# sunzeyeah/item-alignment

Measured on AMD Instinct MI355X. Metric: item-pairs/sec (train step) RoBERTa-large+ViT-B two-tower, higher is better.
Workload: dtype bf16

## Files before the change

include/itemalign.h:

```cpp
#ifndef ITEMALIGN_H
#define ITEMALIGN_H
#include <stddef.h>
#include <stdint.h>

#ifdef __cplusplus
extern "C" {
#endif

typedef struct ihipStream_t* ia_stream_t;

#define IA_OK 0
#define IA_ERR_ARG (-1)
#define IA_ERR_LAUNCH (-2)
#define IA_ERR_WORKSPACE (-3)
#define IA_ERR_UNSUPPORTED (-4)

const char* ia_strerror(int code);
#define IA_ABI_VERSION 17
int ia_abi_version(void);

#define IA_EPI_NONE 0
#define IA_EPI_BIAS 1
#define IA_EPI_BIAS_GELU 2
#define IA_EPI_ADD 3
#define IA_EPI_DGELU 4
#define IA_EPI_BIAS_ADD 5
#define IA_EPI_DGELU_COLSUM 6
#define IA_EPI_BIAS_GELU_ACT 7
int ia_gemm_bf16(const void* A, int a_kstrided, int lda, const void* B, int b_kstrided, int ldb, void* C, int c_is_f32, int ldc,
                 int M, int N, int K, int epilogue, const float* bias, const void* aux, int ldaux, void* C2, int accumulate,
                 void* workspace, size_t workspace_bytes, ia_stream_t stream);
int ia_gemm_bf16_qscale(const void* A, int lda, const void* B, int ldb, void* C, int ldc, int M, int N, int K, const float* bias,
                        int scaled_cols, float col_scale, ia_stream_t stream);
size_t ia_gemm_workspace_bytes(int M, int N, int K, int c_is_f32);
size_t ia_gemm_colsum_workspace_bytes(int M, int N);
size_t ia_gemm_wgrad_rows_workspace_bytes(int N_out, int N_in, int M_rows);
int ia_gemm_wgrad_rows_filters(int N_out, int N_in, int M_rows);
int ia_gemm_wgrad_rows(const void* dY, int ldy, const void* X, int ldx, float* dW, int ldw, int N_out, int N_in, int M_rows,
                       const uint8_t* row_live, int accumulate, void* workspace, size_t workspace_bytes, ia_stream_t stream);
size_t ia_ktile_mask_bytes(int M_rows);
int ia_ktile_mask(const uint8_t* row_live, int M_rows, uint32_t* mask, ia_stream_t stream);
int ia_ktile_mask_host(const uint8_t* row_live, int M_rows, uint32_t* mask);

int ia_prof_begin(int variant, int max_launches);
int ia_prof_end(double* total_ms, double* total_flops, int* launches);
double ia_prof_bytes(void);
int ia_debug_cu_hog(int workgroups, float milliseconds, ia_stream_t stream);
int ia_debug_gemm_dynamic(int on);

int ia_ln_fwd(const void* x, const float* bias, const void* residual, void* z_out, void* y, float* mean, float* rstd,
              const float* gamma, const float* beta, int M, int H, float eps, float drop_p, uint32_t seed, uint32_t stream_id,
              ia_stream_t stream);
size_t ia_ln_bwd_workspace_bytes(int M, int H);
int ia_ln_bwd(const void* dy, const void* dres, const void* z, const float* mean, const float* rstd, const float* gamma, void* dz,
              void* dx, float* dgamma, float* dbeta, float* dbias, int M, int H, float drop_p, uint32_t seed, uint32_t stream_id,
              void* workspace, size_t workspace_bytes, int accumulate, ia_stream_t stream);
int ia_ln_bwd2(const void* dy, const void* dy2, const void* dres, const void* z, const float* mean, const float* rstd, const float* gamma,
               void* dz, void* dx, float* dgamma, float* dbeta, float* dbias, int M, int H, float drop_p, uint32_t seed, uint32_t stream_id,
               void* workspace, size_t workspace_bytes, int accumulate, ia_stream_t stream);
int ia_ln_bwd2_rows(const void* dy, const void* dy2, const void* dres, const void* z, const float* mean, const float* rstd,
                    const float* gamma, void* dz, void* dx, float* dgamma, float* dbeta, float* dbias, int M, int H, float drop_p,
                    uint32_t seed, uint32_t stream_id, const uint8_t* row_live, void* workspace, size_t workspace_bytes, int accumulate,
                    ia_stream_t stream);
size_t ia_colsum_workspace_bytes(int M, int N);
int ia_colsum(const void* x, int ld, int M, int N, float* out, int accumulate, void* workspace, size_t workspace_bytes,
              ia_stream_t stream);

int ia_attn_fwd(const void* q, const void* k, const void* v, int ld_qkv, const uint8_t* key_mask, void* out, int ld_o, float* lse2,
                int B, int nh, int L, float scale, float drop_p, uint32_t seed, ia_stream_t stream);
int ia_attn_bwd(const void* q, const void* k, const void* v, int ld_qkv, const uint8_t* key_mask, const void* out, const void* d_out,
                int ld_o, const float* lse2, float* delta, void* dq, void* dk, void* dv, int ld_dqkv, int B, int nh, int L,
                float scale, float drop_p, uint32_t seed, ia_stream_t stream);
size_t ia_attn_bwd_bias_workspace_bytes(int B, int nh, int L);
int ia_attn_bwd_bias(const void* q, const void* k, const void* v, int ld_qkv, const uint8_t* key_mask, const void* out, const void* d_out,
                     int ld_o, const float* lse2, float* delta, void* dq, void* dk, void* dv, int ld_dqkv, float* dbias, void* workspace,
                     size_t workspace_bytes, int B, int nh, int L, float scale, float drop_p, uint32_t seed, ia_stream_t stream);

int ia_attn_fwd_ps(const void* q, const void* k, const void* v, int ld_qkv, const uint8_t* key_mask, void* out, int ld_o, float* lse2,
                   int B, int nh, int L, float scale, float drop_p, uint32_t seed, ia_stream_t stream);
int ia_attn_bwd_bias_ps(const void* q, const void* k, const void* v, int ld_qkv, const uint8_t* key_mask, const void* out, const void* d_out,
                        int ld_o, const float* lse2, float* delta, void* dq, void* dk, void* dv, int ld_dqkv, float* dbias, void* workspace,
                        size_t workspace_bytes, int B, int nh, int L, float scale, float drop_p, uint32_t seed, ia_stream_t stream);
#define IA_ATTN_Q_PRESCALED 1
#define IA_ATTN_MASKED_ROWS_DEAD 2
int ia_attn_bwd_bias_ex(int flags, const void* q, const void* k, const void* v, int ld_qkv, const uint8_t* key_mask, const void* out,
                        const void* d_out, int ld_o, const float* lse2, float* delta, void* dq, void* dk, void* dv, int ld_dqkv, float* dbias,
                        void* workspace, size_t workspace_bytes, int B, int nh, int L, float scale, float drop_p, uint32_t seed,
                        ia_stream_t stream);

int ia_attn_fwd_x(const void* q, int ld_q, const void* k, const void* v, int ld_kv, const uint8_t* key_mask, void* out, int ld_o,
                  float* lse2, int B, int nh, int Lq, int Lk, float scale, float drop_p, uint32_t seed, ia_stream_t stream);
int ia_attn_bwd_x(const void* q, int ld_q, const void* k, const void* v, int ld_kv, const uint8_t* key_mask, const void* out,
                  const void* d_out, int ld_o, const float* lse2, float* delta, void* dq, int ld_dq, void* dk, void* dv, int ld_dkv,
                  int B, int nh, int Lq, int Lk, float scale, float drop_p, uint32_t seed, ia_stream_t stream);
int ia_attn_fwd_causal_x(const void* q, int ld_q, const void* k, const void* v, int ld_kv, void* out, int ld_o, float* lse2, int B, int nh,
                         int Lk, int fold, float scale, ia_stream_t stream);
int ia_attn_bwd_causal_x(const void* q, int ld_q, const void* k, const void* v, int ld_kv, const void* out, const void* d_out, int ld_o,
                         const float* lse2, float* delta, void* dq, int ld_dq, void* dk, void* dv, int ld_dkv, int B, int nh, int Lk,
                         int fold, float scale, ia_stream_t stream);

int ia_rotary_split_fwd(const void* src, int ld_src, void* q_out, void* kv_out, int M, int n, int nh, ia_stream_t stream);
int ia_rotary_split_bwd(const void* dq, const void* dkv, void* dsrc, int ld_src, int M, int n, int nh, ia_stream_t stream);
int ia_swiglu_fwd(const void* src, int ld_src, void* out, int M, int F, ia_stream_t stream);
int ia_swiglu_bwd(const void* dout, const void* src, int ld_src, void* dsrc, int ld_dsrc, int M, int F, ia_stream_t stream);

int ia_kg_gather_fwd(const float* ent_table, const float* rel_table, const int64_t* ids, int ld_ids, int ent_col, int rel_lo,
                     float* h_sign, float* r, int B, int P, int Dk, ia_stream_t stream);
int ia_kg_gather_bwd(const float* dr, const int64_t* ids, int ld_ids, int rel_lo, float* rel_grad, int B, int P, int Dk,
                     ia_stream_t stream);
int ia_kg_rows_fwd(const float* h, const float* r, const float* hp, float* rows, int rows_per_item, int row0, int B, int P, int H,
                   ia_stream_t stream);
int ia_kg_rows_bwd(const float* drows, int rows_per_item, int row0, float* dh, float* dr, float* dhp, int B, int P, int H,
                   ia_stream_t stream);

#define IA_SIM_INNER 0
#define IA_SIM_COSINE 1
#define IA_SIM_L1 2
#define IA_SIM_L2 3
int ia_pair_sim_fwd(const float* x, const float* y, float* sim, float* probs, int B, int D, int measure, ia_stream_t stream);
int ia_pair_sim_bwd(const float* x, const float* y, const float* sim, const float* probs, const float* dsim, const float* dprobs,
                    float* dx, float* dy, int B, int D, int measure, ia_stream_t stream);

int ia_nchw_to_nhwc_bf16(const float* in, void* out, int B, int C, int H, int W, int Cp, ia_stream_t stream);
size_t ia_conv_nhwc_workspace_bytes(int B, int H, int W, int C, int Cout, int k, int stride, int groups);
int ia_conv_nhwc_fwd(const void* x, const void* what, const float* bias, void* y, int B, int H, int W, int C, int Cout, int k, int stride,
// ... 257 lines not shown
```

item_alignment_amd/_lib.py:

```python
import ctypes as C
import os

_HERE = os.path.dirname(os.path.abspath(__file__))
LIB_PATH = os.path.join(_HERE, "libitemalign_hip.so")

vp, i32, u32, f32, sz = C.c_void_p, C.c_int, C.c_uint32, C.c_float, C.c_size_t
PP, IP = C.POINTER(C.c_void_p), C.POINTER(C.c_int)


class LayerWeights(C.Structure):
    _fields_ = [(n, vp) for n in ("w_qkv", "b_qkv", "w_o", "b_o", "ln1_g", "ln1_b", "w_fc1", "b_fc1", "w_fc2", "b_fc2",
                                  "ln2_g", "ln2_b", "wt_qkv", "wt_o", "wt_fc1", "wt_fc2")]


class LayerGrads(C.Structure):
    _fields_ = [(n, vp) for n in ("w_qkv", "b_qkv", "w_o", "b_o", "ln1_g", "ln1_b", "w_fc1", "b_fc1", "w_fc2", "b_fc2",
                                  "ln2_g", "ln2_b")]


class LayerCfg(C.Structure):
    _fields_ = [("B", i32), ("L", i32), ("H", i32), ("I", i32), ("nh", i32), ("pre_ln", i32), ("eps", f32),
                ("hidden_drop", f32), ("attn_drop", f32), ("seed", u32), ("layer_id", u32), ("cu_seqlens", vp), ("total_tokens", i32),
                ("dx_colsum_out", vp), ("dy_colsum_done", i32), ("masked_rows_dead", i32)]


SIGNATURES = {
    "ia_strerror": (C.c_char_p, [i32]),
    "ia_abi_version": (i32, []),
    "ia_gemm_bf16": (i32, [vp, i32, i32, vp, i32, i32, vp, i32, i32, i32, i32, i32, i32, vp, vp, i32, vp, i32, vp, sz, vp]),
    "ia_gemm_workspace_bytes": (sz, [i32, i32, i32, i32]),
    "ia_gemm_colsum_workspace_bytes": (sz, [i32, i32]),
    "ia_gemm_wgrad_rows_workspace_bytes": (sz, [i32, i32, i32]),
    "ia_gemm_wgrad_rows_filters": (i32, [i32, i32, i32]),
    "ia_gemm_wgrad_rows": (i32, [vp, i32, vp, i32, vp, i32, i32, i32, i32, vp, i32, vp, sz, vp]),
    "ia_ktile_mask_bytes": (sz, [i32]),
    "ia_ktile_mask": (i32, [vp, i32, vp, vp]),
    "ia_ktile_mask_host": (i32, [vp, i32, vp]),
    "ia_prof_begin": (i32, [i32, i32]),
    "ia_prof_end": (i32, [C.POINTER(C.c_double), C.POINTER(C.c_double), C.POINTER(i32)]),
    "ia_prof_bytes": (C.c_double, []),
    "ia_debug_cu_hog": (i32, [i32, C.c_float, vp]),
    "ia_debug_gemm_dynamic": (i32, [i32]),
    "ia_ln_fwd": (i32, [vp, vp, vp, vp, vp, vp, vp, vp, vp, i32, i32, f32, f32, u32, u32, vp]),
    "ia_ln_bwd_workspace_bytes": (sz, [i32, i32]),
    "ia_ln_bwd": (i32, [vp, vp, vp, vp, vp, vp, vp, vp, vp, vp, vp, i32, i32, f32, u32, u32, vp, sz, i32, vp]),
    "ia_ln_bwd2": (i32, [vp, vp, vp, vp, vp, vp, vp, vp, vp, vp, vp, vp, i32, i32, f32, u32, u32, vp, sz, i32, vp]),
    "ia_ln_bwd2_rows": (i32, [vp, vp, vp, vp, vp, vp, vp, vp, vp, vp, vp, vp, i32, i32, f32, u32, u32, vp, vp, sz, i32, vp]),
    "ia_colsum_workspace_bytes": (sz, [i32, i32]),
    "ia_colsum": (i32, [vp, i32, i32, i32, vp, i32, vp, sz, vp]),
    "ia_attn_fwd": (i32, [vp, vp, vp, i32, vp, vp, i32, vp, i32, i32, i32, f32, f32, u32, vp]),
    "ia_attn_bwd": (i32, [vp, vp, vp, i32, vp, vp, vp, i32, vp, vp, vp, vp, vp, i32, i32, i32, i32, f32, f32, u32, vp]),
    "ia_attn_bwd_bias_workspace_bytes": (sz, [i32, i32, i32]),
    "ia_attn_bwd_bias": (i32, [vp, vp, vp, i32, vp, vp, vp, i32, vp, vp, vp, vp, vp, i32, vp, vp, sz, i32, i32, i32, f32, f32, u32, vp]),
    "ia_attn_fwd_ps": (i32, [vp, vp, vp, i32, vp, vp, i32, vp, i32, i32, i32, f32, f32, u32, vp]),
    "ia_attn_bwd_bias_ps": (i32, [vp, vp, vp, i32, vp, vp, vp, i32, vp, vp, vp, vp, vp, i32, vp, vp, sz, i32, i32, i32, f32, f32, u32, vp]),
    "ia_attn_bwd_bias_ex": (i32, [i32, vp, vp, vp, i32, vp, vp, vp, i32, vp, vp, vp, vp, vp, i32, vp, vp, sz, i32, i32, i32, f32, f32, u32, vp]),
    "ia_gemm_bf16_qscale": (i32, [vp, i32, vp, i32, vp, i32, i32, i32, i32, vp, i32, f32, vp]),
    "ia_attn_fwd_x": (i32, [vp, i32, vp, vp, i32, vp, vp, i32, vp, i32, i32, i32, i32, f32, f32, u32, vp]),
    "ia_attn_bwd_x": (i32, [vp, i32, vp, vp, i32, vp, vp, vp, i32, vp, vp, vp, i32, vp, vp, i32, i32, i32, i32, i32, f32, f32, u32, vp]),
    "ia_attn_fwd_causal_x": (i32, [vp, i32, vp, vp, i32, vp, i32, vp, i32, i32, i32, i32, f32, vp]),
    "ia_attn_bwd_causal_x": (i32, [vp, i32, vp, vp, i32, vp, vp, i32, vp, vp, vp, i32, vp, vp, i32, i32, i32, i32, i32, f32, vp]),
    "ia_rotary_split_fwd": (i32, [vp, i32, vp, vp, i32, i32, i32, vp]),
    "ia_rotary_split_bwd": (i32, [vp, vp, vp, i32, i32, i32, i32, vp]),
    "ia_swiglu_fwd": (i32, [vp, i32, vp, i32, i32, vp]),
    "ia_swiglu_bwd": (i32, [vp, vp, i32, vp, i32, i32, i32, vp]),
    "ia_kg_gather_fwd": (i32, [vp, vp, vp, i32, i32, i32, vp, vp, i32, i32, i32, vp]),
    "ia_kg_gather_bwd": (i32, [vp, vp, i32, i32, vp, i32, i32, i32, vp]),
    "ia_kg_rows_fwd": (i32, [vp, vp, vp, vp, i32, i32, i32, i32, i32, vp]),
    "ia_kg_rows_bwd": (i32, [vp, i32, i32, vp, vp, vp, i32, i32, i32, vp]),
    "ia_pair_sim_fwd": (i32, [vp, vp, vp, vp, i32, i32, i32, vp]),
    "ia_pair_sim_bwd": (i32, [vp, vp, vp, vp, vp, vp, vp, vp, i32, i32, i32, vp]),
    "ia_nchw_to_nhwc_bf16": (i32, [vp, vp, i32, i32, i32, i32, i32, vp]),
    "ia_conv_nhwc_workspace_bytes": (sz, [i32, i32, i32, i32, i32, i32, i32, i32]),
    "ia_conv_nhwc_fwd": (i32, [vp, vp, vp, vp, i32, i32, i32, i32, i32, i32, i32, i32, vp, sz, vp]),
    "ia_conv_nhwc_bwd_data": (i32, [vp, vp, vp, i32, i32, i32, i32, i32, i32, i32, i32, vp, sz, vp]),
    "ia_conv_nhwc_bwd_weight": (i32, [vp, vp, vp, vp, i32, i32, i32, i32, i32, i32, i32, i32, i32, vp, sz, vp]),
    "ia_ws_conv_weight_fwd": (i32, [vp, vp, vp, vp, vp, i32, i32, i32, i32, f32, f32, vp]),
    "ia_ws_conv_weight_bwd": (i32, [vp, vp, vp, vp, vp, vp, vp, i32, i32, i32, i32, f32, vp]),
    "ia_silu_fwd": (i32, [vp, vp, sz, f32, vp]),
    "ia_silu_bwd": (i32, [vp, vp, vp, vp, sz, f32, vp]),
    "ia_silu_bwd_sum": (i32, [vp, vp, vp, vp, vp, sz, f32, vp]),
    "ia_avgpool2_fwd": (i32, [vp, vp, i32, i32, i32, i32, vp]),
    "ia_avgpool2_bwd": (i32, [vp, vp, i32, i32, i32, i32, vp]),
    "ia_gap_workspace_bytes": (sz, [i32, i32, i32]),
    "ia_gap_fwd": (i32, [vp, vp, i32, i32, i32, vp, sz, vp]),
    "ia_gap_bwd": (i32, [vp, vp, i32, i32, i32, vp]),
    "ia_eca_fwd": (i32, [vp, vp, i32, vp, vp, vp, vp, i32, i32, i32, f32, vp, sz, vp]),
    "ia_eca_fwd_linear_workspace_bytes": (sz, [i32, i32, i32]),
    "ia_eca_fwd_linear": (i32, [vp, vp, vp, vp, i32, vp, i32, vp, vp, vp, f32, vp, vp, i32, i32, i32, f32, vp, sz, vp]),
    "ia_eca_silu_bwd": (i32, [vp, vp, vp, vp, f32, vp, vp, i32, vp, vp, vp, vp, vp, i32, i32, i32, f32, vp, sz, vp]),
    "ia_eca_bwd_workspace_bytes": (sz, [i32, i32, i32]),
    "ia_eca_bwd": (i32, [vp, vp, vp, i32, vp, vp, vp, vp, i32, i32, i32, f32, vp, sz, vp]),
    "ia_conv3x3_padded_fwd": (i32, [vp, vp, vp, vp, i32, i32, i32, i32, i32, i32, vp]),
    "ia_conv3x3_padded_bwd_data": (i32, [vp, vp, vp, i32, i32, i32, i32, i32, i32, vp]),
    "ia_conv3x3_direct_supported": (i32, [i32, i32, i32]),
    "ia_conv3x3_flip_weights": (i32, [vp, vp, i32, i32, i32, vp]),
    "ia_conv3x3_padded_bwd_data_t": (i32, [vp, vp, vp, i32, i32, i32, i32, i32, i32, vp]),
    "ia_conv3x3_padded_workspace_bytes": (sz, [i32, i32, i32, i32, i32, i32]),
    "ia_conv3x3_padded_bwd_weight": (i32, [vp, vp, vp, vp, i32, i32, i32, i32, i32, i32, vp, sz, vp]),
    "ia_pad_rows": (i32, [vp, vp, i32, i32, i32, i32, i32, i32, vp]),
    "ia_silu_pad_fwd": (i32, [vp, vp, i32, i32, i32, i32, f32, i32, i32, vp]),
    "ia_silu_pad_bwd": (i32, [vp, vp, vp, i32, i32, i32, i32, f32, i32, i32, vp]),
    "ia_bn_act_workspace_bytes": (sz, [i32, i32, i32]),
    "ia_bn_act_fwd": (i32, [vp, vp, vp, vp, vp, vp, vp, vp, i32, i32, i32, f32, f32, i32, i32, vp, sz, vp]),
    "ia_bn_act_bwd": (i32, [vp, vp, vp, vp, vp, vp, vp, vp, vp, vp, i32, i32, i32, i32, i32, vp, sz, vp]),
    "ia_patches_nchw": (i32, [vp, vp, i32, i32, i32, i32, i32, i32, i32, i32, vp]),
    "ia_conv3x3_s2_supported": (i32, [i32, i32, i32]),
    "ia_conv3x3_s2_padded_workspace_bytes": (sz, [i32, i32, i32, i32, i32, i32]),
    "ia_conv3x3_s2_padded_fwd": (i32, [vp, vp, vp, vp, i32, i32, i32, i32, i32, i32, i32, vp]),
    "ia_conv3x3_s2_padded_bwd_weight": (i32, [vp, vp, vp, vp, i32, i32, i32, i32, i32, i32, i32, vp, sz, vp]),
    "ia_conv3x3_s2_padded_bwd_data_t": (i32, [vp, vp, vp, i32, i32, i32, i32, i32, i32, i32, vp]),
    "ia_gn_act_workspace_bytes": (sz, [i32, i32, i32]),
    "ia_gn_act_fwd": (i32, [vp, vp, vp, vp, vp, vp, i32, i32, i32, i32, f32, i32, vp, sz, vp]),
    "ia_gn_act_bwd": (i32, [vp, vp, vp, vp, vp, vp, vp, vp, vp, vp, i32, i32, i32, i32, i32, vp, sz, vp]),
    "ia_maxpool3s2_fwd": (i32, [vp, vp, vp, i32, i32, i32, i32, vp]),
    "ia_maxpool3s2_fwd_ex": (i32, [vp, vp, vp, i32, i32, i32, i32, i32, vp]),
    "ia_maxpool3s2_bwd": (i32, [vp, vp, vp, i32, i32, i32, i32, vp]),
    "ia_rows_subsample_fwd": (i32, [vp, vp, i32, i32, i32, i32, i32, vp]),
    "ia_rows_subsample_bwd": (i32, [vp, vp, vp, i32, i32, i32, i32, i32, vp]),
    "ia_conv_weight_pack": (i32, [vp, vp, i32, i32, i32, i32, i32, vp]),
    "ia_conv_weight_unpack_grad": (i32, [vp, vp, i32, i32, i32, i32, i32, vp]),
    "ia_resize_pass_u8": (i32, [vp, vp, vp, vp, i32, i32, i32, i32, i32, i32, vp]),
    "ia_resize_pass_u8_ex": (i32, [vp, sz, sz, vp, vp, vp, i32, i32, i32, i32, i32, i32, vp]),
    "ia_color_jitter_step_u8": (i32, [vp, vp, vp, vp, i32, i32, i32, i32, vp]),
    "ia_u8_to_nchw_normalized": (i32, [vp, vp, vp, i32, i32, i32, C.POINTER(f32), C.POINTER(f32), vp]),
    "ia_embed_ln_fwd": (i32, [vp, vp, vp, vp, vp, vp, vp, vp, vp, vp, vp, vp, vp, vp, i32, i32, f32, f32, u32, u32, vp]),
    "ia_embed_ln_bwd_workspace_bytes": (sz, [i32, i32]),
    "ia_embed_ln_bwd": (i32, [vp, vp, vp, vp, vp, vp, vp, vp, vp, vp, vp, vp, vp, vp, vp, vp, vp, vp, vp, i32, i32, i32, i32, i32, f32, u32, u32,
                               vp, sz, vp]),
    "ia_im2col_patch": (i32, [vp, vp, i32, i32, i32, i32, vp]),
    "ia_vit_tokens_fwd": (i32, [vp, vp, vp, vp, i32, i32, i32, vp]),
    "ia_vit_tokens_bwd": (i32, [vp, vp, vp, vp, i32, i32, i32, i32, vp]),
    "ia_gather_rows_fwd": (i32, [vp, i32, vp, vp, i32, i32, f32, u32, u32, vp]),
    "ia_gather_rows_bwd": (i32, [vp, i32, vp, vp, i32, i32, f32, u32, u32, i32, vp]),
    "ia_linear_small_fwd": (i32, [vp, i32, vp, vp, vp, i32, i32, i32, i32, vp]),
    "ia_linear_small_bwd": (i32, [vp, vp, vp, i32, vp, vp, i32, vp, vp, i32, i32, i32, i32, vp]),
    "ia_pair_head_ce_fwd": (i32, [vp, vp, vp, vp, vp, vp, vp, vp, vp, i32, i32, i32, vp]),
    "ia_attn_fwd_varlen": (i32, [vp, vp, vp, i32, vp, i32, vp, i32, vp, i32, i32, i32, f32, f32, u32, vp]),
    "ia_attn_bwd_varlen": (i32, [vp, vp, vp, i32, vp, i32, vp, vp, i32, vp, vp, vp, vp, vp, i32, i32, i32, i32, f32, f32, u32, vp]),
    "ia_attn_fwd_varlen_ps": (i32, [vp, vp, vp, i32, vp, i32, vp, i32, vp, i32, i32, i32, f32, f32, u32, vp]),
    "ia_attn_bwd_varlen_ps": (i32, [vp, vp, vp, i32, vp, i32, vp, vp, i32, vp, vp, vp, vp, vp, i32, i32, i32, i32, f32, f32, u32, vp]),
    "ia_span_mean_fwd": (i32, [vp, i32, vp, vp, i32, i32, vp]),
    "ia_span_mean_bwd": (i32, [vp, vp, vp, vp, i32, i32, i32, vp]),
    "ia_pair_head_ce_bwd": (i32, [vp, vp, vp, vp, vp, vp, vp, vp, vp, vp, i32, i32, i32, vp]),
    "ia_transpose_bf16_batched": (i32, [vp, vp, vp, i32, i32, vp]),
    "ia_adamw_flat": (i32, [vp, vp, vp, vp, vp, vp, i32, f32, f32, f32, f32, f32, i32, f32, vp]),
    "ia_kgpt_workspace_bytes": (sz, [i32, i32, i32]),
    "ia_kgpt_score": (i32, [vp, vp, vp, vp, vp, vp, vp, vp, i32, i32, i32, i32, i32, i32, f32, vp, vp, vp, vp, vp, vp, vp, vp, vp, vp, vp, sz,
                            vp]),
    "ia_kgpt_adam_l2": (i32, [vp, vp, vp, vp, sz, f32, f32, f32, f32, f32, i32, vp]),
    "ia_kgpt_row_normalize": (i32, [vp, i32, i32, vp]),
    "ia_kgpt_corrupt": (i32, [vp, vp, vp, i32, vp, i32, i32, C.c_uint64, vp, vp, vp]),
    "ia_kgpt_lp_workspace_bytes": (sz, [i32, i32]),
    "ia_kgpt_lp_rank": (i32, [vp, vp, vp, vp, vp, i32, i32, i32, i32, i32, i32, vp, vp, i32, vp, vp, vp, vp, vp, sz, vp]),
    "ia_gcn_propagate_fwd": (i32, [vp, vp, i32, vp, vp, vp, vp, i32, i32, f32, f32, u32, u32, vp, i32, vp]),
    "ia_gcn_propagate_bwd": (i32, [vp, vp, i32, vp, vp, vp, vp, i32, i32, i32, f32, f32, u32, u32, vp, i32, vp]),
    "ia_gcn_mix_fwd": (i32, [vp, vp, vp, i32, i32, f32, f32, u32, u32, vp]),
    "ia_gcn_workspace_bytes": (sz, [i32, i32, i32]),
    "ia_gcn_mix_bwd": (i32, [vp, vp, vp, vp, vp, vp, i32, i32, f32, f32, vp, sz, vp]),
    "ia_gcn_input_fwd": (i32, [vp, vp, vp, vp, i32, i32, i32, f32, u32, u32, vp]),
    "ia_gcn_input_bwd": (i32, [vp, vp, vp, vp, vp, i32, i32, i32, f32, u32, u32, vp, sz, vp]),
    "ia_gcn_pair_gather_fwd": (i32, [vp, vp, vp, i32, i32, i32, f32, u32, u32, vp]),
    "ia_gcn_pair_scatter_bwd": (i32, [vp, vp, vp, vp, i32, i32, i32, f32, u32, u32, vp]),
    "ia_textcnn_pack_taps": (i32, [PP, IP, i32, i32, i32, vp, vp]),
    "ia_textcnn_pool_fwd": (i32, [vp, i32, PP, IP, i32, i32, i32, i32, f32, f32, u32, u32, u32, vp, vp, vp]),
    "ia_textcnn_pool_bwd_w": (i32, [vp, vp, vp, vp, IP, i32, i32, i32, i32, i32, f32, f32, u32, u32, u32, PP, PP, vp]),
    "ia_textcnn_pool_bwd_x": (i32, [vp, vp, PP, IP, i32, i32, i32, i32, i32, f32, f32, u32, u32, u32, vp, vp]),
    "ia_cast_f32_to_bf16": (i32, [vp, vp, sz, vp]),
    "ia_cast_bf16_to_f32": (i32, [vp, vp, sz, vp]),
    "ia_layer_stash_bytes": (sz, [C.POINTER(LayerCfg)]),
    "ia_layer_bwd_scratch_bytes": (sz, [C.POINTER(LayerCfg)]),
    "ia_layer_fwd": (i32, [C.POINTER(LayerCfg), C.POINTER(LayerWeights), vp, vp, vp, vp, vp]),
    "ia_comm_unique_id": (i32, [vp]),
    "ia_comm_init": (i32, [vp, i32, i32, C.POINTER(vp)]),
    "ia_comm_allreduce_bucket": (i32, [vp, vp, sz, i32, vp]),
    "ia_comm_finalize": (i32, [vp]),
    "ia_comm_last_error": (C.c_char_p, []),
    "ia_layer_infer_scratch_bytes": (sz, [C.POINTER(LayerCfg)]),
    "ia_layer_fwd_infer": (i32, [C.POINTER(LayerCfg), C.POINTER(LayerWeights), vp, vp, vp, vp, sz, vp]),
    "ia_layer_bwd": (i32, [C.POINTER(LayerCfg), C.POINTER(LayerWeights), C.POINTER(LayerGrads), vp, vp, vp, vp, vp, vp, vp, sz, vp]),
    "ia_layer_bwd2": (i32, [C.POINTER(LayerCfg), C.POINTER(LayerWeights), C.POINTER(LayerGrads), vp, vp, vp, vp, vp, vp, vp, vp, vp, sz, vp]),
}

_lib = None


ABI_VERSION = 17


class ItemAlignError(RuntimeError):
    pass


def load():
    global _lib
    if _lib is not None:
        return _lib
    if not os.path.exists(LIB_PATH):
        raise ItemAlignError(
            f"{LIB_PATH} not found: build it with `python -c 'import __graft_entry__ as g; g.build()'` "
            "(or `make -C item_alignment_amd/csrc`). The MI355X path has no CPU fallback.")
    import torch
    lib = C.CDLL(LIB_PATH)
    for name, (res, args) in SIGNATURES.items():
        fn = getattr(lib, name)
        fn.restype = res
        fn.argtypes = args
    got = lib.ia_abi_version()
    if got != ABI_VERSION:
        raise ItemAlignError(f"{LIB_PATH} has ABI version {got}, this package needs {ABI_VERSION} (include/itemalign.h: IA_ABI_VERSION): "
                             "stale build, run `make -C item_alignment_amd/csrc`")
    _lib = lib
    return lib


def check(rc, what):
    if rc != 0:
        msg = load().ia_strerror(rc).decode()
        raise ItemAlignError(f"{what} failed: {msg} (code {rc})")


def stream_ptr():
    import torch
    return torch.cuda.current_stream().cuda_stream


def ptr(t):
    return None if t is None else t.data_ptr()
```

item_alignment_amd/csrc/common.h:

```cpp
#pragma once
#include <hip/hip_runtime.h>
#include <stdint.h>

typedef __bf16 bf16;
typedef __attribute__((ext_vector_type(8))) __bf16 bf16x8;
typedef __attribute__((ext_vector_type(4))) __bf16 bf16x4;
typedef __attribute__((ext_vector_type(2))) __bf16 bf16x2;
typedef __attribute__((ext_vector_type(4))) short s16x4;
typedef __attribute__((ext_vector_type(8))) short s16x8;
typedef __attribute__((ext_vector_type(4))) float f32x4;
typedef __attribute__((ext_vector_type(2))) float f32x2;
typedef __attribute__((ext_vector_type(16))) float f32x16;
typedef __attribute__((ext_vector_type(4))) uint32_t u32x4;
typedef __attribute__((ext_vector_type(2))) uint32_t u32x2;

#define IA_LDS(p) ((__attribute__((address_space(3))) void*)(p))
#define IA_DEV __device__ __forceinline__

IA_DEV uint32_t ia_lds_addr(const void* p) { return (uint32_t)(uintptr_t)IA_LDS(p); }
template <int OFF>
IA_DEV s16x4 ia_tr_read(uint32_t lds_byte_addr) {
  s16x4 d;
  asm volatile("ds_read_b64_tr_b16 %0, %1 offset:%2" : "=v"(d) : "v"(lds_byte_addr), "n"(OFF));
  return d;
// ... 55 lines not shown
IA_DEV uint32_t ia_mix32(uint32_t x) {
  x ^= x >> 16; x *= 0x7feb352dU; x ^= x >> 15; x *= 0x846ca68bU; x ^= x >> 16;
  return x;
}
IA_DEV uint32_t ia_rng(uint32_t seed, uint32_t stream, uint32_t idx) {
  return ia_mix32(idx ^ ia_mix32(stream ^ (seed * 0x9E3779B9U)));
}

constexpr uint32_t IA_RNG_PAIR_C = 0x9E3779B1U;
IA_DEV uint32_t ia_rng_row(uint32_t seed, uint32_t stream, uint32_t row) { return ia_mix32(row ^ ia_mix32(stream ^ (seed * 0x9E3779B9U))); }
IA_DEV uint32_t ia_rng_pair(uint32_t rowkey, uint32_t pair_c) {
  const uint32_t h = (rowkey ^ pair_c) * 0x846ca68bU;
  return h ^ (h >> 16);
}

IA_DEV void gelu_parts(float x, float& cdf, float& pdf) {
  const float z = fabsf(x) * 0.70710678118654752f;
  const float t = __builtin_amdgcn_rcpf(1.0f + 0.3275911f * z);
  const float e = __builtin_amdgcn_exp2f(x * x * (-0.5f * 1.4426950408889634f));
  const float poly = t * (0.254829592f + t * (-0.284496736f + t * (1.421413741f + t * (-1.453152027f + t * 1.061405429f))));
  const float erf_abs = 1.0f - poly * e;
  cdf = 0.5f * (1.0f + copysignf(erf_abs, x));
  pdf = 0.3989422804014327f * e;
}
typedef float f32x2_t __attribute__((ext_vector_type(2)));
IA_DEV void gelu_pair(f32x2_t x, f32x2_t& act, f32x2_t& der) {
  constexpr float L2E = 1.4426950408889634f;
  constexpr float C0 = 1.5949398799788077f, C1 = 0.07403000634661838f, C2 = -0.0007007124749191571f;
  constexpr float U_MAX = C1 / (2.f * 0.0007007124749191571f);
  f32x2_t u = x * x;
  u[0] = __builtin_fminf(u[0], U_MAX); u[1] = __builtin_fminf(u[1], U_MAX);
  const f32x2_t np = (u * (-C2 * L2E) + (-C1 * L2E)) * u + (-C0 * L2E);
  const f32x2_t t = x * np;
  const f32x2_t e = {__builtin_amdgcn_exp2f(t[0]), __builtin_amdgcn_exp2f(t[1])};
  const f32x2_t den = e + 1.0f;
  const f32x2_t s = {__builtin_amdgcn_rcpf(den[0]), __builtin_amdgcn_rcpf(den[1])};
  act = x * s;
  const f32x2_t q = (u * (5.f * C2) + (3.f * C1)) * u + C0;
  const f32x2_t r = 1.0f - s;
  der = (act * r) * q + s;
}
IA_DEV f32x2_t gelu_act_pair(f32x2_t x) {
  constexpr float L2E = 1.4426950408889634f;
  constexpr float C0 = 1.5949398799788077f, C1 = 0.07403000634661838f, C2 = -0.0007007124749191571f;
  constexpr float U_MAX = C1 / (2.f * 0.0007007124749191571f);
  f32x2_t u = x * x;
  u[0] = __builtin_fminf(u[0], U_MAX); u[1] = __builtin_fminf(u[1], U_MAX);
  const f32x2_t t = x * ((u * (-C2 * L2E) + (-C1 * L2E)) * u + (-C0 * L2E));
  const f32x2_t e = {__builtin_amdgcn_exp2f(t[0]), __builtin_amdgcn_exp2f(t[1])};
  const f32x2_t den = e + 1.0f;
  return x * f32x2_t{__builtin_amdgcn_rcpf(den[0]), __builtin_amdgcn_rcpf(den[1])};
}
IA_DEV float gelu_erf(float x) { float c, d; gelu_parts(x, c, d); return x * c; }
IA_DEV float gelu_erf_grad(float x) { float c, d; gelu_parts(x, c, d); return c + x * d; }

inline hipError_t g_ia_last_hip_error = hipSuccess;
static inline int ia_check_launch() {
  hipError_t e = hipGetLastError();
  if (e != hipSuccess) g_ia_last_hip_error = e;
  return e == hipSuccess ? IA_OK : IA_ERR_LAUNCH;
}

struct IaViewGemm {
  const void* A; int a_kstrided, lda;
  const void* B; int b_kstrided, ldb;
  void* C; int c_is_f32, ldc;
  int M, N, K;
  const float* bias;
  float* rsum_out;
  void* workspace; size_t workspace_bytes;
  int a_view, b_view, pw, lca, lcbk, lcbn;
  size_t a_window, b_window;
  int groups; long ga, gb, gc, gbias;
};
__attribute__((visibility("hidden"))) int ia_gemm_view(const IaViewGemm& v, hipStream_t stream);
__attribute__((visibility("hidden"))) int ia_sum_rows_f32(const float* part, int nblk, int N, float* out, int accumulate, hipStream_t stream);
extern "C" size_t ia_colsum_workspace_bytes(int M, int N);
extern "C" int ia_colsum(const void* x, int ld, int M, int N, float* out, int accumulate, void* workspace, size_t workspace_bytes,
                         hipStream_t stream);
__attribute__((visibility("hidden"))) size_t ia_gemm_view_workspace_bytes(int M, int N, int K, int groups);
__attribute__((visibility("hidden"))) int ia_gemm_wgrad_masked(const void* dY, int ldy, const void* X, int ldx, float* dW, int ldw, int N_out,
                                                               int N_in, int M_rows, const uint32_t* ktile_mask, int accumulate,
                                                               void* workspace, size_t workspace_bytes, hipStream_t stream);
```

item_alignment_amd/csrc/engine.hip:

```cpp
#include "common.h"
#include "../../include/itemalign.h"

namespace {

inline size_t al(size_t b) { return (b + 255) & ~(size_t)255; }
inline size_t rows_of(const ia_layer_cfg* c) { return c->cu_seqlens ? (size_t)c->total_tokens : (size_t)c->B * c->L; }

struct Carver {
  char* base; size_t bytes = 0;
  char* take(size_t b) { char* r = base ? base + bytes : nullptr; bytes += al(b); return r; }
};

struct FwdBufs {
  char* qkv; char* ctx;
  char* xn;
  char* proj;
  char* ln;
  char* ffn;
  char* hpre;
  char* hact;
  float* lse; float* mean1; float* rstd1; float* mean2; float* rstd2;
  size_t bytes;
};

void name_rows(FwdBufs& s, bool pre_ln, char* t0, char* t1, char* t2) {
  if (pre_ln) { s.xn = t0; s.proj = t1; s.ln = t2; s.ffn = nullptr; }
  else { s.xn = nullptr; s.proj = t0; s.ln = t1; s.ffn = t2; }
}

FwdBufs carve_stash(const ia_layer_cfg* c, void* base) {
  const size_t M = rows_of(c), H = c->H, I = c->I;
  Carver a{(char*)base};
  FwdBufs s;
  s.qkv = a.take(M * 3 * H * 2); s.ctx = a.take(M * H * 2);
  char* t0 = a.take(M * H * 2); char* t1 = a.take(M * H * 2); char* t2 = a.take(M * H * 2);
  name_rows(s, c->pre_ln, t0, t1, t2);
  s.hpre = a.take(M * I * 2); s.hact = a.take(M * I * 2);
  s.lse = (float*)a.take((size_t)c->B * c->nh * c->L * 4);
  s.mean1 = (float*)a.take(M * 4); s.rstd1 = (float*)a.take(M * 4);
  s.mean2 = (float*)a.take(M * 4); s.rstd2 = (float*)a.take(M * 4);
  s.bytes = a.bytes;
  return s;
}

FwdBufs carve_infer(const ia_layer_cfg* c, void* base) {
  const size_t M = rows_of(c), H = c->H, I = c->I;
  Carver a{(char*)base};
  FwdBufs s;
  s.qkv = a.take(M * 3 * H * 2); s.ctx = a.take(M * H * 2);
  char* t0 = a.take(M * H * 2); char* t1 = a.take(M * H * 2);
  name_rows(s, c->pre_ln, t0, t1, t0);
  s.hpre = nullptr; s.hact = a.take(M * I * 2);
  s.lse = (float*)a.take((size_t)c->B * c->nh * c->L * 4);
  s.mean1 = s.mean2 = (float*)a.take(M * 4); s.rstd1 = s.rstd2 = (float*)a.take(M * 4);
  s.bytes = a.bytes;
  return s;
}

struct Scratch {
  char* g0; char* g1; char* g2; char* gI; char* gqkv; float* delta; char* ws; size_t ws_bytes; char* gws; size_t gws_bytes; uint32_t* live_kt; size_t bytes;
};

size_t max3(size_t a, size_t b, size_t c) { return a > b ? (a > c ? a : c) : (b > c ? b : c); }

Scratch carve_scratch(const ia_layer_cfg* c, void* base) {
  const size_t M = rows_of(c), H = c->H, I = c->I;
  Carver a{(char*)base};
  Scratch s;
  s.g0 = a.take(M * H * 2); s.g1 = a.take(M * H * 2); s.g2 = a.take(M * H * 2);
  s.gI = a.take(M * I * 2); s.gqkv = a.take(M * 3 * H * 2);
  s.delta = (float*)a.take((size_t)c->B * c->nh * c->L * 4);
  s.ws_bytes = max3(ia_ln_bwd_workspace_bytes((int)M, (int)H), ia_gemm_colsum_workspace_bytes((int)M, (int)I),
                    max3(ia_colsum_workspace_bytes((int)M, (int)(3 * H)), ia_attn_bwd_bias_workspace_bytes(c->B, c->nh, c->L), 0));
  s.ws = a.take(s.ws_bytes);
  s.gws_bytes = max3(ia_gemm_workspace_bytes((int)(3 * H), (int)H, (int)M, 1), ia_gemm_workspace_bytes((int)I, (int)H, (int)M, 1),
                     max3(ia_gemm_workspace_bytes((int)H, (int)I, (int)M, 1), ia_gemm_workspace_bytes((int)H, (int)H, (int)M, 1), 0));
  s.gws = a.take(s.gws_bytes);
  s.live_kt = (uint32_t*)a.take(ia_ktile_mask_bytes((int)M));
  s.bytes = a.bytes;
  return s;
}

bool cfg_ok(const ia_layer_cfg* c) {
  if (c && c->cu_seqlens && (c->total_tokens <= 0 || c->total_tokens > c->B * c->L)) return false;
  return c && c->B > 0 && c->L > 0 && c->H > 0 && c->I > 0 && c->nh > 0 && c->H == c->nh * 64 && (c->H & 7) == 0 && (c->I & 7) == 0;
}

#define IA_TRY(expr) do { int rc_ = (expr); if (rc_) return rc_; } while (0)

int dgrad(const void* dy, int k_out, const void* w, const void* wt, int n_in, void* dx, int M, int epilogue, const void* aux, int ldaux, void* c2,
          void* ws, size_t ws_bytes, ia_stream_t st) {
  if (wt)
    return ia_gemm_bf16(dy, 0, k_out, wt, 0, k_out, dx, 0, n_in, M, n_in, k_out, epilogue, nullptr, aux, ldaux, c2, 0, ws, ws_bytes, st);
  return ia_gemm_bf16(dy, 0, k_out, w, 1, n_in, dx, 0, n_in, M, n_in, k_out, epilogue, nullptr, aux, ldaux, c2, 0, ws, ws_bytes, st);
}

int wgrad(const void* dy, int n_out, const void* x, int n_in, float* dw, int M, const uint32_t* live_kt, void* ws, size_t ws_bytes, ia_stream_t st) {
  if (live_kt) return ia_gemm_wgrad_masked(dy, n_out, x, n_in, dw, n_in, n_out, n_in, M, live_kt, 1, ws, ws_bytes, st);
  return ia_gemm_bf16(dy, 1, n_out, x, 1, n_in, dw, 1, n_in, n_out, n_in, M, IA_EPI_NONE, nullptr, nullptr, 0, nullptr, 1, ws, ws_bytes, st);
}

bool q_prescale(const ia_layer_cfg* c) { return (c->H & 127) == 0; }
int qkv_proj(const ia_layer_cfg* c, const void* x, const ia_layer_weights* w, void* qkv, int M, float scale, ia_stream_t st) {
  const int H = c->H;
  if (q_prescale(c)) return ia_gemm_bf16_qscale(x, H, w->w_qkv, H, qkv, 3 * H, M, 3 * H, H, w->b_qkv, H, scale * 1.4426950408889634f, st);
  return ia_gemm_bf16(x, 0, H, w->w_qkv, 0, H, qkv, 0, 3 * H, M, 3 * H, H, IA_EPI_BIAS, w->b_qkv, nullptr, 0, nullptr, 0, nullptr, 0, st);
}

int attn_fwd(const ia_layer_cfg* c, const char* qkv, const uint8_t* key_mask, char* ctx, float* lse, float scale, float drop, uint32_t seed,
             ia_stream_t st) {
  const int H = c->H;
  const bool ps = q_prescale(c);
  if (c->cu_seqlens)
    return (ps ? ia_attn_fwd_varlen_ps : ia_attn_fwd_varlen)(qkv, qkv + (size_t)H * 2, qkv + (size_t)2 * H * 2, 3 * H, c->cu_seqlens, c->total_tokens, ctx, H, lse, c->B, c->nh,
                              c->L, scale, drop, seed, st);
  return (ps ? ia_attn_fwd_ps : ia_attn_fwd)(qkv, qkv + (size_t)H * 2, qkv + (size_t)2 * H * 2, 3 * H, key_mask, ctx, H, lse, c->B, c->nh, c->L, scale, drop, seed, st);
}

int attn_bwd(const ia_layer_cfg* c, const char* qkv, const uint8_t* key_mask, const char* ctx, const char* dctx, const float* lse, float* delta,
             char* gqkv, float* db_qkv, void* ws, size_t ws_bytes, float scale, float drop, uint32_t seed, ia_stream_t st) {
  const int H = c->H;
  const bool ps = q_prescale(c);
  if (c->cu_seqlens) {
    int rc = (ps ? ia_attn_bwd_varlen_ps : ia_attn_bwd_varlen)(qkv, qkv + (size_t)H * 2, qkv + (size_t)2 * H * 2, 3 * H, c->cu_seqlens, c->total_tokens, ctx, dctx, H, lse, delta,
                                gqkv, gqkv + (size_t)H * 2, gqkv + (size_t)2 * H * 2, 3 * H, c->B, c->nh, c->L, scale, drop, seed, st);
    return rc ? rc : ia_colsum(gqkv, 3 * H, (int)rows_of(c), 3 * H, db_qkv, 1, ws, ws_bytes, st);
  }
  const int flags = (ps ? IA_ATTN_Q_PRESCALED : 0) | (c->masked_rows_dead ? IA_ATTN_MASKED_ROWS_DEAD : 0);
  return ia_attn_bwd_bias_ex(flags, qkv, qkv + (size_t)H * 2, qkv + (size_t)2 * H * 2, 3 * H, key_mask, ctx, dctx, H, lse, delta, gqkv,
                             gqkv + (size_t)H * 2, gqkv + (size_t)2 * H * 2, 3 * H, db_qkv, ws, ws_bytes, c->B, c->nh, c->L, scale, drop, seed, st);
}

int layer_forward(const ia_layer_cfg* c, const ia_layer_weights* w, const void* x, const uint8_t* key_mask, void* y, const FwdBufs& s,
                  bool keep, ia_stream_t st) {
  const int M = (int)rows_of(c), H = c->H, I = c->I;
  const float scale = 0.125f;
  const int gelu = keep ? IA_EPI_BIAS_GELU : IA_EPI_BIAS_GELU_ACT;
  if (!c->pre_ln) {
    const float hidden_drop = keep ? c->hidden_drop : 0.f, attn_drop = keep ? c->attn_drop : 0.f;
    const uint32_t seed = keep ? c->seed : 0u, attn_seed = keep ? c->seed * 2654435761u + c->layer_id * 97u + 17u : 0u;
    const uint32_t ln1_stream = keep ? c->layer_id * 4u + 0u : 0u, ln2_stream = keep ? c->layer_id * 4u + 1u : 0u;
    IA_TRY(qkv_proj(c, x, w, s.qkv, M, scale, st));
    IA_TRY(attn_fwd(c, s.qkv, key_mask, s.ctx, s.lse, scale, attn_drop, attn_seed, st));
    IA_TRY(ia_gemm_bf16(s.ctx, 0, H, w->w_o, 0, H, s.proj, 0, H, M, H, H, IA_EPI_NONE, nullptr, nullptr, 0, nullptr, 0, nullptr, 0, st));
    IA_TRY(ia_ln_fwd(s.proj, w->b_o, x, keep ? s.proj : nullptr, s.ln, s.mean1, s.rstd1, w->ln1_g, w->ln1_b, M, H, c->eps, hidden_drop, seed,
                     ln1_stream, st));
    IA_TRY(ia_gemm_bf16(s.ln, 0, H, w->w_fc1, 0, H, s.hact, 0, I, M, I, H, gelu, w->b_fc1, nullptr, 0, s.hpre, 0, nullptr, 0, st));
    IA_TRY(ia_gemm_bf16(s.hact, 0, I, w->w_fc2, 0, I, s.ffn, 0, H, M, H, I, IA_EPI_NONE, nullptr, nullptr, 0, nullptr, 0, nullptr, 0, st));
    IA_TRY(ia_ln_fwd(s.ffn, w->b_fc2, s.ln, keep ? s.ffn : nullptr, y, s.mean2, s.rstd2, w->ln2_g, w->ln2_b, M, H, c->eps, hidden_drop, seed,
                     ln2_stream, st));
  } else {
    IA_TRY(ia_ln_fwd(x, nullptr, nullptr, nullptr, s.xn, s.mean1, s.rstd1, w->ln1_g, w->ln1_b, M, H, c->eps, 0.f, 0, 0, st));
    IA_TRY(qkv_proj(c, s.xn, w, s.qkv, M, scale, st));
    IA_TRY(attn_fwd(c, s.qkv, key_mask, s.ctx, s.lse, scale, 0.f, 0, st));
    IA_TRY(ia_gemm_bf16(s.ctx, 0, H, w->w_o, 0, H, s.proj, 0, H, M, H, H, IA_EPI_NONE, nullptr, nullptr, 0, nullptr, 0, nullptr, 0, st));
    IA_TRY(ia_ln_fwd(s.proj, w->b_o, x, s.proj, s.ln, s.mean2, s.rstd2, w->ln2_g, w->ln2_b, M, H, c->eps, 0.f, 0, 0, st));
    IA_TRY(ia_gemm_bf16(s.ln, 0, H, w->w_fc1, 0, H, s.hact, 0, I, M, I, H, gelu, w->b_fc1, nullptr, 0, s.hpre, 0, nullptr, 0, st));
    IA_TRY(ia_gemm_bf16(s.hact, 0, I, w->w_fc2, 0, I, y, 0, H, M, H, I, IA_EPI_BIAS_ADD, w->b_fc2, s.proj, H, nullptr, 0, nullptr, 0, st));
  }
  return IA_OK;
}

}

extern "C" size_t ia_layer_stash_bytes(const ia_layer_cfg* cfg) {
  (void)hipGetLastError();
  if (!cfg_ok(cfg)) return 0;
  return carve_stash(cfg, nullptr).bytes;
}

extern "C" size_t ia_layer_bwd_scratch_bytes(const ia_layer_cfg* cfg) {
  (void)hipGetLastError();
  if (!cfg_ok(cfg)) return 0;
  return carve_scratch(cfg, nullptr).bytes;
}

extern "C" size_t ia_layer_infer_scratch_bytes(const ia_layer_cfg* cfg) {
  (void)hipGetLastError();
  if (!cfg_ok(cfg)) return 0;
  return carve_infer(cfg, nullptr).bytes;
}

extern "C" int ia_layer_fwd(const ia_layer_cfg* c, const ia_layer_weights* w, const void* x, const uint8_t* key_mask, void* y,
                            void* stash, ia_stream_t st) {
  (void)hipGetLastError();
  if (!cfg_ok(c) || !w || !x || !y || !stash) return IA_ERR_ARG;
  if (c->pre_ln && (c->hidden_drop > 0.f || c->attn_drop > 0.f)) return IA_ERR_UNSUPPORTED;
  return layer_forward(c, w, x, key_mask, y, carve_stash(c, stash), true, st);
}

extern "C" int ia_layer_fwd_infer(const ia_layer_cfg* c, const ia_layer_weights* w, const void* x, const uint8_t* key_mask, void* y,
                                  void* scratch, size_t scratch_bytes, ia_stream_t st) {
  (void)hipGetLastError();
  if (!cfg_ok(c) || !w || !x || !y || !scratch) return IA_ERR_ARG;
  if (scratch_bytes < ia_layer_infer_scratch_bytes(c)) return IA_ERR_WORKSPACE;
  return layer_forward(c, w, x, key_mask, y, carve_infer(c, scratch), false, st);
}

extern "C" int ia_layer_bwd2(const ia_layer_cfg* c, const ia_layer_weights* w, const ia_layer_grads* g, const void* x,
                             const uint8_t* key_mask, const void* y, const void* stash, const void* dy, const void* dy2, void* dx, void* dx2,
                             void* scratch, size_t scratch_bytes, ia_stream_t st);

extern "C" int ia_layer_bwd(const ia_layer_cfg* c, const ia_layer_weights* w, const ia_layer_grads* g, const void* x,
                            const uint8_t* key_mask, const void* y, const void* stash, const void* dy, void* dx, void* scratch,
                            size_t scratch_bytes, ia_stream_t st) {
  return ia_layer_bwd2(c, w, g, x, key_mask, y, stash, dy, nullptr, dx, nullptr, scratch, scratch_bytes, st);
}

extern "C" int ia_layer_bwd2(const ia_layer_cfg* c, const ia_layer_weights* w, const ia_layer_grads* g, const void* x,
                             const uint8_t* key_mask, const void* y, const void* stash, const void* dy, const void* dy2, void* dx, void* dx2,
                             void* scratch, size_t scratch_bytes, ia_stream_t st) {
  (void)hipGetLastError();
  (void)y;
  if (!cfg_ok(c) || !w || !g || !x || !stash || !dy || !dx || !scratch) return IA_ERR_ARG;
  if (c->pre_ln && (dy2 || dx2)) return IA_ERR_UNSUPPORTED;
  if (scratch_bytes < ia_layer_bwd_scratch_bytes(c)) return IA_ERR_WORKSPACE;
  const int M = (int)rows_of(c), H = c->H, I = c->I;
  const FwdBufs s = carve_stash(c, const_cast<void*>(stash));
  const Scratch k = carve_scratch(c, scratch);
  const float scale = 0.125f;
  const uint32_t attn_seed = c->seed * 2654435761u + c->layer_id * 97u + 17u;
  const bool drop = c->hidden_drop > 0.f;
  if (!c->pre_ln) {
    const uint8_t* const live = (c->masked_rows_dead && !c->cu_seqlens) ? key_mask : nullptr;
    const uint32_t* const live_kt = live ? k.live_kt : nullptr;
    if (live) IA_TRY(ia_ktile_mask(live, M, k.live_kt, st));
    IA_TRY(ia_ln_bwd2_rows(dy, dy2, nullptr, s.ffn, s.mean2, s.rstd2, w->ln2_g, k.g0, drop ? k.g1 : nullptr, g->ln2_g, g->ln2_b, g->b_fc2, M, H,
                           c->hidden_drop, c->seed, c->layer_id * 4u + 1u, live, k.ws, k.ws_bytes, 1, st));
    const char* d_ffn = drop ? k.g1 : k.g0;
    IA_TRY(wgrad(d_ffn, H, s.hact, I, (float*)g->w_fc2, M, live_kt, k.gws, k.gws_bytes, st));
    IA_TRY(dgrad(d_ffn, H, w->w_fc2, w->wt_fc2, I, k.gI, M, IA_EPI_DGELU_COLSUM, s.hpre, I, g->b_fc1, k.ws, k.ws_bytes, st));
    IA_TRY(wgrad(k.gI, I, s.ln, H, (float*)g->w_fc1, M, live_kt, k.gws, k.gws_bytes, st));
    IA_TRY(dgrad(k.gI, I, w->w_fc1, w->wt_fc1, H, k.g2, M, IA_EPI_NONE, nullptr, 0, nullptr, nullptr, 0, st));
    char* dz1buf = dx2 ? (char*)dx2 : k.g0;
    IA_TRY(ia_ln_bwd2_rows(k.g2, k.g0, nullptr, s.proj, s.mean1, s.rstd1, w->ln1_g, dz1buf, drop ? k.g1 : nullptr, g->ln1_g, g->ln1_b, g->b_o, M, H,
                           c->hidden_drop, c->seed, c->layer_id * 4u + 0u, live, k.ws, k.ws_bytes, 1, st));
    const char* d_att = drop ? k.g1 : dz1buf;
    IA_TRY(wgrad(d_att, H, s.ctx, H, (float*)g->w_o, M, live_kt, k.gws, k.gws_bytes, st));
    IA_TRY(dgrad(d_att, H, w->w_o, w->wt_o, H, k.g2, M, IA_EPI_NONE, nullptr, 0, nullptr, nullptr, 0, st));
    IA_TRY(attn_bwd(c, s.qkv, key_mask, s.ctx, k.g2, s.lse, k.delta, k.gqkv, g->b_qkv, k.ws, k.ws_bytes, scale, c->attn_drop, attn_seed, st));
    IA_TRY(wgrad(k.gqkv, 3 * H, x, H, (float*)g->w_qkv, M, live_kt, k.gws, k.gws_bytes, st));
    if (dx2)
      IA_TRY(dgrad(k.gqkv, 3 * H, w->w_qkv, w->wt_qkv, H, dx, M, IA_EPI_NONE, nullptr, 0, nullptr, nullptr, 0, st));
    else
      IA_TRY(dgrad(k.gqkv, 3 * H, w->w_qkv, w->wt_qkv, H, dx, M, IA_EPI_ADD, dz1buf, H, nullptr, nullptr, 0, st));
  } else {
    if (!c->dy_colsum_done) IA_TRY(ia_colsum(dy, H, M, H, g->b_fc2, 1, k.ws, k.ws_bytes, st));
    IA_TRY(ia_gemm_bf16(dy, 1, H, s.hact, 1, I, g->w_fc2, 1, I, H, I, M, IA_EPI_NONE, nullptr, nullptr, 0, nullptr, 1, k.gws, k.gws_bytes, st));
    IA_TRY(dgrad(dy, H, w->w_fc2, w->wt_fc2, I, k.gI, M, IA_EPI_DGELU_COLSUM, s.hpre, I, g->b_fc1, k.ws, k.ws_bytes, st));
    IA_TRY(ia_gemm_bf16(k.gI, 1, I, s.ln, 1, H, g->w_fc1, 1, H, I, H, M, IA_EPI_NONE, nullptr, nullptr, 0, nullptr, 1, k.gws, k.gws_bytes, st));
    IA_TRY(dgrad(k.gI, I, w->w_fc1, w->wt_fc1, H, k.g0, M, IA_EPI_NONE, nullptr, 0, nullptr, nullptr, 0, st));
    IA_TRY(ia_ln_bwd(k.g0, dy, s.proj, s.mean2, s.rstd2, w->ln2_g, k.g1, nullptr, g->ln2_g, g->ln2_b, g->b_o, M, H, 0.f, 0, 0, k.ws,
                     k.ws_bytes, 1, st));
    IA_TRY(ia_gemm_bf16(k.g1, 1, H, s.ctx, 1, H, g->w_o, 1, H, H, H, M, IA_EPI_NONE, nullptr, nullptr, 0, nullptr, 1, k.gws, k.gws_bytes, st));
    IA_TRY(dgrad(k.g1, H, w->w_o, w->wt_o, H, k.g2, M, IA_EPI_NONE, nullptr, 0, nullptr, nullptr, 0, st));
    IA_TRY(attn_bwd(c, s.qkv, key_mask, s.ctx, k.g2, s.lse, k.delta, k.gqkv, g->b_qkv, k.ws, k.ws_bytes, scale, 0.f, 0, st));
    IA_TRY(ia_gemm_bf16(k.gqkv, 1, 3 * H, s.xn, 1, H, g->w_qkv, 1, H, 3 * H, H, M, IA_EPI_NONE, nullptr, nullptr, 0, nullptr, 1, k.gws, k.gws_bytes, st));
    IA_TRY(dgrad(k.gqkv, 3 * H, w->w_qkv, w->wt_qkv, H, k.g0, M, IA_EPI_NONE, nullptr, 0, nullptr, nullptr, 0, st));
    IA_TRY(ia_ln_bwd(k.g0, k.g1, x, s.mean1, s.rstd1, w->ln1_g, dx, nullptr, g->ln1_g, g->ln1_b, c->dx_colsum_out, M, H, 0.f, 0, 0, k.ws,
                     k.ws_bytes, 1, st));
  }
  return IA_OK;
}
```

item_alignment_amd/csrc/gemm.hip:

```cpp
#include "common.h"
#include <atomic>
#include <cstdlib>
#include <type_traits>

#ifndef IA_GEMM_DBG_HOOKS
#define IA_GEMM_DBG_HOOKS 0
#endif
#define IA_DBG(p) (IA_GEMM_DBG_HOOKS ? (p).dbg : 0)

namespace {

constexpr int BK = 64;
constexpr uint32_t OOB = 0xFFFFFFF0u;

enum { EPI_NONE = 0, EPI_BIAS = 1, EPI_BIAS_GELU = 2, EPI_ADD = 3, EPI_DGELU = 4, EPI_BIAS_ADD = 5, EPI_DGELU_CS = 6, EPI_BIAS_GELU_ACT = 7 };
constexpr int EPI_NONE_LIVE = 8;

struct GemmArgs {
  const bf16* A; const bf16* B; void* C; bf16* C2;
  union {
    const float* bias;
    const uint32_t* live_kt;
  };
  const bf16* aux;
  int M, N, K;
  int lda, ldb, ldc, ldaux;
  uint64_t a_bytes, b_bytes;
  int accumulate;
  int qcols; float qscale;
  int tiles_m, tiles_n;
  int splits, nk_per_split;
  float* csum_part;
  int split_id;
  float* ws;
  float* rsum_out;
  float* rsum_ws;
  int dbg;
  int a_view, b_view, pw, lca, lcbk, lcbn;
  int groups;
  long ga, gb, gc, gbias;
  uint32_t* tile_ctr;
};

constexpr int CTR_SLOTS = 1024, CTR_WORDS = 16;
__device__ uint32_t g_tile_ctr[CTR_SLOTS * CTR_WORDS];

IA_DEV int tap_delta(int t, int pw) { return (t / 3 - 1) * pw + (t % 3 - 1); }

IA_DEV __amdgpu_buffer_rsrc_t rsrc_at(const bf16* base, uint64_t total_bytes, uint64_t origin) {
  const uint64_t ob = origin * 2, rem = total_bytes > ob ? total_bytes - ob : 0;
  return ia_rsrc(base + origin, (uint32_t)(rem < 0x7FFFFFF0ull ? rem : 0x7FFFFFF0ull));
}

template <int EPI, bool OUTF32>
IA_DEV void epi_store4(const GemmArgs& p, int m, int n, f32x4 v) {
  if (EPI == EPI_BIAS || EPI == EPI_BIAS_GELU || EPI == EPI_BIAS_GELU_ACT || EPI == EPI_BIAS_ADD) {
    const f32x4 b = *reinterpret_cast<const f32x4*>(p.bias + n);
    v += b;
    if (EPI == EPI_BIAS && n < p.qcols) v *= p.qscale;
  }
  if (EPI == EPI_BIAS_GELU) {
    bf16x4 der;
#pragma unroll
    for (int r = 0; r < 4; r += 2) {
      f32x2_t a, d;
      gelu_pair(f32x2_t{v[r], v[r + 1]}, a, d);
      v[r] = a[0]; v[r + 1] = a[1];
      der[r] = f2bf(d[0]); der[r + 1] = f2bf(d[1]);
    }
    *reinterpret_cast<bf16x4*>(p.C2 + (size_t)m * p.ldc + n) = der;
  }
  if (EPI == EPI_BIAS_GELU_ACT) {
#pragma unroll
    for (int r = 0; r < 4; r += 2) {
      const f32x2_t a = gelu_act_pair(f32x2_t{v[r], v[r + 1]});
      v[r] = a[0]; v[r + 1] = a[1];
    }
  }
  if (EPI == EPI_ADD || EPI == EPI_BIAS_ADD) {
    const bf16x4 a = *reinterpret_cast<const bf16x4*>(p.aux + (size_t)m * p.ldaux + n);
#pragma unroll
    for (int r = 0; r < 4; ++r) v[r] += bf2f(a[r]);
  }
  if (EPI == EPI_DGELU || EPI == EPI_DGELU_CS) {
    const bf16x4 a = *reinterpret_cast<const bf16x4*>(p.aux + (size_t)m * p.ldaux + n);
#pragma unroll
    for (int r = 0; r < 4; ++r) v[r] *= bf2f(a[r]);
  }
  if (OUTF32) {
    if (p.splits > 1) {
      *reinterpret_cast<f32x4*>(p.ws + ((size_t)p.split_id * p.M + m) * p.N + n) = v;
      return;
    }
    float* c = reinterpret_cast<float*>(p.C) + (size_t)m * p.ldc + n;
    if (p.accumulate) { const f32x4 o = *reinterpret_cast<const f32x4*>(c); v += o; }
    *reinterpret_cast<f32x4*>(c) = v;
  } else {
    bf16x4 o = {f2bf(v[0]), f2bf(v[1]), f2bf(v[2]), f2bf(v[3])};
    *reinterpret_cast<bf16x4*>(reinterpret_cast<bf16*>(p.C) + (size_t)m * p.ldc + n) = o;
  }
}

template <typename V>
IA_DEV void gstore16(void* ptr, V v) {
  static_assert(sizeof(V) == 16, "16-byte store");
// ... 377 lines not shown
  bf16x8 d;
  asm volatile("ds_read_b128 %0, %1 offset:%2" : "=v"(d) : "v"(addr), "n"(IMM));
  return d;
}
template <int IMM>
IA_DEV s16x4 rd_tr(uint32_t addr) {
  s16x4 d;
  asm volatile("ds_read_b64_tr_b16 %0, %1 offset:%2" : "=v"(d) : "v"(addr), "n"(IMM));
  return d;
}

template <bool KS>
IA_DEV void frag_bases(uint32_t (&base)[4], uint32_t tile_addr, int x0, int lane, int nperm_row) {
  if (!KS) {
    const int hh = lane >> 5;
    const int row = x0 + nperm_row;
#pragma unroll
    for (int ks = 0; ks < 4; ++ks) base[ks] = tile_addr + row * 128 + ((((ks * 2 + hh) ^ ((row >> 1) & 7))) << 4);
  } else {
    const int p = lane & 15, G = lane >> 4;
#pragma unroll
    for (int j = 0; j < 4; ++j) {
      const int row = 8 * (G >> 1) + (p >> 2);
      const int col = x0 + j * 32 + 16 * (G & 1) + (p & 3) * 4;
      base[j] = tile_addr + row * 512 + ((((col >> 3) ^ ((row & 3) << 2))) << 4) + (col & 7) * 2;
    }
  }
}

template <int N> IA_DEV void tie(Op<false>& o) {
  asm volatile("s_waitcnt lgkmcnt(%4)" : "+v"(o.v[0]), "+v"(o.v[1]), "+v"(o.v[2]), "+v"(o.v[3]) : "n"(N));
}
template <int N> IA_DEV void tie2(Op<false>& a, Op<false>& b) {
  asm volatile("s_waitcnt lgkmcnt(%8)" : "+v"(a.v[0]), "+v"(a.v[1]), "+v"(a.v[2]), "+v"(a.v[3]), "+v"(b.v[0]), "+v"(b.v[1]), "+v"(b.v[2]), "+v"(b.v[3]) : "n"(N));
}
template <int N> IA_DEV void tie6(Op<false>& a, Op<false>& b, Op<false>& c, Op<false>& d, Op<false>& e, Op<false>& f) {
  asm volatile("s_waitcnt lgkmcnt(%24)"
               : "+v"(a.v[0]), "+v"(a.v[1]), "+v"(a.v[2]), "+v"(a.v[3]), "+v"(b.v[0]), "+v"(b.v[1]), "+v"(b.v[2]), "+v"(b.v[3]),
                 "+v"(c.v[0]), "+v"(c.v[1]), "+v"(c.v[2]), "+v"(c.v[3]), "+v"(d.v[0]), "+v"(d.v[1]), "+v"(d.v[2]), "+v"(d.v[3]),
                 "+v"(e.v[0]), "+v"(e.v[1]), "+v"(e.v[2]), "+v"(e.v[3]), "+v"(f.v[0]), "+v"(f.v[1]), "+v"(f.v[2]), "+v"(f.v[3])
               : "n"(N));
}
template <int N> IA_DEV void tie(Op<true>& o) {
  asm volatile("s_waitcnt lgkmcnt(%8)" : "+v"(o.lo[0]), "+v"(o.lo[1]), "+v"(o.lo[2]), "+v"(o.lo[3]), "+v"(o.hi[0]), "+v"(o.hi[1]), "+v"(o.hi[2]), "+v"(o.hi[3]) : "n"(N));
}
template <int N> IA_DEV void tie2(Op<true>& a, Op<true>& b) { tie<N>(a); tie<N>(b); }
template <int N> IA_DEV void tie6(Op<true>& a, Op<true>& b, Op<true>& c, Op<true>& d, Op<true>& e, Op<true>& f) {
  tie<N>(a); tie<N>(b); tie<N>(c); tie<N>(d); tie<N>(e); tie<N>(f);
}


template <int S, bool KS>
IA_DEV void read_frag(Op<KS>& f, int j, const uint32_t (&base)[4], uint32_t bufoff) {
  if constexpr (!KS) {
    const uint32_t a = base[S] + bufoff;
    if (j == 0) f.v[0] = rd128<0>(a);
    if (j == 1) f.v[1] = rd128<4096>(a);
    if (j == 2) f.v[2] = rd128<8192>(a);
    if (j == 3) f.v[3] = rd128<12288>(a);
  } else {
    f.lo[j] = rd_tr<S * 8192>(base[j] + bufoff);
    f.hi[j] = rd_tr<S * 8192 + 4 * 512>(base[j] + bufoff);
  }
}

template <bool FRESH, typename FA, typename FB, typename Filler>
IA_DEV void mfma_step(f32x16 (&acc)[4][4], const FA& fa, const FB& fb, Filler&& filler) {
  bf16x8 va[4], vb[4];
#pragma unroll
  for (int j = 0; j < 4; ++j) { va[j] = frag_of(fa, j); vb[j] = frag_of(fb, j); }
#pragma unroll
  for (int mi = 0; mi < 4; ++mi)
#pragma unroll
    for (int ni = 0; ni < 4; ++ni) {
      if constexpr (FRESH) {
        const f32x16 z = {0.f, 0.f, 0.f, 0.f, 0.f, 0.f, 0.f, 0.f, 0.f, 0.f, 0.f, 0.f, 0.f, 0.f, 0.f, 0.f};
        acc[mi][ni] = __builtin_amdgcn_mfma_f32_32x32x16_bf16(vb[ni], va[mi], z, 0, 0, 0);
      } else acc[mi][ni] = __builtin_amdgcn_mfma_f32_32x32x16_bf16(vb[ni], va[mi], acc[mi][ni], 0, 0, 0);
      filler(mi * 4 + ni);
      __builtin_amdgcn_sched_barrier(0);
    }
}

struct LiveWalk {
  uint64_t rest;
  uint32_t w;
  int wi, cur;
};
IA_DEV void live_start(LiveWalk& k, uint32_t mv) { k.rest = __ballot(mv != 0u); k.w = 0u; k.wi = 0; k.cur = -1; }
IA_DEV int live_next(LiveWalk& k, uint32_t mv) {
  const bool open = k.w == 0u, any = k.rest != 0ull;
  const int wi = open ? (any ? __builtin_ctzll(k.rest) : 0) : k.wi;
  const uint32_t fetched = __builtin_amdgcn_readlane(mv, wi);
  const uint32_t w = open ? (any ? fetched : 0u) : k.w;
  k.rest = open ? (k.rest & (k.rest - 1ull)) : k.rest;
  const int idx = w != 0u ? wi * 32 + __builtin_ctz(w) : k.cur + 1;
  k.w = w & (w - 1u); k.wi = wi; k.cur = idx;
  return idx;
}

template <bool AKS, bool BKS, int PEND, bool PEEL_OK = true, bool LIVE = false>
IA_DEV void main_loop(const GemmArgs& p, char* smem, f32x16 (&acc)[4][4], __amdgpu_buffer_rsrc_t rsA, __amdgpu_buffer_rsrc_t rsB, int xa, int xb,
                      int kt0, int ktaA0, int ktaB0, int n_tiles, int nk_all, int wm, int wn, int wave, int lane, bool prologue_only,
                      bool stores_in_flight, uint32_t live_mv = 0u) {
  static_assert(!LIVE || (AKS && BKS), "the live-k-tile walk advances the running lane offsets of two k-strided operands");
  constexpr bool ROUND = !AKS && !BKS;
  const int li = lane & 31;
  const int gt = wave * 64 + lane;
  uint32_t voffA, stepA, voffB, stepB;
  if (!AKS) { const int row = gt >> 3; voffA = (uint32_t)(((xa + row) * p.lda + (((gt & 7) ^ ((row >> 1) & 7)) * 8)) * 2); stepA = (uint32_t)(32 * p.lda * 2); }
  else { const int row = gt >> 5; voffA = (uint32_t)((row * p.lda + xa + (((gt & 31) ^ ((row & 3) << 2)) * 8)) * 2); stepA = (uint32_t)(8 * p.lda * 2); }
  if (!BKS) { const int row = gt >> 3; voffB = (uint32_t)(((xb + row) * p.ldb + (((gt & 7) ^ ((row >> 1) & 7)) * 8)) * 2); stepB = (uint32_t)(32 * p.ldb * 2); }
  else { const int row = gt >> 5; voffB = (uint32_t)((row * p.ldb + xb + (((gt & 31) ^ ((row & 3) << 2)) * 8)) * 2); stepB = (uint32_t)(8 * p.ldb * 2); }
  const uint32_t kstepA = AKS ? (uint32_t)(BK * p.lda * 2) : (uint32_t)(BK * 2), kstepB = BKS ? (uint32_t)(BK * p.ldb * 2) : (uint32_t)(BK * 2);
  const int klA = AKS ? (gt >> 5) : ((gt & 7) ^ (((gt >> 3) >> 1) & 7)) * 8;
  const int klB = BKS ? (gt >> 5) : ((gt & 7) ^ (((gt >> 3) >> 1) & 7)) * 8;
  char* const my_part = smem + wave * 1024;
  const int dbg = IA_GEMM_DBG_HOOKS ? p.dbg : 0;
  const bool dma_on = !(dbg & 2);
  [[maybe_unused]] LiveWalk lw;
  int live0 = 0, live1 = 1;
  if constexpr (LIVE) { live_start(lw, live_mv); live0 = live_next(lw, live_mv); live1 = live_next(lw, live_mv); }

  auto dma_piece = [&](int u, int i) {
    const bool isB = i >= 8;
    const int j = i & 7;
    char* dst = my_part + (isB ? TILE_BYTES : 0) + (u & 1) * 2 * TILE_BYTES + j * 4096;
    const int kt = kt0 + u;
    const int kta = (dbg & 4) ? 0 : (isB ? ktaB0 : ktaA0) + (LIVE ? (u == 0 ? live0 : live1) : u);
    const bool ks = isB ? BKS : AKS;
    const uint32_t soff = (uint32_t)kta * (isB ? kstepB : kstepA) + (uint32_t)j * (isB ? stepB : stepA);
    if (ks) {
      const uint32_t off = (dma_on && (!LIVE || u < n_tiles)) ? (isB ? voffB : voffA) + soff : OOB;
      __builtin_amdgcn_raw_ptr_buffer_load_lds(isB ? rsB : rsA, IA_LDS(dst), 16, off, 0, 0, 0);
    } else {
      const int lim = (u < n_tiles && dma_on) ? p.K - kt * BK : 0;
      const uint32_t off = (isB ? klB : klA) + (ks ? j * 8 : 0) < lim ? (isB ? voffB : voffA) : OOB;
      __builtin_amdgcn_raw_ptr_buffer_load_lds(isB ? rsB : rsA, IA_LDS(dst), 16, off, (int)soff, 0, 0);
    }
  };

  auto off_of = [&](int u, bool isB) -> uint32_t {
    const int lim = (u < n_tiles && dma_on) ? p.K - (kt0 + u) * BK : 0;
    return (isB ? klB : klA) < lim ? (isB ? voffB : voffA) : OOB;
  };
  auto dma_c = [&](int u, int i, uint32_t off) {
    const bool isB = i >= 8;
    const int j = i & 7;
    char* dst = my_part + (isB ? TILE_BYTES : 0) + (u & 1) * 2 * TILE_BYTES + j * 4096;
    const int kta = (dbg & 4) ? 0 : (isB ? ktaB0 : ktaA0) + u;
    const uint32_t soff = (uint32_t)kta * (isB ? kstepB : kstepA) + (uint32_t)j * (isB ? stepB : stepA);
    __builtin_amdgcn_raw_ptr_buffer_load_lds(isB ? rsB : rsA, IA_LDS(dst), 16, off, (int)soff, 0, 0);
  };

  int live2 = 2;
  if constexpr (LIVE) { if (!prologue_only) live2 = live_next(lw, live_mv); }
  uint32_t runA = voffA + (uint32_t)((dbg & 4) ? 0 : ktaA0 + live2) * kstepA, runB = voffB + (uint32_t)((dbg & 4) ? 0 : ktaB0 + live2) * kstepB;
  auto dma_run = [&](int u, int i) {
    const bool isB = i >= 8;
    if (!(isB ? BKS : AKS) || (dbg & 4)) { dma_piece(u, i); return; }
    const int j = i & 7;
    char* dst = my_part + (isB ? TILE_BYTES : 0) + (u & 1) * 2 * TILE_BYTES + j * 4096;
    const uint32_t off = (isB ? runB : runA) + (uint32_t)j * (isB ? stepB : stepA);
    __builtin_amdgcn_raw_ptr_buffer_load_lds(isB ? rsB : rsA, IA_LDS(dst), 16, dma_on ? off : OOB, 0, 0, 0);
  };

  if (prologue_only) {
#pragma unroll
    for (int i = 0; i < 16; ++i) dma_piece(0, i);
#pragma unroll
    for (int i = 0; i < (ROUND ? 12 : 16); ++i) dma_piece(1, i);
    return;
  }
  if (stores_in_flight) asm volatile("s_waitcnt vmcnt(%0)" : : "n"(PEND < 60 ? PEND : 60) : "memory");
  else asm volatile("s_waitcnt vmcnt(0)" ::: "memory");
  __builtin_amdgcn_s_barrier();

  const int nperm = ((li >> 2) & 1) * 16 + (li >> 3) * 4 + (li & 3);
  uint32_t baseA[4], baseB[4];
  const uint32_t smem_addr = ia_lds_addr(smem);
  frag_bases<AKS>(baseA, smem_addr, wm * 128, lane, li);
  frag_bases<BKS>(baseB, smem_addr + TILE_BYTES, wn * 128, lane, nperm);
  constexpr int NRA = AKS ? 8 : 4, NRB = BKS ? 8 : 4, NR = NRA + NRB;
  constexpr int NR15 = NR > 15 ? 15 : NR;

  Op<AKS> a0, a1, a2, a3;
  Op<BKS> b0, b1, b2, b3;
#pragma unroll
  for (int j = 0; j < 4; ++j) read_frag<0>(a0, j, baseA, 0u);
#pragma unroll
  for (int j = 0; j < 4; ++j) read_frag<0>(b0, j, baseB, 0u);

  using Acc = std::false_type;

  uint32_t bo = 0;
  int u = 0;
  if constexpr (ROUND) {
  uint32_t offA = OOB, offB = off_of(1, true);
  auto trip = [&](auto FIRST_T) {
    const uint32_t bn = bo ^ (uint32_t)(2 * TILE_BYTES);
    tie2<0>(a0, b0);
    mfma_step<decltype(FIRST_T)::value>(acc, a0, b0, [&](int i) {
      if (i < 4) { read_frag<1>(a1, i, baseA, bo); read_frag<1>(b1, i, baseB, bo); }
      else if (i < 8) { read_frag<2>(a2, i - 4, baseA, bo); read_frag<2>(b2, i - 4, baseB, bo); }
      else if (i < 12) { read_frag<3>(a3, i - 8, baseA, bo); read_frag<3>(b3, i - 8, baseB, bo); }
      if (i % 4 == 3) dma_c(u + 1, 12 + i / 4, offB);
      if (i == 12) offA = off_of(u + 2, false);
    });
    tie6<0>(a1, b1, a2, b2, a3, b3);
    __builtin_amdgcn_sched_barrier(0);
    if (!(dbg & 16)) __builtin_amdgcn_s_barrier();
    __builtin_amdgcn_sched_barrier(0);
    mfma_step<false>(acc, a1, b1, [&](int i) {
      if (i % 4 == 1) dma_c(u + 2, i / 4, offA);
    });
    mfma_step<false>(acc, a2, b2, [&](int i) {
      if (i % 4 == 1) dma_c(u + 2, 4 + i / 4, offA);
      if (i == 14) offB = off_of(u + 2, true);
    });
    asm volatile("s_waitcnt vmcnt(8)" ::: "memory");
    __builtin_amdgcn_sched_barrier(0);
    if (!(dbg & 16)) __builtin_amdgcn_s_barrier();
    __builtin_amdgcn_sched_barrier(0);
    mfma_step<false>(acc, a3, b3, [&](int i) {
      if (i < 4) read_frag<0>(a0, i, baseA, bn);
      else if (i < 8) read_frag<0>(b0, i - 4, baseB, bn);
      if (i % 4 == 3) dma_c(u + 2, 8 + i / 4, offB);
    });
    bo = bn;
    ++u;
    };
  if constexpr (PEEL_OK) {
    trip(std::true_type{});
    do { trip(Acc{}); } while (u < n_tiles);
  } else {
    do { trip(Acc{}); } while (u < n_tiles);
  }
  tie2<0>(a0, b0);
  return;
  }
  do {
    const uint32_t bn = bo ^ (uint32_t)(2 * TILE_BYTES);
    tie<0>(a0); tie<0>(b0);
    mfma_step<false>(acc, a0, b0, [&](int i) {
      if (i < 4) read_frag<1>(a1, i, baseA, bo);
      else if (i < 8) read_frag<1>(b1, i - 4, baseB, bo);
      else if (i < 12) read_frag<2>(a2, i - 8, baseA, bo);
      else read_frag<2>(b2, i - 12, baseB, bo);
    });
    tie<NR15>(a1); tie<NR15>(b1);
    mfma_step<false>(acc, a1, b1, [&](int i) {
      if (i < 4) read_frag<3>(a3, i, baseA, bo);
      else if (i < 8) read_frag<3>(b3, i - 4, baseB, bo);
    });
    tie<0>(a2); tie<0>(b2); tie<0>(a3); tie<0>(b3);
    __builtin_amdgcn_sched_barrier(0);
    if (!(dbg & 16)) __builtin_amdgcn_s_barrier();
    __builtin_amdgcn_sched_barrier(0);
    mfma_step<false>(acc, a2, b2, [&](int i) {
      if (i & 1) dma_run(u + 2, i >> 1);
    });
    asm volatile("s_waitcnt vmcnt(8)" ::: "memory");
    __builtin_amdgcn_sched_barrier(0);
    if (!(dbg & 16)) __builtin_amdgcn_s_barrier();
    __builtin_amdgcn_sched_barrier(0);
    mfma_step<false>(acc, a3, b3, [&](int i) {
      if (i & 1) dma_run(u + 2, 8 + (i >> 1));
      if (!(i & 1)) {
        if (i < 8) read_frag<0>(a0, i >> 1, baseA, bn);
        else read_frag<0>(b0, (i - 8) >> 1, baseB, bn);
      }
    });
    bo = bn;
    ++u;
    if constexpr (LIVE) {
      const int at = lw.cur;
      const uint32_t hop = (uint32_t)(live_next(lw, live_mv) - at);
      runA += hop * kstepA; asm volatile("" : "+v"(runA));
      runB += hop * kstepB; asm volatile("" : "+v"(runB));
    } else {
      if (AKS) { runA += kstepA; asm volatile("" : "+v"(runA)); }
      if (BKS) { runB += kstepB; asm volatile("" : "+v"(runB)); }
    }
  } while (u < n_tiles);
  tie<0>(a0); tie<0>(b0);
}

template <bool BKS, int NH, bool WITH_BIAS>
IA_DEV void drain_half_plain(const GemmArgs& p, f32x16 (&acc)[4][4], int m0, int n0, char* stg, int lane_e, const f32x4 (&bct)[4][4], float ts = 1.f) {
  static_assert(!(WITH_BIAS && BKS), "bias rows are laid out for the k-contiguous B fragment permutation");
  const int hh = lane_e >> 5, li = lane_e & 31, rrow = lane_e >> 3, c8 = lane_e & 7;
  auto stage = [&](int mi) {
    char* const sl = stg + (mi & 1) * 4096;
#pragma unroll
    for (int ni = 0; ni < 2; ++ni) {
      f32x16& a = acc[mi][NH * 2 + ni];
      if (!BKS) {
#pragma unroll
        for (int h8 = 0; h8 < 2; ++h8) {
          f32x4 t0, t1;
#pragma unroll
          for (int j = 0; j < 4; ++j) {
            asm volatile("v_accvgpr_read_b32 %0, %1" : "=v"(t0[j]) : "a"(a[h8 * 8 + j]));
            asm volatile("v_accvgpr_read_b32 %0, %1" : "=v"(t1[j]) : "a"(a[h8 * 8 + 4 + j]));
          }
          if (WITH_BIAS) { t0 = t0 * ts + bct[NH * 2 + ni][h8 * 2]; t1 = t1 * ts + bct[NH * 2 + ni][h8 * 2 + 1]; }
          const bf16x8 v = {f2bf(t0[0]), f2bf(t0[1]), f2bf(t0[2]), f2bf(t0[3]), f2bf(t1[0]), f2bf(t1[1]), f2bf(t1[2]), f2bf(t1[3])};
          const int chunk = (ni * 32 + hh * 16 + h8 * 8) >> 3;
          *reinterpret_cast<bf16x8*>(sl + li * 128 + ((chunk ^ (li & 7)) << 4)) = v;
        }
      } else {
#pragma unroll
        for (int rg = 0; rg < 4; ++rg) {
          f32x4 t0;
#pragma unroll
          for (int j = 0; j < 4; ++j) asm volatile("v_accvgpr_read_b32 %0, %1" : "=v"(t0[j]) : "a"(a[rg * 4 + j]));
          const bf16x4 v = {f2bf(t0[0]), f2bf(t0[1]), f2bf(t0[2]), f2bf(t0[3])};
          const int col = ni * 32 + rg * 8 + hh * 4;
          *reinterpret_cast<bf16x4*>(sl + li * 128 + (((col >> 3) ^ (li & 7)) << 4) + (col & 7) * 2) = v;
        }
      }
#pragma unroll
      for (int r = 0; r < 16; ++r) a[r] = 0.f;
      __builtin_amdgcn_sched_barrier(0);
    }
  };
  const int rows_left = p.M - m0;
  const uint64_t wbytes = rows_left > 0 ? (uint64_t)rows_left * p.ldc * 2 : 0;
  const __amdgpu_buffer_rsrc_t rsC = ia_rsrc(reinterpret_cast<bf16*>(p.C) + (size_t)m0 * p.ldc, (uint32_t)(wbytes < 0x7FFFFFF0ull ? wbytes : 0x7FFFFFF0ull));
  const int ncol = n0 + c8 * 8;
  const uint32_t voffC = ncol < p.N ? (uint32_t)((rrow * p.ldc + ncol) * 2) : 0x80000000u;
  stage(0);
#pragma unroll
  for (int mi = 0; mi < 4; ++mi) {
    __builtin_amdgcn_wave_barrier();
    const char* const sl = stg + (mi & 1) * 4096;
    u32x4 v[4];
#pragma unroll
    for (int it = 0; it < 4; ++it) {
      const int row = it * 8 + rrow;
      v[it] = *reinterpret_cast<const u32x4*>(sl + row * 128 + ((c8 ^ (row & 7)) << 4));
    }
    __builtin_amdgcn_wave_barrier();
    if (mi < 3) stage(mi + 1);
#pragma unroll
    for (int it = 0; it < 4; ++it) {
      const uint32_t off = voffC + (uint32_t)((mi * 32 + it * 8) * p.ldc * 2);
      if (!IA_GEMM_DBG_HOOKS || !(p.dbg & 64)) __builtin_amdgcn_raw_buffer_store_b128(v[it], rsC, (int)off, 0, 0);
      else asm volatile("" : : "v"(v[it]));
    }
  }
}

template <int EPI, bool OUTF32, bool BKS, int NH>
IA_DEV void drain_half(const GemmArgs& p, f32x16 (&acc)[4][4], int m0, int n0, char* stg, int lane_e, bool full, bool bias_ready, f32x4 bias_lo,
                       f32x4 bias_hi) {
  const int hh = lane_e >> 5, li = lane_e & 31;
  const int rrow = lane_e >> 3, c8 = lane_e & 7;
  constexpr bool HAS_BIAS = EPI == EPI_BIAS || EPI == EPI_BIAS_GELU || EPI == EPI_BIAS_GELU_ACT || EPI == EPI_BIAS_ADD;
  constexpr bool HAS_AUX = EPI == EPI_ADD || EPI == EPI_BIAS_ADD || EPI == EPI_DGELU || EPI == EPI_DGELU_CS;
  constexpr int AHEAD = 4;
  auto drain = [&](auto PREFETCHED) {
    constexpr bool PRE = decltype(PREFETCHED)::value;
    f32x4 pb0, pb1;
    float cs[8];
    if (EPI == EPI_DGELU_CS) {
#pragma unroll
      for (int j = 0; j < 8; ++j) asm volatile("v_mov_b32 %0, 0" : "=v"(cs[j]));
    }
    bf16x8 ax[AHEAD + 1];
    constexpr bool BUF = PRE && !OUTF32;
    const auto window = [&](const void* base, int ld) {
      const uint64_t bytes = (uint64_t)(p.M - m0) * ld * 2;
      return ia_rsrc(reinterpret_cast<const bf16*>(base) + (size_t)m0 * ld, (uint32_t)(bytes < 0x7FFFFFF0ull ? bytes : 0x7FFFFFF0ull));
    };
    BufIO io{ia_rsrc(nullptr, 0), ia_rsrc(nullptr, 0), 0u};
    __amdgpu_buffer_rsrc_t rsAux = ia_rsrc(nullptr, 0);
    uint32_t voffC = 0, voffAux = 0;
    if (BUF) {
      io.rsC = window(p.C, p.ldc);
      if (EPI == EPI_BIAS_GELU) io.rsC2 = window(p.C2, p.ldc);
      voffC = (uint32_t)((rrow * p.ldc + n0 + c8 * 8) * 2);
      if (HAS_AUX) { rsAux = window(p.aux, p.ldaux); voffAux = (uint32_t)((rrow * p.ldaux + n0 + c8 * 8) * 2); }
    }
    auto aux_of = [&](int c) {
      const int row_in = (c >> 2) * 32 + ((c >> 1) & 1) * 16 + (c & 1) * 8;
      if (BUF) return __builtin_bit_cast(bf16x8, __builtin_amdgcn_raw_buffer_load_b128(rsAux, (int)(voffAux + (uint32_t)(row_in * p.ldaux * 2)), 0, 0));
      return *reinterpret_cast<const bf16x8*>(p.aux + (size_t)(m0 + row_in + rrow) * p.ldaux + n0 + c8 * 8);
    };
    if (PRE && HAS_BIAS) {
      if (bias_ready) { pb0 = bias_lo; pb1 = bias_hi; }
      else { pb0 = *reinterpret_cast<const f32x4*>(p.bias + n0 + c8 * 8); pb1 = *reinterpret_cast<const f32x4*>(p.bias + n0 + c8 * 8 + 4); }
    }
    if (PRE && HAS_AUX) {
#pragma unroll
      for (int c = 0; c < AHEAD; ++c) ax[c] = aux_of(c);
    }
    auto stage = [&](int mi) {
#pragma unroll
      for (int ni = 0; ni < 2; ++ni)
#pragma unroll
        for (int rg = 0; rg < 4; ++rg) {
          const int chunk = (ni * 32 + (BKS ? rg * 8 + hh * 4 : hh * 16 + rg * 4)) >> 2;
          f32x16& a = acc[mi][NH * 2 + ni];
          const f32x4 v = {a[rg * 4], a[rg * 4 + 1], a[rg * 4 + 2], a[rg * 4 + 3]};
          *reinterpret_cast<f32x4*>(stg + li * 256 + ((chunk ^ (li & 15)) << 4)) = v;
          a[rg * 4] = 0.f; a[rg * 4 + 1] = 0.f; a[rg * 4 + 2] = 0.f; a[rg * 4 + 3] = 0.f;
        }
    };
    stage(0);
#pragma unroll
    for (int mi = 0; mi < 4; ++mi) {
      __builtin_amdgcn_wave_barrier();
      f32x4 lo[4], hi[4];
#pragma unroll
      for (int it = 0; it < 4; ++it) {
        const int row = it * 8 + rrow;
        lo[it] = *reinterpret_cast<const f32x4*>(stg + row * 256 + (((2 * c8) ^ (row & 15)) << 4));
        hi[it] = *reinterpret_cast<const f32x4*>(stg + row * 256 + (((2 * c8 + 1) ^ (row & 15)) << 4));
      }
      asm volatile("s_waitcnt lgkmcnt(0)" : "+v"(lo[0]), "+v"(lo[1]), "+v"(lo[2]), "+v"(lo[3]), "+v"(hi[0]), "+v"(hi[1]), "+v"(hi[2]), "+v"(hi[3]));
      __builtin_amdgcn_wave_barrier();
      if (mi < 3) stage(mi + 1);
#pragma unroll
      for (int it = 0; it < 4; ++it) {
        const int row = it * 8 + rrow;
        const int m = m0 + mi * 32 + row, n = n0 + c8 * 8;
        const int c = mi * 4 + it;
        if (PRE) {
          if (HAS_AUX && c + AHEAD < 16) {
            ax[(c + AHEAD) % (AHEAD + 1)] = aux_of(c + AHEAD);
            asm volatile("" ::: "memory");
          }
          io.off = voffC + (uint32_t)((mi * 32 + it * 8) * p.ldc * 2);
          if (!(IA_DBG(p) & 64)) epi_store8<EPI, OUTF32, true, BUF>(p, m, n, lo[it], hi[it], pb0, pb1, ax[c % (AHEAD + 1)], cs, &io);
        } else {
          if (m < p.M && n < p.N && !(IA_DBG(p) & 64)) epi_store8<EPI, OUTF32, false>(p, m, n, lo[it], hi[it], pb0, pb1, ax[0], cs);
        }
        if (IA_DBG(p) & 64) asm volatile("" : : "v"(lo[it]), "v"(hi[it]));
      }
    }
    if (EPI == EPI_DGELU_CS) {
#pragma unroll
      for (int r = 0; r < 8; ++r) {
        float v = cs[r];
        v += __builtin_bit_cast(float, __builtin_amdgcn_update_dpp(__builtin_bit_cast(int, v), __builtin_bit_cast(int, v), 0x128, 0xF, 0xF, false));
        v = ia_add_xor32(ia_add_xor16(v));
        cs[r] = v;
      }
      if (rrow == 0 && n0 + c8 * 8 < p.N) {
        float* dst = p.csum_part + (size_t)(m0 >> 7) * p.N + n0 + c8 * 8;
        gstore16(dst, f32x4{cs[0], cs[1], cs[2], cs[3]});
        gstore16(dst + 4, f32x4{cs[4], cs[5], cs[6], cs[7]});
      }
    }
  };
  if (full && (HAS_BIAS || HAS_AUX) && !(IA_DBG(p) & 256)) drain(std::true_type{}); else drain(std::false_type{});
}

template <bool AKS, bool BKS, int EPI_, bool OUTF32>
__global__ __launch_bounds__(256) void gemm_kernel(GemmArgs p) {
  constexpr bool LIVE = EPI_ == EPI_NONE_LIVE;
  constexpr int EPI = LIVE ? (int)EPI_NONE : EPI_;
  static_assert(!LIVE || (AKS && BKS && OUTF32), "live k-tiles: the weight-gradient form only");
  extern __shared__ __attribute__((aligned(16))) char smem[];
  const int tid = threadIdx.x, lane0 = tid & 63;
  const int wave = __builtin_amdgcn_readfirstlane(tid >> 6);
  const int wm = wave >> 1, wn = wave & 1;
  const int nk_all = (p.K + BK - 1) / BK;
  const int total_tiles = p.tiles_m * p.tiles_n;
  int first_tile = blockIdx.x;
  bool ordered = false;
  p.split_id = 0;
  if (p.splits > 1) {
    const int w = xcd_chunk(blockIdx.x, gridDim.x);
    p.split_id = w / total_tiles;
    first_tile = w % total_tiles;
    ordered = true;
  }
  const int kt0 = p.split_id * p.nk_per_split;
  int n_tiles = min(nk_all, kt0 + p.nk_per_split) - kt0;
  uint32_t live_mv = 0u;
  if constexpr (LIVE) {
    const int nw = (nk_all + 31) >> 5, first = kt0 + 32 * lane0, wlo = first >> 5, sh = first & 31, left = n_tiles - 32 * lane0;
    const uint32_t lo = wlo < nw ? p.live_kt[wlo] : 0u, hi = wlo + 1 < nw ? p.live_kt[wlo + 1] : 0u;
    live_mv = sh ? (lo >> sh) | (hi << (32 - sh)) : lo;
    live_mv = left >= 32 ? live_mv : (left > 0 ? live_mv & ((1u << left) - 1u) : 0u);
    n_tiles = 0;
    for (uint64_t rest = __ballot(live_mv != 0u); rest; rest &= rest - 1ull)
      n_tiles += __builtin_popcount(__builtin_amdgcn_readlane(live_mv, __builtin_ctzll(rest)));
  }
  constexpr int PEND = 2 * (16 * epi_stores_per_call<EPI, OUTF32>() + epi_extra_stores<EPI>());
  auto coords = [&](int tile, int& bm, int& bn) {
    if (ordered) tile_of_order(p, tile, bm, bn); else tile_of_index(p, tile, total_tiles, bm, bn);
  };
  auto run = [&](int tile, bool prologue_only, f32x16 (&acc)[4][4], bool stores_in_flight) {
    int bm, bn;
    coords(tile, bm, bn);
    int lane = lane0;
    asm volatile("" : "+v"(lane));
    const uint64_t oa = (uint64_t)(AKS ? kt0 * BK : bm * BM) * p.lda, ob = (uint64_t)(BKS ? kt0 * BK : bn * BN) * p.ldb;
    constexpr bool PEEL_OK = !(EPI == EPI_BIAS && !OUTF32 && !BKS);
    main_loop<AKS, BKS, PEND, PEEL_OK, LIVE>(p, smem, acc, rsrc_at(p.A, p.a_bytes, oa), rsrc_at(p.B, p.b_bytes, ob), AKS ? bm * BM : 0, BKS ? bn * BN : 0, kt0,
                              AKS ? 0 : kt0, BKS ? 0 : kt0, n_tiles, nk_all, wm, wn, wave, lane, prologue_only, stores_in_flight, live_mv);
  };

  const bool dyn = p.tile_ctr != nullptr && !ordered;
  const int xcd = blockIdx.x & 7, q8 = total_tiles >> 3, r8 = total_tiles & 7;
  auto run_start = [&](int x) { return x < r8 ? x * (q8 + 1) : r8 * (q8 + 1) + (x - r8) * q8; };
  auto run_len = [&](int x) { return q8 + (x < r8 ? 1 : 0); };
  int* const mailbox = reinterpret_cast<int*>(smem + 2 * 2 * TILE_BYTES);
  uint32_t claimed = 0;
  auto claim_issue = [&]() {
    if (wave == 0 && lane0 == 0)
      {
        const uint64_t a64 = (uint64_t)(p.tile_ctr + xcd);
        const uint32_t alo = __builtin_amdgcn_readfirstlane((uint32_t)a64), ahi = __builtin_amdgcn_readfirstlane((uint32_t)(a64 >> 32));
        const uint64_t addr = ((uint64_t)ahi << 32) | alo;
        asm volatile("s_nop 4\n\tglobal_atomic_add %0, %1, %2, %3 sc0" : "=v"(claimed) : "v"(0u), "v"(1u), "s"(addr) : "memory");
      }
  };
  auto claim_resolve = [&]() -> int {
    asm volatile("s_waitcnt vmcnt(0)" : "+v"(claimed));
    if (wave == 0) {
      int pos = (int)__builtin_amdgcn_readfirstlane(claimed), w = -1;
      if (pos < run_len(xcd)) w = run_start(xcd) + pos;
      else {
        uint32_t seen = 0xFFFFFFFFu;
        if (lane0 < 8) seen = __hip_atomic_load(p.tile_ctr + lane0, __ATOMIC_RELAXED, __HIP_MEMORY_SCOPE_AGENT);
        const uint32_t mask = (uint32_t)__ballot((int)seen >= q8 + (lane0 < r8 ? 1 : 0)) | (1u << xcd);
        for (int d = 1; d < 8 && w < 0; ++d) {
          const int x = (xcd + d) & 7;
          if ((mask >> x) & 1u) continue;
          uint32_t got = 0;
          if (lane0 == 0) got = __hip_atomic_fetch_add(p.tile_ctr + x, 1u, __ATOMIC_RELAXED, __HIP_MEMORY_SCOPE_AGENT);
          pos = (int)__builtin_amdgcn_readfirstlane(got);
          if (pos < run_len(x)) w = run_start(x) + pos;
        }
      }
      if (lane0 == 0) *reinterpret_cast<volatile int*>(mailbox) = w;
    }
    __syncthreads();
    const int w = __builtin_amdgcn_readfirstlane(*reinterpret_cast<volatile int*>(mailbox));
    __syncthreads();
    return w;
  };
  auto leave = [&]() {
    asm volatile("s_waitcnt vmcnt(0)" : "+v"(claimed) : : "memory");
    if (dyn && wave == 0 && lane0 == 0) {
      const uint32_t d = __hip_atomic_fetch_add(p.tile_ctr + 8, 1u, __ATOMIC_RELAXED, __HIP_MEMORY_SCOPE_AGENT);
      if (d == gridDim.x - 1) {
#pragma unroll
        for (int i = 0; i < 9; ++i) __hip_atomic_store(p.tile_ctr + i, 0u, __ATOMIC_RELAXED, __HIP_MEMORY_SCOPE_AGENT);
      }
    }
  };
  if (dyn) {
    ordered = true;
    claim_issue();
    first_tile = claim_resolve();
    if (first_tile < 0) { leave(); return; }
    claim_issue();
  }

  f32x16 acc[4][4];
#pragma unroll
  for (int i = 0; i < 4; ++i)
#pragma unroll
    for (int j = 0; j < 4; ++j)
#pragma unroll
      for (int r = 0; r < 16; ++r) acc[i][j][r] = 0.f;
  int tile = first_tile;
  run(tile, true, acc, false);
  bool stores_in_flight = false;
  constexpr bool HAS_BIAS_K = EPI == EPI_BIAS || EPI == EPI_BIAS_GELU || EPI == EPI_BIAS_GELU_ACT || EPI == EPI_BIAS_ADD;
  while (true) {
    int bm, bn;
    coords(tile, bm, bn);
    const int m0_pre = bm * BM + wm * 128, n0_pre = bn * BN + wn * 128;
    const bool full = m0_pre + 128 <= p.M && n0_pre + 128 <= p.N;
    constexpr bool BIAS_CT = EPI == EPI_BIAS && !OUTF32 && !BKS;
    f32x4 pbv[4] = {};
    f32x4 bct[4][4] = {};
    int lane_b = lane0;
    asm volatile("" : "+v"(lane_b));
    const bool bias_pre = HAS_BIAS_K && full;
    if (bias_pre && BIAS_CT) {
      const float* bp = p.bias + n0_pre + (lane_b >> 5) * 16;
#pragma unroll
      for (int ni = 0; ni < 4; ++ni)
#pragma unroll
        for (int q = 0; q < 4; ++q) bct[ni][q] = *reinterpret_cast<const f32x4*>(bp + ni * 32 + q * 4);
    } else if (bias_pre) {
      const float* bp = p.bias + n0_pre + (lane_b & 7) * 8;
      pbv[0] = *reinterpret_cast<const f32x4*>(bp); pbv[1] = *reinterpret_cast<const f32x4*>(bp + 4);
      pbv[2] = *reinterpret_cast<const f32x4*>(bp + 64); pbv[3] = *reinterpret_cast<const f32x4*>(bp + 68);
    }
    run(tile, false, acc, stores_in_flight);
    float ts = 1.f;
    if (bias_pre && BIAS_CT) {
#pragma unroll
      for (int ni = 0; ni < 4; ++ni)
        asm volatile("s_waitcnt vmcnt(0)" : "+v"(bct[ni][0]), "+v"(bct[ni][1]), "+v"(bct[ni][2]), "+v"(bct[ni][3]));
      if (n0_pre < p.qcols) {
        ts = p.qscale;
#pragma unroll
        for (int ni = 0; ni < 4; ++ni)
#pragma unroll
          for (int q = 0; q < 4; ++q) bct[ni][q] *= ts;
      }
    } else if (bias_pre) asm volatile("s_waitcnt vmcnt(0)" : "+v"(pbv[0]), "+v"(pbv[1]), "+v"(pbv[2]), "+v"(pbv[3]));
    int next = ordered ? total_tiles : tile + gridDim.x;
    if (dyn) {
      next = claim_resolve();
      claim_issue();
      if (next < 0) next = total_tiles;
    }
    if (next < total_tiles) run(next, true, acc, false);

    int lane_e = lane0;
    asm volatile("" : "+v"(lane_e));
    int m0 = m0_pre, n0 = n0_pre;
    asm volatile("" : "+s"(m0), "+s"(n0));
    char* stg = smem + 2 * 2 * TILE_BYTES + wave * 2 * STAGE_BYTES;
    if (!(IA_DBG(p) & 32)) {
      if constexpr (EPI == EPI_NONE && !OUTF32) {
        drain_half_plain<BKS, 0, false>(p, acc, m0, n0, stg, lane_e, bct);
        drain_half_plain<BKS, 1, false>(p, acc, m0, n0 + 64, stg, lane_e, bct);
      } else if (BIAS_CT && bias_pre) {
        drain_half_plain<false, 0, BIAS_CT>(p, acc, m0, n0, stg, lane_e, bct, ts);
        drain_half_plain<false, 1, BIAS_CT>(p, acc, m0, n0 + 64, stg, lane_e, bct, ts);
      } else {
        drain_half<EPI, OUTF32, BKS, 0>(p, acc, m0, n0, stg, lane_e, full || (m0 + 128 <= p.M && n0 + 64 <= p.N), bias_pre, pbv[0], pbv[1]);
        drain_half<EPI, OUTF32, BKS, 1>(p, acc, m0, n0 + 64, stg, lane_e, full, bias_pre, pbv[2], pbv[3]);
      }
    }
    if (next >= total_tiles) break;
    stores_in_flight = !(IA_DBG(p) & 96) && full;
    if (!stores_in_flight) asm volatile("s_waitcnt vmcnt(0)" ::: "memory");
    tile = next;
  }
  leave();
}

}



namespace t256la {
using namespace t256w;

__global__ __launch_bounds__(256) void gemm_kernel(GemmArgs p) {
  extern __shared__ __attribute__((aligned(16))) char smem[];
  const int tid = threadIdx.x, lane0 = tid & 63;
  const int wave = __builtin_amdgcn_readfirstlane(tid >> 6);
  const int wm = wave >> 1, wn = wave & 1;
  const int nk_all = (p.K + BK - 1) / BK;
  const int total_tiles = p.tiles_m * p.tiles_n;
  const int n_tiles = nk_all;
  auto coords = [&](int tile, int& bm, int& bn) { tile_of_index(p, tile, total_tiles, bm, bn); };
  auto window_a = [&](int tile) {
    int bm = 0, bn = 0;
    if (tile < total_tiles) coords(tile, bm, bn);
    return tile < total_tiles ? rsrc_at(p.A, p.a_bytes, (uint64_t)bm * BM * p.lda) : ia_rsrc(p.A, 0u);
  };
  auto window_b = [&](int tile) {
    int bm = 0, bn = 0;
    if (tile < total_tiles) coords(tile, bm, bn);
    return tile < total_tiles ? rsrc_at(p.B, p.b_bytes, (uint64_t)bn * BN * p.ldb) : ia_rsrc(p.B, 0u);
  };

  int lane = lane0;
  asm volatile("" : "+v"(lane));
  const int li = lane & 31;
  const int gt = wave * 64 + lane;
  const int rowd = gt >> 3;
  const uint32_t voffA = (uint32_t)((rowd * p.lda + (((gt & 7) ^ ((rowd >> 1) & 7)) * 8)) * 2), stepA = (uint32_t)(32 * p.lda * 2);
  const uint32_t voffB = (uint32_t)((rowd * p.ldb + (((gt & 7) ^ ((rowd >> 1) & 7)) * 8)) * 2), stepB = (uint32_t)(32 * p.ldb * 2);
  const int kl = ((gt & 7) ^ (((gt >> 3) >> 1) & 7)) * 8;
  char* const my_part = smem + wave * 1024;
  const int nperm = ((li >> 2) & 1) * 16 + (li >> 3) * 4 + (li & 3);
  uint32_t baseA[4], baseB[4];
  const uint32_t smem_addr = ia_lds_addr(smem);
  frag_bases<false>(baseA, smem_addr, wm * 128, lane, li);
  frag_bases<false>(baseB, smem_addr + TILE_BYTES, wn * 128, lane, nperm);

  int tile = blockIdx.x;
  __amdgpu_buffer_rsrc_t rsA = window_a(tile), rsB = window_b(tile);
  __amdgpu_buffer_rsrc_t rsAn = window_a(tile + (int)gridDim.x), rsBn = window_b(tile + (int)gridDim.x);

  auto off_of = [&](int v) -> uint32_t {
    const int kt = v >= n_tiles ? v - n_tiles : v;
    return kl < p.K - kt * BK ? 1u : 0u;
  };
  auto dma = [&](int v, int i, uint32_t ok, uint32_t buf) {
    const bool isB = i >= 8, nx = v >= n_tiles;
    const int j = i & 7, kt = nx ? v - n_tiles : v;
    char* dst = my_part + (isB ? TILE_BYTES : 0) + buf + j * 4096;
    const uint32_t soff = (uint32_t)kt * (uint32_t)(BK * 2) + (uint32_t)j * (isB ? stepB : stepA);
    const uint32_t off = ok ? (isB ? voffB : voffA) : OOB;
    __builtin_amdgcn_raw_ptr_buffer_load_lds(isB ? (nx ? rsBn : rsB) : (nx ? rsAn : rsA), IA_LDS(dst), 16, off, (int)soff, 0, 0);
  };

#pragma unroll
  for (int i = 0; i < 16; ++i) dma(0, i, off_of(0), 0u);
#pragma unroll
  for (int i = 0; i < 16; ++i) dma(1, i, off_of(1), (uint32_t)(2 * TILE_BYTES));
  asm volatile("s_waitcnt vmcnt(0)" ::: "memory");
  __builtin_amdgcn_s_barrier();
  Op<false> a0, a1, a2, a3, b0, b1, b2, b3;
#pragma unroll
  for (int j = 0; j < 4; ++j) read_frag<0>(a0, j, baseA, 0u);
#pragma unroll
  for (int j = 0; j < 4; ++j) read_frag<0>(b0, j, baseB, 0u);
  uint32_t bo = 0;

  f32x16 acc[4][4];
#pragma unroll
  for (int i = 0; i < 4; ++i)
#pragma unroll
    for (int j = 0; j < 4; ++j)
#pragma unroll
      for (int r = 0; r < 16; ++r) acc[i][j][r] = 0.f;

  using Acc = std::false_type;

  const f32x4 no_bias[4][4] = {};
  while (true) {
    int bm, bn;
    coords(tile, bm, bn);
    const int m0_pre = bm * BM + wm * 128, n0_pre = bn * BN + wn * 128;
    int u = 0;
    uint32_t okA = 0u, okB = off_of(1);
    auto trip = [&](auto FIRST_T) {
      constexpr bool FIRST = decltype(FIRST_T)::value;
      const uint32_t bn_ = bo ^ (uint32_t)(2 * TILE_BYTES);
      tie2<0>(a0, b0);
      mfma_step<FIRST>(acc, a0, b0, [&](int i) {
        if (i < 4) { read_frag<1>(a1, i, baseA, bo); read_frag<1>(b1, i, baseB, bo); }
        else if (i < 8) { read_frag<2>(a2, i - 4, baseA, bo); read_frag<2>(b2, i - 4, baseB, bo); }
        else if (i < 12) { read_frag<3>(a3, i - 8, baseA, bo); read_frag<3>(b3, i - 8, baseB, bo); }
        if (!FIRST && i % 4 == 3) dma(u + 1, 12 + i / 4, okB, bn_);
        if (i == 12) okA = off_of(u + 2);
      });
      tie6<0>(a1, b1, a2, b2, a3, b3);
      __builtin_amdgcn_sched_barrier(0);
      __builtin_amdgcn_s_barrier();
      __builtin_amdgcn_sched_barrier(0);
      mfma_step<false>(acc, a1, b1, [&](int i) {
        if (i % 4 == 1) dma(u + 2, i / 4, okA, bo);
      });
      mfma_step<false>(acc, a2, b2, [&](int i) {
        if (i % 4 == 1) dma(u + 2, 4 + i / 4, okA, bo);
        if (i == 14) okB = off_of(u + 2);
      });
      if constexpr (FIRST) asm volatile("s_waitcnt vmcnt(40)" ::: "memory");
      else asm volatile("s_waitcnt vmcnt(8)" ::: "memory");
      __builtin_amdgcn_sched_barrier(0);
      __builtin_amdgcn_s_barrier();
      __builtin_amdgcn_sched_barrier(0);
      mfma_step<false>(acc, a3, b3, [&](int i) {
        if (i < 4) read_frag<0>(a0, i, baseA, bn_);
        else if (i < 8) read_frag<0>(b0, i - 4, baseB, bn_);
        if (i % 4 == 3) dma(u + 2, 8 + i / 4, okB, bo);
      });
      bo = bn_;
      ++u;
    };
    trip(std::true_type{});
    do { trip(Acc{}); } while (u < n_tiles);
    {
      const uint32_t ok1 = off_of(n_tiles + 1), b1_ = bo ^ (uint32_t)(2 * TILE_BYTES);
#pragma unroll
      for (int i = 12; i < 16; ++i) dma(n_tiles + 1, i, ok1, b1_);
    }

    int lane_e = lane0;
    asm volatile("" : "+v"(lane_e));
    int m0 = m0_pre, n0 = n0_pre;
    asm volatile("" : "+s"(m0), "+s"(n0));
    char* stg = smem + 2 * 2 * TILE_BYTES + wave * 2 * STAGE_BYTES;
    drain_half_plain<false, 0, false>(p, acc, m0, n0, stg, lane_e, no_bias);
    drain_half_plain<false, 1, false>(p, acc, m0, n0 + 64, stg, lane_e, no_bias);
    tile += (int)gridDim.x;
    if (tile >= total_tiles) break;
    rsA = rsAn; rsB = rsBn;
    rsAn = window_a(tile + (int)gridDim.x); rsBn = window_b(tile + (int)gridDim.x);
  }
  tie2<0>(a0, b0);
  asm volatile("s_waitcnt vmcnt(0)" ::: "memory");
}
}

struct GemmProf {
  bool on = false;
  int variant = -1, n = 0, cap = 0;
  double flops = 0.0, bytes = 0.0;
  hipEvent_t* ev = nullptr;
};
GemmProf g_prof;

IA_DEV void fold_row_sums(const float* rsum_ws, float* rsum_out, int M, int splits) {
  __shared__ float rs[256];
  if (!rsum_ws || (int)blockIdx.x * 32 >= M) return;
  const int lane = threadIdx.x & 7, m = blockIdx.x * 32 + (threadIdx.x >> 3);
  float a = 0.f;
  if (m < M)
    for (int sp = lane; sp < splits; sp += 8) a += rsum_ws[((size_t)blockIdx.y * splits + sp) * M + m];
  rs[threadIdx.x] = a;
  __syncthreads();
  if (lane == 0 && m < M) {
    float sum = rs[threadIdx.x];
#pragma unroll
    for (int l = 1; l < 8; ++l) sum += rs[threadIdx.x + l];
    rsum_out[(size_t)blockIdx.y * M + m] += sum;
  }
  __syncthreads();
}

__global__ __launch_bounds__(256) void splitk_reduce_kernel(const float* __restrict__ ws, float* __restrict__ C, int M, int N, int ldc,
                                                            int splits, int accumulate, long gc, const float* rsum_ws, float* rsum_out) {
  fold_row_sums(rsum_ws, rsum_out, M, splits);
  ws += (size_t)blockIdx.y * splits * M * N;
  C += (size_t)blockIdx.y * gc;
  const size_t total4 = (size_t)M * N / 4;
  for (size_t t = (size_t)blockIdx.x * 256 + threadIdx.x; t < total4; t += (size_t)gridDim.x * 256) {
    const size_t e = t * 4;
    const int m = (int)(e / N), n = (int)(e % N);
    f32x4 acc = *reinterpret_cast<const f32x4*>(ws + e);
    for (int s = 1; s < splits; ++s) acc += *reinterpret_cast<const f32x4*>(ws + (size_t)s * M * N + e);
    float* c = C + (size_t)m * ldc + n;
    if (accumulate) acc += *reinterpret_cast<const f32x4*>(c);
    *reinterpret_cast<f32x4*>(c) = acc;
  }
}

__global__ __launch_bounds__(256) void splitk_reduce_deep_kernel(const float* __restrict__ ws, float* __restrict__ C, int M, int N, int ldc,
                                                                 int splits, int accumulate, long gc, const float* rsum_ws, float* rsum_out) {
  __shared__ f32x4 red[256];
  fold_row_sums(rsum_ws, rsum_out, M, splits);
  ws += (size_t)blockIdx.y * splits * M * N;
  C += (size_t)blockIdx.y * gc;
  const size_t total4 = (size_t)M * N / 4;
  const int lane = threadIdx.x & 7;
  const size_t t = (size_t)blockIdx.x * 32 + (threadIdx.x >> 3);
  f32x4 acc = {0.f, 0.f, 0.f, 0.f};
  if (t < total4)
    for (int sp = lane; sp < splits; sp += 8) acc += *reinterpret_cast<const f32x4*>(ws + (size_t)sp * M * N + t * 4);
  red[threadIdx.x] = acc;
  __syncthreads();
  if (lane == 0 && t < total4) {
    f32x4 sum = red[threadIdx.x];
#pragma unroll
    for (int l = 1; l < 8; ++l) sum += red[threadIdx.x + l];
    const size_t e = t * 4;
    float* c = C + (size_t)(e / N) * ldc + (e % N);
    if (accumulate) sum += *reinterpret_cast<const f32x4*>(c);
    *reinterpret_cast<f32x4*>(c) = sum;
  }
}

struct Plan { bool big; int splits; };

Plan make_plan(int M, int N, int K, bool f32_out, int groups = 1) {
  Plan pl;
  const int nk = (K + BK - 1) / BK;
  const long t256n = (long)((M + 255) / 256) * ((N + 255) / 256);
  const int smax = f32_out ? (nk / 8 > 32 ? 32 : (nk / 8 < 1 ? 1 : nk / 8)) : 1;
  pl.big = M >= 256 && N >= 256 && (N & 7) == 0 && t256n * smax >= 160;
  if (groups > 1) pl.big = false;
  const long tiles = pl.big ? t256n : (long)((M + 127) / 128) * ((N + 127) / 128) * groups;
  const long slots = pl.big ? 256 : 512;
  int smax2 = smax;
  if (f32_out && slots / tiles > smax2) { smax2 = (int)(slots / tiles); if (smax2 > nk / 8) smax2 = nk / 8 < 1 ? 1 : nk / 8; if (smax2 < smax) smax2 = smax; }
  const double reduce_per_split = (double)tiles * (pl.big ? 0.0244 : 0.0061);
  int best = 1;
  double best_cost = 1e30;
  for (int s = 1; s <= smax2; ++s) {
    const long rounds = (tiles * s + slots - 1) / slots;
    const double cost = (double)rounds * ((nk + s - 1) / s + 6) + (s > 1 ? s * reduce_per_split : 0.0);
    if (cost < best_cost - 1e-9) { best_cost = cost; best = s; }
  }
  pl.splits = best;
  return pl;
}

int g_dynamic = -1;
constexpr int MAX_DEVICES = 16;
uint32_t* g_ctr_base[MAX_DEVICES] = {};
std::atomic<unsigned> g_launch_seq{0};
uint32_t* next_ctr_slot() {
  if (g_dynamic < 0) {
    const char* e = getenv("IA_GEMM_DYNAMIC");
    g_dynamic = e ? atoi(e) : 0;
  }
  if (!g_dynamic) return nullptr;
  int dev = 0;
  if (hipGetDevice(&dev) != hipSuccess || dev < 0 || dev >= MAX_DEVICES) return nullptr;
  uint32_t* base = __atomic_load_n(&g_ctr_base[dev], __ATOMIC_ACQUIRE);
  if (!base) {
    if (hipGetSymbolAddress((void**)&base, HIP_SYMBOL(g_tile_ctr)) != hipSuccess || !base) return nullptr;
    __atomic_store_n(&g_ctr_base[dev], base, __ATOMIC_RELEASE);
  }
  return base + (size_t)(g_launch_seq.fetch_add(1u, std::memory_order_relaxed) % CTR_SLOTS) * CTR_WORDS;
}

template <bool AKS, bool BKS, int EPI, bool OUTF32>
int launch(GemmArgs a, bool big, hipStream_t st) {
  constexpr int vid = AKS * 1000 + BKS * 100 + EPI * 10 + (OUTF32 ? 1 : 0);
  constexpr bool WGRAD = AKS && BKS && EPI == EPI_NONE && OUTF32;
  const bool rec = g_prof.on && g_prof.variant == vid && g_prof.n < g_prof.cap && !(WGRAD && a.live_kt);
  if (rec) (void)hipEventRecord(g_prof.ev[2 * g_prof.n], st);
  if (big) {
    a.tiles_m = (a.M + t256w::BM - 1) / t256w::BM; a.tiles_n = (a.N + t256w::BN - 1) / t256w::BN;
    const int ntile = a.tiles_m * a.tiles_n;
    const int gx = a.splits > 1 ? ntile * a.splits : (ntile < 256 ? ntile : 256);
    a.tile_ctr = (a.splits == 1 && ntile > gx) ? next_ctr_slot() : nullptr;
    void (*kern)(GemmArgs) = t256w::gemm_kernel<AKS, BKS, EPI, OUTF32>;
    static bool attr_set[3] = {false, false, false};
    int la = 0;
    if constexpr (WGRAD) {
      if (a.live_kt) { kern = t256w::gemm_kernel<true, true, EPI_NONE_LIVE, true>; la = 2; }
    }
    if constexpr (!AKS && !BKS && EPI == EPI_NONE && !OUTF32) {
      const char* e = getenv("IA_GEMM_LA");
      if ((e ? atoi(e) : 1) && a.splits == 1 && ntile > gx && !a.tile_ctr && a.K >= 2 * BK && !(IA_DBG(a))) { kern = t256la::gemm_kernel; la = 1; }
    }
    if (!attr_set[la]) {
      if (hipFuncSetAttribute((const void*)kern, hipFuncAttributeMaxDynamicSharedMemorySize, t256w::LDS_BYTES) != hipSuccess) return IA_ERR_LAUNCH;
      attr_set[la] = true;
    }
    hipLaunchKernelGGL(kern, dim3(gx), dim3(256), t256w::LDS_BYTES, st, a);
  } else {
    a.tiles_m = (a.M + t128::BM - 1) / t128::BM; a.tiles_n = (a.N + t128::BN - 1) / t128::BN;
    hipLaunchKernelGGL((t128::gemm_kernel<AKS, BKS, EPI, OUTF32>), dim3(a.tiles_m * a.tiles_n * a.splits * a.groups), dim3(256), 0, st, a);
  }
  if (OUTF32 && a.splits > 16) {
    size_t g = ((size_t)a.M * a.N / 4 + 31) / 32;
    if (a.rsum_out && g < (size_t)(a.M + 31) / 32) g = (size_t)(a.M + 31) / 32;
    hipLaunchKernelGGL(splitk_reduce_deep_kernel, dim3((unsigned)g, a.groups), dim3(256), 0, st, a.ws, (float*)a.C, a.M, a.N, a.ldc, a.splits,
                       a.accumulate, a.gc, a.rsum_out ? a.rsum_ws : nullptr, a.rsum_out);
  } else if (OUTF32 && a.splits > 1) {
    size_t g = ((size_t)a.M * a.N / 4 + 255) / 256; if (g > 4096) g = 4096;
    if (a.rsum_out && g < (size_t)(a.M + 31) / 32) g = (size_t)(a.M + 31) / 32;
    hipLaunchKernelGGL(splitk_reduce_kernel, dim3((int)g, a.groups), dim3(256), 0, st, a.ws, (float*)a.C, a.M, a.N, a.ldc, a.splits, a.accumulate,
                       a.gc, a.rsum_out ? a.rsum_ws : nullptr, a.rsum_out);
  }
  if (rec) {
    (void)hipEventRecord(g_prof.ev[2 * g_prof.n + 1], st);
    g_prof.flops += 2.0 * a.M * a.N * a.K;
    g_prof.bytes += 2.0 * ((double)a.M * a.K + (double)a.N * a.K) + (OUTF32 ? 4.0 : 2.0) * a.M * a.N;
    ++g_prof.n;
  }
  return ia_check_launch();
}

}

extern "C" size_t ia_gemm_workspace_bytes(int M, int N, int K, int c_is_f32) {
  if (!c_is_f32 || M <= 0 || N <= 0 || K <= 0) return 0;
  const Plan pl = make_plan(M, N, K, true);
  return pl.splits > 1 ? (size_t)pl.splits * M * (N + 1) * sizeof(float) : 0;
}

static int gemm_core(const void* A, int a_kstrided, int lda, const void* B, int b_kstrided, int ldb, void* C, int c_is_f32, int ldc, int M,
                     int N, int K, int epilogue, const float* bias, const void* aux, int ldaux, void* C2, int accumulate, void* workspace,
                     size_t workspace_bytes, const IaViewGemm* view, hipStream_t stream, int qcols = 0, float qscale = 1.f,
                     const uint32_t* live_kt = nullptr);

extern "C" size_t ia_gemm_colsum_workspace_bytes(int M, int N) {
  if (M <= 0 || N <= 0) return 0;
  const size_t fused = (size_t)((M + 255) / 256) * 2 * N * sizeof(float), plain = ia_colsum_workspace_bytes(M, N);
  return fused > plain ? fused : plain;
}

extern "C" int ia_gemm_bf16(const void* A, int a_kstrided, int lda, const void* B, int b_kstrided, int ldb,
                            void* C, int c_is_f32, int ldc, int M, int N, int K, int epilogue,
                            const float* bias, const void* aux, int ldaux, void* C2, int accumulate, void* workspace,
                            size_t workspace_bytes, hipStream_t stream) {
  return gemm_core(A, a_kstrided, lda, B, b_kstrided, ldb, C, c_is_f32, ldc, M, N, K, epilogue, bias, aux, ldaux, C2, accumulate, workspace,
                   workspace_bytes, nullptr, stream);
}

extern "C" int ia_gemm_bf16_qscale(const void* A, int lda, const void* B, int ldb, void* C, int ldc, int M, int N, int K, const float* bias,
                                   int scaled_cols, float col_scale, hipStream_t stream) {
  return gemm_core(A, 0, lda, B, 0, ldb, C, 0, ldc, M, N, K, EPI_BIAS, bias, nullptr, 0, nullptr, 0, nullptr, 0, nullptr, stream, scaled_cols,
                   col_scale);
}

static __host__ __device__ inline uint32_t ktile_live(const uint8_t* row_live, int M, int t) {
  const uint8_t* r = row_live + (size_t)t * BK;
  const int n = M - t * BK < BK ? M - t * BK : BK;
  uint64_t any = 0;
  if (n == BK && ((uintptr_t)r & 7) == 0) {
    for (int i = 0; i < BK / 8; ++i) any |= reinterpret_cast<const uint64_t*>(r)[i];
  } else {
    for (int i = 0; i < n; ++i) any |= r[i];
  }
  return any != 0 ? 1u : 0u;
}
namespace {
__global__ __launch_bounds__(256) void ktile_mask_kernel(const uint8_t* __restrict__ row_live, int M, int nk, uint32_t* __restrict__ mask) {
  const int t = blockIdx.x * 256 + threadIdx.x;
  const uint64_t b = __ballot(t < nk && ktile_live(row_live, M, t));
  if ((threadIdx.x & 31) == 0 && t < nk) mask[t >> 5] = (uint32_t)(b >> (threadIdx.x & 32));
}
inline size_t al256(size_t b) { return (b + 255) & ~(size_t)255; }
}

extern "C" size_t ia_ktile_mask_bytes(int M_rows) {
  if (M_rows <= 0) return 0;
  return (size_t)(((M_rows + BK - 1) / BK + 31) / 32) * sizeof(uint32_t);
}
extern "C" int ia_ktile_mask(const uint8_t* row_live, int M_rows, uint32_t* mask, hipStream_t stream) {
  (void)hipGetLastError();
  if (!row_live || !mask || M_rows <= 0) return IA_ERR_ARG;
  const int nk = (M_rows + BK - 1) / BK;
  hipLaunchKernelGGL(ktile_mask_kernel, dim3((nk + 255) / 256), dim3(256), 0, stream, row_live, M_rows, nk, mask);
  return ia_check_launch();
}
extern "C" int ia_ktile_mask_host(const uint8_t* row_live, int M_rows, uint32_t* mask) {
  if (!row_live || !mask || M_rows <= 0) return IA_ERR_ARG;
  const int nk = (M_rows + BK - 1) / BK;
  for (int w = 0; w < (nk + 31) / 32; ++w) mask[w] = 0u;
  for (int t = 0; t < nk; ++t) mask[t >> 5] |= ktile_live(row_live, M_rows, t) << (t & 31);
  return IA_OK;
}
int ia_gemm_wgrad_masked(const void* dY, int ldy, const void* X, int ldx, float* dW, int ldw, int N_out, int N_in, int M_rows,
                         const uint32_t* ktile_mask, int accumulate, void* workspace, size_t workspace_bytes, hipStream_t stream) {
  return gemm_core(dY, 1, ldy, X, 1, ldx, dW, 1, ldw, N_out, N_in, M_rows, EPI_NONE, nullptr, nullptr, 0, nullptr, accumulate, workspace,
                   workspace_bytes, nullptr, stream, 0, 1.f, ktile_mask);
}
extern "C" size_t ia_gemm_wgrad_rows_workspace_bytes(int N_out, int N_in, int M_rows) {
  if (N_out <= 0 || N_in <= 0 || M_rows <= 0) return 0;
  return al256(ia_gemm_workspace_bytes(N_out, N_in, M_rows, 1)) + ia_ktile_mask_bytes(M_rows);
}
extern "C" int ia_gemm_wgrad_rows_filters(int N_out, int N_in, int M_rows) {
  if (N_out <= 0 || N_in <= 0 || M_rows <= 0) return 0;
  const Plan pl = make_plan(N_out, N_in, M_rows, true);
  const int nk = (M_rows + BK - 1) / BK;
  return pl.big && (nk + pl.splits - 1) / pl.splits <= t256w::LIVE_MAX_KTILES ? 1 : 0;
}
extern "C" int ia_gemm_wgrad_rows(const void* dY, int ldy, const void* X, int ldx, float* dW, int ldw, int N_out, int N_in, int M_rows,
                                  const uint8_t* row_live, int accumulate, void* workspace, size_t workspace_bytes, hipStream_t stream) {
  if (!row_live)
    return gemm_core(dY, 1, ldy, X, 1, ldx, dW, 1, ldw, N_out, N_in, M_rows, EPI_NONE, nullptr, nullptr, 0, nullptr, accumulate, workspace,
                     workspace_bytes, nullptr, stream);
  if (N_out <= 0 || N_in <= 0 || M_rows <= 0) return IA_ERR_ARG;
  const size_t split_bytes = al256(ia_gemm_workspace_bytes(N_out, N_in, M_rows, 1));
  if (!workspace || workspace_bytes < split_bytes + ia_ktile_mask_bytes(M_rows) || ((uintptr_t)workspace & 15)) return IA_ERR_WORKSPACE;
  uint32_t* mask = reinterpret_cast<uint32_t*>((char*)workspace + split_bytes);
  int rc = ia_ktile_mask(row_live, M_rows, mask, stream);
  return rc ? rc : ia_gemm_wgrad_masked(dY, ldy, X, ldx, dW, ldw, N_out, N_in, M_rows, mask, accumulate, workspace, split_bytes, stream);
}

int ia_gemm_view(const IaViewGemm& v, hipStream_t stream) {
  if ((v.a_view && (v.a_kstrided || (v.a_view != 1 && v.a_view != -1))) || (v.b_view && (!v.b_kstrided || v.b_view < 1 || v.b_view > 2)) ||
      v.pw <= 2 || (!v.a_view && !v.b_view) || v.groups < 1 || v.lca < 3 || v.lcbk < 3 || v.lcbn < 3)
    return IA_ERR_ARG;
  return gemm_core(v.A, v.a_kstrided, v.lda, v.B, v.b_kstrided, v.ldb, v.C, v.c_is_f32, v.ldc, v.M, v.N, v.K, v.bias ? EPI_BIAS : EPI_NONE,
                   v.bias, nullptr, 0, v.rsum_out, 0, v.workspace, v.workspace_bytes, &v, stream);
}

size_t ia_gemm_view_workspace_bytes(int M, int N, int K, int groups) {
  if (M <= 0 || N <= 0 || K <= 0 || groups <= 0) return 0;
  const Plan pl = make_plan(M, N, K, true, groups);
  return pl.splits > 1 ? (size_t)groups * pl.splits * M * (N + 1) * sizeof(float) : 0;
}

template <bool BKS>
static int launch_dgelu_colsum(GemmArgs& g, bool big, float* csum, void* workspace, size_t workspace_bytes, hipStream_t stream) {
  if (!csum || !workspace || workspace_bytes < ia_gemm_colsum_workspace_bytes(g.M, g.N) || g.ldc != g.N) return IA_ERR_WORKSPACE;
  if (!big) {
    int rc = launch<false, BKS, EPI_DGELU, false>(g, false, stream);
    return rc ? rc : ia_colsum(g.C, g.ldc, g.M, g.N, csum, 1, workspace, workspace_bytes, stream);
  }
  g.csum_part = (float*)workspace;
  int rc = launch<false, BKS, EPI_DGELU_CS, false>(g, true, stream);
  return rc ? rc : ia_sum_rows_f32((const float*)workspace, ((g.M + 255) / 256) * 2, g.N, csum, 1, stream);
}

static int gemm_core(const void* A, int a_kstrided, int lda, const void* B, int b_kstrided, int ldb, void* C, int c_is_f32, int ldc, int M,
                     int N, int K, int epilogue, const float* bias, const void* aux, int ldaux, void* C2, int accumulate, void* workspace,
                     size_t workspace_bytes, const IaViewGemm* view, hipStream_t stream, int qcols, float qscale, const uint32_t* live_kt) {
  const uint64_t a_window = view ? view->a_window : 0, b_window = view ? view->b_window : 0;
  const int groups = view ? view->groups : 1;
  (void)hipGetLastError();
  if (!A || !B || !C || M <= 0 || N <= 0 || K <= 0) return IA_ERR_ARG;
  if ((lda & 7) || (ldb & 7) || (ldc & 3) || (N & 3)) return IA_ERR_ARG;
  if (((uintptr_t)A & 15) || ((uintptr_t)B & 15) || ((uintptr_t)C & 15)) return IA_ERR_ARG;
  GemmArgs g;
  g.A = (const bf16*)A; g.B = (const bf16*)B; g.C = C; g.C2 = (bf16*)C2; g.bias = bias; g.aux = (const bf16*)aux;
  g.M = M; g.N = N; g.K = K; g.lda = lda; g.ldb = ldb; g.ldc = ldc; g.ldaux = ldaux; g.accumulate = accumulate;
  if (qcols < 0 || qcols > N || (qcols & 127) || (qcols && (epilogue != EPI_BIAS || c_is_f32 || a_kstrided || b_kstrided))) return IA_ERR_ARG;
  g.qcols = qcols; g.qscale = qscale;
  const uint64_t ab = a_window ? a_window : (a_kstrided ? ((uint64_t)(K - 1) * lda + M) * 2 : ((uint64_t)(M - 1) * lda + K) * 2);
  const uint64_t bb = b_window ? b_window : (b_kstrided ? ((uint64_t)(K - 1) * ldb + N) * 2 : ((uint64_t)(N - 1) * ldb + K) * 2);
  g.csum_part = nullptr; g.split_id = 0; g.tile_ctr = nullptr;
  g.a_view = g.b_view = g.pw = 0; g.lca = g.lcbk = g.lcbn = 6;
  g.groups = 1; g.ga = g.gb = g.gc = g.gbias = 0;
  if (view) {
    g.a_view = view->a_view; g.b_view = view->b_view; g.pw = view->pw; g.lca = view->lca; g.lcbk = view->lcbk; g.lcbn = view->lcbn;
    g.groups = groups; g.ga = view->ga; g.gb = view->gb; g.gc = view->gc; g.gbias = view->gbias;
  }
  if (!a_kstrided && (K & 7)) return IA_ERR_ARG;
  g.a_bytes = ab; g.b_bytes = bb;
  g.tiles_m = g.tiles_n = 0;
  { static int dbg = -1; if (dbg < 0) { const char* e = getenv("IA_GEMM_DBG"); dbg = e ? atoi(e) : 0; } g.dbg = dbg; }
  const int nk = (K + BK - 1) / BK;
  Plan pl = make_plan(M, N, K, c_is_f32 != 0, groups);
  g.splits = 1; g.nk_per_split = nk; g.ws = nullptr;
  const bool big = pl.big && !view && !(g.dbg & 128);
  const bool wgrad_form = a_kstrided && b_kstrided && c_is_f32 && epilogue == EPI_NONE;
  g.rsum_out = (wgrad_form && !big) ? (float*)C2 : nullptr;
  g.rsum_ws = nullptr;
  if (c_is_f32 && epilogue == EPI_NONE && pl.splits > 1 && workspace &&
      workspace_bytes >= (size_t)groups * pl.splits * M * (N + (g.rsum_out ? 1 : 0)) * sizeof(float)) {
    g.nk_per_split = (nk + pl.splits - 1) / pl.splits;
    g.splits = (nk + g.nk_per_split - 1) / g.nk_per_split;
    g.ws = (float*)workspace;
    g.rsum_ws = g.ws + (size_t)groups * g.splits * M * N;
  }
  {
    const uint64_t margin = view ? 2 * (uint64_t)(view->pw + 1) : 0, slab = (uint64_t)g.nk_per_split * BK + margin, tile = 256 + margin;
    const uint64_t wa = (a_kstrided ? slab : tile) * (uint64_t)lda * 2 + (a_kstrided ? 0 : (uint64_t)K * 2);
    const uint64_t wb = (b_kstrided ? slab : tile) * (uint64_t)ldb * 2 + (b_kstrided ? 0 : (uint64_t)K * 2);
    if (wa >= 0x7FFFFFF0ull || wb >= 0x7FFFFFF0ull) return IA_ERR_ARG;
  }
  if (a_kstrided && b_kstrided && c_is_f32 && epilogue == EPI_NONE) g.live_kt = (big && g.nk_per_split <= t256w::LIVE_MAX_KTILES) ? live_kt : nullptr;
  const bool needs_bias = epilogue == EPI_BIAS || epilogue == EPI_BIAS_GELU || epilogue == EPI_BIAS_GELU_ACT || epilogue == EPI_BIAS_ADD;
  const bool needs_aux = epilogue == EPI_ADD || epilogue == EPI_DGELU || epilogue == EPI_BIAS_ADD || epilogue == EPI_DGELU_CS;
  if (needs_bias && !bias) return IA_ERR_ARG;
  if (needs_aux && (!aux || (ldaux & 3))) return IA_ERR_ARG;
  if (epilogue == EPI_BIAS_GELU && !C2) return IA_ERR_ARG;

  if (!a_kstrided && !b_kstrided && !c_is_f32) {
    switch (epilogue) {
      case EPI_NONE: return launch<false, false, EPI_NONE, false>(g, big, stream);
      case EPI_BIAS: return launch<false, false, EPI_BIAS, false>(g, big, stream);
      case EPI_BIAS_GELU: return launch<false, false, EPI_BIAS_GELU, false>(g, big, stream);
      case EPI_BIAS_GELU_ACT: return launch<false, false, EPI_BIAS_GELU_ACT, false>(g, big, stream);
      case EPI_BIAS_ADD: return launch<false, false, EPI_BIAS_ADD, false>(g, big, stream);
      case EPI_ADD: return launch<false, false, EPI_ADD, false>(g, big, stream);
      case EPI_DGELU: return launch<false, false, EPI_DGELU, false>(g, big, stream);
      case EPI_DGELU_CS: return launch_dgelu_colsum<false>(g, big, (float*)C2, workspace, workspace_bytes, stream);
    }
  } else if (!a_kstrided && b_kstrided && !c_is_f32) {
    switch (epilogue) {
      case EPI_NONE: return launch<false, true, EPI_NONE, false>(g, big, stream);
      case EPI_ADD: return launch<false, true, EPI_ADD, false>(g, big, stream);
      case EPI_DGELU: return launch<false, true, EPI_DGELU, false>(g, big, stream);
      case EPI_DGELU_CS: return launch_dgelu_colsum<true>(g, big, (float*)C2, workspace, workspace_bytes, stream);
    }
  } else if (a_kstrided && b_kstrided && c_is_f32) {
    if (epilogue == EPI_NONE) {
      int rc = launch<true, true, EPI_NONE, true>(g, big, stream);
      if (!rc && C2 && big) rc = ia_colsum(A, lda, K, M, (float*)C2, 1, workspace, workspace_bytes, stream);
      return rc;
    }
  } else if (!a_kstrided && !b_kstrided && c_is_f32) {
    if (epilogue == EPI_NONE) return launch<false, false, EPI_NONE, true>(g, big, stream);
    if (epilogue == EPI_BIAS) return launch<false, false, EPI_BIAS, true>(g, big, stream);
  }
  return IA_ERR_UNSUPPORTED;
}

extern "C" int ia_prof_begin(int variant, int max_launches) {
  (void)hipGetLastError();
  if (max_launches <= 0) return IA_ERR_ARG;
  if (g_prof.cap < max_launches) {
    for (int i = 0; i < 2 * g_prof.cap; ++i) (void)hipEventDestroy(g_prof.ev[i]);
    delete[] g_prof.ev;
    g_prof.ev = new hipEvent_t[2 * max_launches];
    for (int i = 0; i < 2 * max_launches; ++i)
      if (hipEventCreate(&g_prof.ev[i]) != hipSuccess) return IA_ERR_LAUNCH;
    g_prof.cap = max_launches;
  }
  g_prof.variant = variant; g_prof.n = 0; g_prof.flops = 0.0; g_prof.bytes = 0.0; g_prof.on = true;
  return IA_OK;
}

extern "C" int ia_prof_end(double* total_ms, double* total_flops, int* launches) {
  (void)hipGetLastError();
  g_prof.on = false;
  double ms = 0.0;
  for (int i = 0; i < g_prof.n; ++i) {
    if (hipEventSynchronize(g_prof.ev[2 * i + 1]) != hipSuccess) return IA_ERR_LAUNCH;
    float t = 0.f;
    if (hipEventElapsedTime(&t, g_prof.ev[2 * i], g_prof.ev[2 * i + 1]) != hipSuccess) return IA_ERR_LAUNCH;
    ms += t;
  }
  if (total_ms) *total_ms = ms;
  if (total_flops) *total_flops = g_prof.flops;
  if (launches) *launches = g_prof.n;
  return IA_OK;
}

namespace {
__global__ __launch_bounds__(256) void cu_hog_kernel(unsigned long long ticks) {
  extern __shared__ __attribute__((aligned(16))) char hog_smem[];
  if (threadIdx.x == 0) *reinterpret_cast<volatile int*>(hog_smem) = 1;
  const unsigned long long t0 = wall_clock64();
  while (wall_clock64() - t0 < ticks) __builtin_amdgcn_s_sleep(32);
}
}
extern "C" int ia_debug_gemm_dynamic(int on) {
  if (g_dynamic < 0) (void)next_ctr_slot();
  const int prev = g_dynamic;
  if (on >= 0) g_dynamic = on ? 1 : 0;
  return prev;
}
extern "C" int ia_debug_cu_hog(int workgroups, float milliseconds, hipStream_t stream) {
// ... 13 lines not shown
```

item_alignment_amd/ops.py:

```python
import torch

from . import _lib
from ._lib import check, ptr, stream_ptr

EPI_NONE, EPI_BIAS, EPI_BIAS_GELU, EPI_ADD, EPI_DGELU, EPI_BIAS_ADD, EPI_DGELU_COLSUM = 0, 1, 2, 3, 4, 5, 6
ACT_NONE, ACT_TANH = 0, 1
BF16, F32 = torch.bfloat16, torch.float32


def _need(t, dtype, name):
    if t is None:
        return
    if not t.is_cuda:
        raise _lib.ItemAlignError(f"{name} must live on the GPU (the HIP path has no CPU fallback)")
    if t.dtype != dtype:
        raise TypeError(f"{name}: expected {dtype}, got {t.dtype}")
    if not t.is_contiguous():
        raise ValueError(f"{name} must be contiguous")


def gemm(a, b, *, a_kstrided=False, b_kstrided=False, epilogue=EPI_NONE, bias=None, aux=None, out=None, out_f32=False,
         accumulate=False, pre_out=None, colsum_out=None):
    lib = _lib.load()
    _need(a, BF16, "a"); _need(b, BF16, "b"); _need(bias, F32, "bias"); _need(aux, BF16, "aux")
    if a_kstrided:
        K, M = a.shape
    else:
        M, K = a.shape
    if b_kstrided:
        Kb, N = b.shape
    else:
        N, Kb = b.shape
    if K != Kb:
        raise ValueError(f"gemm: inner dims differ ({K} vs {Kb})")
    if out is None:
        out = torch.empty((M, N), device=a.device, dtype=F32 if out_f32 else BF16)
    _need(out, F32 if out_f32 else BF16, "out")
    if epilogue == EPI_BIAS_GELU and pre_out is None:
        pre_out = torch.empty((M, N), device=a.device, dtype=BF16)
    ws_bytes = lib.ia_gemm_workspace_bytes(M, N, K, int(out_f32))
    if epilogue == EPI_DGELU_COLSUM:
        _need(colsum_out, F32, "colsum_out")
        if colsum_out is None:
            raise ValueError("gemm: EPI_DGELU_COLSUM needs colsum_out")
        pre_out = colsum_out
        ws_bytes = max(ws_bytes, lib.ia_gemm_colsum_workspace_bytes(M, N))
    ws = torch.empty(ws_bytes, device=a.device, dtype=torch.uint8) if ws_bytes else None
    check(lib.ia_gemm_bf16(a.data_ptr(), int(a_kstrided), a.shape[1], b.data_ptr(), int(b_kstrided), b.shape[1], out.data_ptr(),
                           int(out_f32), N, M, N, K, epilogue, ptr(bias), ptr(aux), N if aux is not None else 0, ptr(pre_out),
                           int(accumulate), ptr(ws), ws_bytes, stream_ptr()), "ia_gemm_bf16")
    if epilogue == EPI_BIAS_GELU:
        return out, pre_out
    return out


def ktile_mask(row_live):
    lib = _lib.load()
    _need(row_live, torch.uint8, "row_live")
    M = row_live.numel()
    out = torch.empty(lib.ia_ktile_mask_bytes(M) // 4, device=row_live.device, dtype=torch.int32)
    check(lib.ia_ktile_mask(row_live.data_ptr(), M, out.data_ptr(), stream_ptr()), "ia_ktile_mask")
    return out


def gemm_wgrad_rows(dy, x, row_live=None, *, out=None, accumulate=False):
    lib = _lib.load()
    _need(dy, BF16, "dy"); _need(x, BF16, "x"); _need(row_live, torch.uint8, "row_live")
    (M, n_out), (Mx, n_in) = dy.shape, x.shape
    if M != Mx or (row_live is not None and row_live.numel() != M):
        raise ValueError("gemm_wgrad_rows: dy, x and row_live must have the same number of rows")
    if out is None:
        out = torch.empty((n_out, n_in), device=dy.device, dtype=F32)
    _need(out, F32, "out")
    ws_bytes = lib.ia_gemm_wgrad_rows_workspace_bytes(n_out, n_in, M)
    ws = torch.empty(ws_bytes, device=dy.device, dtype=torch.uint8)
    check(lib.ia_gemm_wgrad_rows(dy.data_ptr(), n_out, x.data_ptr(), n_in, out.data_ptr(), n_in, n_out, n_in, M, ptr(row_live),
                                 int(accumulate), ws.data_ptr(), ws_bytes, stream_ptr()), "ia_gemm_wgrad_rows")
    return out


def ln_fwd(x, gamma, beta, eps, *, bias=None, residual=None, write_z=True, drop_p=0.0, seed=0, stream_id=0):
    lib = _lib.load()
    _need(x, BF16, "x"); _need(gamma, F32, "gamma"); _need(beta, F32, "beta"); _need(bias, F32, "bias"); _need(residual, BF16, "residual")
    M, H = x.shape
    y = torch.empty_like(x)
    z = torch.empty_like(x) if write_z else None
    mean = torch.empty(M, device=x.device, dtype=F32)
    rstd = torch.empty(M, device=x.device, dtype=F32)
    check(lib.ia_ln_fwd(x.data_ptr(), ptr(bias), ptr(residual), ptr(z), y.data_ptr(), mean.data_ptr(), rstd.data_ptr(),
                        gamma.data_ptr(), ptr(beta), M, H, eps, drop_p, seed, stream_id, stream_ptr()), "ia_ln_fwd")
    return y, z, mean, rstd


def ln_bwd(dy, z, mean, rstd, gamma, *, dres=None, dgamma=None, dbeta=None, dbias=None, drop_p=0.0, seed=0, stream_id=0):
    lib = _lib.load()
    _need(dy, BF16, "dy"); _need(z, BF16, "z"); _need(dres, BF16, "dres")
    M, H = dy.shape
    dz = torch.empty_like(dy)
    dx = torch.empty_like(dy) if drop_p > 0 else None
    ws_bytes = lib.ia_ln_bwd_workspace_bytes(M, H)
    ws = torch.empty(ws_bytes, device=dy.device, dtype=torch.uint8)
    check(lib.ia_ln_bwd(dy.data_ptr(), ptr(dres), z.data_ptr(), mean.data_ptr(), rstd.data_ptr(), gamma.data_ptr(), dz.data_ptr(),
                        ptr(dx), ptr(dgamma), ptr(dbeta), ptr(dbias), M, H, drop_p, seed, stream_id, ws.data_ptr(), ws_bytes, 1,
                        stream_ptr()), "ia_ln_bwd")
    return dz, dx


def colsum(x, out, accumulate=True):
    lib = _lib.load()
    _need(x, BF16, "x"); _need(out, F32, "out")
    M, N = x.shape
    ws_bytes = lib.ia_colsum_workspace_bytes(M, N)
    ws = torch.empty(ws_bytes, device=x.device, dtype=torch.uint8)
    check(lib.ia_colsum(x.data_ptr(), N, M, N, out.data_ptr(), int(accumulate), ws.data_ptr(), ws_bytes, stream_ptr()), "ia_colsum")
    return out


def gemm_qscale(a, b, bias, scaled_cols, col_scale):
    lib = _lib.load()
    _need(a, BF16, "a"); _need(b, BF16, "b"); _need(bias, F32, "bias")
    M, K = a.shape
    N = b.shape[0]
    out = torch.empty((M, N), device=a.device, dtype=BF16)
    check(lib.ia_gemm_bf16_qscale(a.data_ptr(), K, b.data_ptr(), K, out.data_ptr(), N, M, N, K, bias.data_ptr(), scaled_cols, col_scale,
                                  stream_ptr()), "ia_gemm_bf16_qscale")
    return out


def attn_fwd(qkv, B, L, nh, *, key_mask=None, scale=0.125, drop_p=0.0, seed=0, q_prescaled=False):
    lib = _lib.load()
    _need(qkv, BF16, "qkv"); _need(key_mask, torch.uint8, "key_mask")
    H = nh * 64
    out = torch.empty((B * L, H), device=qkv.device, dtype=BF16)
    lse = torch.empty((B, nh, L), device=qkv.device, dtype=F32)
    base = qkv.data_ptr()
    fn = lib.ia_attn_fwd_ps if q_prescaled else lib.ia_attn_fwd
    check(fn(base, base + 2 * H, base + 4 * H, 3 * H, ptr(key_mask), out.data_ptr(), H, lse.data_ptr(), B, nh, L, scale, drop_p, seed,
             stream_ptr()), "ia_attn_fwd")
    return out, lse


def attn_bwd(qkv, ctx, d_ctx, lse, B, L, nh, *, key_mask=None, scale=0.125, drop_p=0.0, seed=0, dbias=None, q_prescaled=False, return_delta=False,
             masked_rows_dead=False):
    lib = _lib.load()
    _need(qkv, BF16, "qkv"); _need(ctx, BF16, "ctx"); _need(d_ctx, BF16, "d_ctx"); _need(lse, F32, "lse")
    H = nh * 64
    dqkv = torch.empty_like(qkv)
    delta = torch.empty((B, nh, L), device=qkv.device, dtype=F32)
    base, dbase = qkv.data_ptr(), dqkv.data_ptr()
    if (q_prescaled or masked_rows_dead) and dbias is None:
        dbias = torch.zeros(3 * H, device=qkv.device, dtype=F32)
    if masked_rows_dead:
        ws = torch.empty(lib.ia_attn_bwd_bias_workspace_bytes(B, nh, L), device=qkv.device, dtype=torch.uint8)
        check(lib.ia_attn_bwd_bias_ex((1 if q_prescaled else 0) | 2, base, base + 2 * H, base + 4 * H, 3 * H, ptr(key_mask), ctx.data_ptr(),
                                      d_ctx.data_ptr(), H, lse.data_ptr(), delta.data_ptr(), dbase, dbase + 2 * H, dbase + 4 * H, 3 * H,
                                      dbias.data_ptr(), ws.data_ptr(), ws.numel(), B, nh, L, scale, drop_p, seed, stream_ptr()), "ia_attn_bwd_bias_ex")
        return (dqkv, delta) if return_delta else dqkv
    if dbias is not None:
        _need(dbias, F32, "dbias")
        ws = torch.empty(lib.ia_attn_bwd_bias_workspace_bytes(B, nh, L), device=qkv.device, dtype=torch.uint8)
        fn = lib.ia_attn_bwd_bias_ps if q_prescaled else lib.ia_attn_bwd_bias
        check(fn(base, base + 2 * H, base + 4 * H, 3 * H, ptr(key_mask), ctx.data_ptr(), d_ctx.data_ptr(), H, lse.data_ptr(),
                                   delta.data_ptr(), dbase, dbase + 2 * H, dbase + 4 * H, 3 * H, dbias.data_ptr(), ws.data_ptr(), ws.numel(),
# ... 88 lines not shown
```

Measured before the change: 622.7.

## Skip dead padded row blocks in dgrad GEMMs via compacted live row-block lists

Adds a row-block compaction kernel that lists the live 32-row blocks of the key mask, and a ROWS variant of the GEMM main loop and epilogues that gathers A rows and scatters output rows through that list. The post-LN backward dgrad GEMMs for fc1, out-proj and qkv use it when masked rows are dead, so tiles made only of padding are not computed. This costs an extra small launch per layer, scalar loads of block indices, and more complex epilogue addressing. Dead output rows must be zero-filled or otherwise handled consistently.

```diff
diff --git a/include/itemalign.h b/include/itemalign.h
--- a/include/itemalign.h
+++ b/include/itemalign.h
@@ -16,7 +16,7 @@
 #define IA_ERR_UNSUPPORTED (-4)
 
 const char* ia_strerror(int code);
-#define IA_ABI_VERSION 17
+#define IA_ABI_VERSION 18
 int ia_abi_version(void);
 
 #define IA_EPI_NONE 0
@@ -41,6 +41,15 @@
 size_t ia_ktile_mask_bytes(int M_rows);
 int ia_ktile_mask(const uint8_t* row_live, int M_rows, uint32_t* mask, ia_stream_t stream);
 int ia_ktile_mask_host(const uint8_t* row_live, int M_rows, uint32_t* mask);
+size_t ia_gemm_dgrad_rows_workspace_bytes(int M_rows, int N_in, int K_out);
+int ia_gemm_dgrad_rows_filters(int M_rows, int N_in, int K_out);
+int ia_gemm_dgrad_rows(const void* dY, int ldy, const void* W, int w_kstrided, int ldw, void* dX, int ldx, int M_rows, int N_in, int K_out,
+                       int epilogue, const void* aux, int ldaux, void* C2, const uint8_t* row_live, void* workspace, size_t workspace_bytes,
+                       ia_stream_t stream);
+size_t ia_row_blocks_bytes(int M_rows);
+int ia_row_blocks(const uint8_t* row_live, int M_rows, int* list, ia_stream_t stream);
+int ia_row_blocks_host(const uint8_t* row_live, int M_rows, int* list);
+int ia_debug_dgrad_rows(int on);
 
 int ia_prof_begin(int variant, int max_launches);
 int ia_prof_end(double* total_ms, double* total_flops, int* launches);
diff --git a/item_alignment_amd/_lib.py b/item_alignment_amd/_lib.py
--- a/item_alignment_amd/_lib.py
+++ b/item_alignment_amd/_lib.py
@@ -36,6 +36,13 @@
     "ia_ktile_mask_bytes": (sz, [i32]),
     "ia_ktile_mask": (i32, [vp, i32, vp, vp]),
     "ia_ktile_mask_host": (i32, [vp, i32, vp]),
+    "ia_gemm_dgrad_rows_workspace_bytes": (sz, [i32, i32, i32]),
+    "ia_gemm_dgrad_rows_filters": (i32, [i32, i32, i32]),
+    "ia_gemm_dgrad_rows": (i32, [vp, i32, vp, i32, i32, vp, i32, i32, i32, i32, i32, vp, i32, vp, vp, vp, sz, vp]),
+    "ia_row_blocks_bytes": (sz, [i32]),
+    "ia_row_blocks": (i32, [vp, i32, vp, vp]),
+    "ia_row_blocks_host": (i32, [vp, i32, vp]),
+    "ia_debug_dgrad_rows": (i32, [i32]),
     "ia_prof_begin": (i32, [i32, i32]),
     "ia_prof_end": (i32, [C.POINTER(C.c_double), C.POINTER(C.c_double), C.POINTER(i32)]),
     "ia_prof_bytes": (C.c_double, []),
@@ -185,7 +192,7 @@
 _lib = None
 
 
-ABI_VERSION = 17
+ABI_VERSION = 18
 
 
 class ItemAlignError(RuntimeError):
diff --git a/item_alignment_amd/csrc/common.h b/item_alignment_amd/csrc/common.h
--- a/item_alignment_amd/csrc/common.h
+++ b/item_alignment_amd/csrc/common.h
@@ -161,3 +161,8 @@
 __attribute__((visibility("hidden"))) int ia_gemm_wgrad_masked(const void* dY, int ldy, const void* X, int ldx, float* dW, int ldw, int N_out,
                                                                int N_in, int M_rows, const uint32_t* ktile_mask, int accumulate,
                                                                void* workspace, size_t workspace_bytes, hipStream_t stream);
+
+__attribute__((visibility("hidden"))) int ia_gemm_dgrad_blocks(const void* dY, int ldy, const void* W, int w_kstrided, int ldw, void* dX, int ldx,
+                                                               int M_rows, int N_in, int K_out, int epilogue, const void* aux, int ldaux, void* C2,
+                                                               const int* row_blocks, void* workspace, size_t workspace_bytes,
+                                                               hipStream_t stream);
diff --git a/item_alignment_amd/csrc/engine.hip b/item_alignment_amd/csrc/engine.hip
--- a/item_alignment_amd/csrc/engine.hip
+++ b/item_alignment_amd/csrc/engine.hip
@@ -58,7 +58,7 @@
 }
 
 struct Scratch {
-  char* g0; char* g1; char* g2; char* gI; char* gqkv; float* delta; char* ws; size_t ws_bytes; char* gws; size_t gws_bytes; uint32_t* live_kt; size_t bytes;
+  char* g0; char* g1; char* g2; char* gI; char* gqkv; float* delta; char* ws; size_t ws_bytes; char* gws; size_t gws_bytes; uint32_t* live_kt; int* row_blk; size_t bytes;
 };
 
 size_t max3(size_t a, size_t b, size_t c) { return a > b ? (a > c ? a : c) : (b > c ? b : c); }
@@ -77,6 +77,7 @@
                      max3(ia_gemm_workspace_bytes((int)H, (int)I, (int)M, 1), ia_gemm_workspace_bytes((int)H, (int)H, (int)M, 1), 0));
   s.gws = a.take(s.gws_bytes);
   s.live_kt = (uint32_t*)a.take(ia_ktile_mask_bytes((int)M));
+  s.row_blk = (int*)a.take(ia_row_blocks_bytes((int)M));
   s.bytes = a.bytes;
   return s;
 }
@@ -86,10 +87,15 @@
   return c && c->B > 0 && c->L > 0 && c->H > 0 && c->I > 0 && c->nh > 0 && c->H == c->nh * 64 && (c->H & 7) == 0 && (c->I & 7) == 0;
 }
 
+int g_dgrad_rows = 1;
+
 #define IA_TRY(expr) do { int rc_ = (expr); if (rc_) return rc_; } while (0)
 
 int dgrad(const void* dy, int k_out, const void* w, const void* wt, int n_in, void* dx, int M, int epilogue, const void* aux, int ldaux, void* c2,
-          void* ws, size_t ws_bytes, ia_stream_t st) {
+          void* ws, size_t ws_bytes, ia_stream_t st, const int* row_blk = nullptr) {
+  if (row_blk)
+    return ia_gemm_dgrad_blocks(dy, k_out, wt ? wt : w, wt ? 0 : 1, wt ? k_out : n_in, dx, n_in, M, n_in, k_out, epilogue, aux, ldaux, c2, row_blk,
+                                ws, ws_bytes, st);
   if (wt)
     return ia_gemm_bf16(dy, 0, k_out, wt, 0, k_out, dx, 0, n_in, M, n_in, k_out, epilogue, nullptr, aux, ldaux, c2, 0, ws, ws_bytes, st);
   return ia_gemm_bf16(dy, 0, k_out, w, 1, n_in, dx, 0, n_in, M, n_in, k_out, epilogue, nullptr, aux, ldaux, c2, 0, ws, ws_bytes, st);
@@ -163,6 +169,12 @@
 
 }
 
+extern "C" int ia_debug_dgrad_rows(int on) {
+  const int was = g_dgrad_rows;
+  g_dgrad_rows = on ? 1 : 0;
+  return was;
+}
+
 extern "C" size_t ia_layer_stash_bytes(const ia_layer_cfg* cfg) {
   (void)hipGetLastError();
   if (!cfg_ok(cfg)) return 0;
@@ -224,26 +236,28 @@
   if (!c->pre_ln) {
     const uint8_t* const live = (c->masked_rows_dead && !c->cu_seqlens) ? key_mask : nullptr;
     const uint32_t* const live_kt = live ? k.live_kt : nullptr;
+    const int* const row_blk = (live && g_dgrad_rows) ? k.row_blk : nullptr;
     if (live) IA_TRY(ia_ktile_mask(live, M, k.live_kt, st));
+    if (row_blk) IA_TRY(ia_row_blocks(live, M, k.row_blk, st));
     IA_TRY(ia_ln_bwd2_rows(dy, dy2, nullptr, s.ffn, s.mean2, s.rstd2, w->ln2_g, k.g0, drop ? k.g1 : nullptr, g->ln2_g, g->ln2_b, g->b_fc2, M, H,
                            c->hidden_drop, c->seed, c->layer_id * 4u + 1u, live, k.ws, k.ws_bytes, 1, st));
     const char* d_ffn = drop ? k.g1 : k.g0;
     IA_TRY(wgrad(d_ffn, H, s.hact, I, (float*)g->w_fc2, M, live_kt, k.gws, k.gws_bytes, st));
     IA_TRY(dgrad(d_ffn, H, w->w_fc2, w->wt_fc2, I, k.gI, M, IA_EPI_DGELU_COLSUM, s.hpre, I, g->b_fc1, k.ws, k.ws_bytes, st));
     IA_TRY(wgrad(k.gI, I, s.ln, H, (float*)g->w_fc1, M, live_kt, k.gws, k.gws_bytes, st));
-    IA_TRY(dgrad(k.gI, I, w->w_fc1, w->wt_fc1, H, k.g2, M, IA_EPI_NONE, nullptr, 0, nullptr, nullptr, 0, st));
+    IA_TRY(dgrad(k.gI, I, w->w_fc1, w->wt_fc1, H, k.g2, M, IA_EPI_NONE, nullptr, 0, nullptr, nullptr, 0, st, row_blk));
     char* dz1buf = dx2 ? (char*)dx2 : k.g0;
     IA_TRY(ia_ln_bwd2_rows(k.g2, k.g0, nullptr, s.proj, s.mean1, s.rstd1, w->ln1_g, dz1buf, drop ? k.g1 : nullptr, g->ln1_g, g->ln1_b, g->b_o, M, H,
                            c->hidden_drop, c->seed, c->layer_id * 4u + 0u, live, k.ws, k.ws_bytes, 1, st));
     const char* d_att = drop ? k.g1 : dz1buf;
     IA_TRY(wgrad(d_att, H, s.ctx, H, (float*)g->w_o, M, live_kt, k.gws, k.gws_bytes, st));
-    IA_TRY(dgrad(d_att, H, w->w_o, w->wt_o, H, k.g2, M, IA_EPI_NONE, nullptr, 0, nullptr, nullptr, 0, st));
+    IA_TRY(dgrad(d_att, H, w->w_o, w->wt_o, H, k.g2, M, IA_EPI_NONE, nullptr, 0, nullptr, nullptr, 0, st, row_blk));
     IA_TRY(attn_bwd(c, s.qkv, key_mask, s.ctx, k.g2, s.lse, k.delta, k.gqkv, g->b_qkv, k.ws, k.ws_bytes, scale, c->attn_drop, attn_seed, st));
     IA_TRY(wgrad(k.gqkv, 3 * H, x, H, (float*)g->w_qkv, M, live_kt, k.gws, k.gws_bytes, st));
     if (dx2)
-      IA_TRY(dgrad(k.gqkv, 3 * H, w->w_qkv, w->wt_qkv, H, dx, M, IA_EPI_NONE, nullptr, 0, nullptr, nullptr, 0, st));
+      IA_TRY(dgrad(k.gqkv, 3 * H, w->w_qkv, w->wt_qkv, H, dx, M, IA_EPI_NONE, nullptr, 0, nullptr, nullptr, 0, st, row_blk));
     else
-      IA_TRY(dgrad(k.gqkv, 3 * H, w->w_qkv, w->wt_qkv, H, dx, M, IA_EPI_ADD, dz1buf, H, nullptr, nullptr, 0, st));
+      IA_TRY(dgrad(k.gqkv, 3 * H, w->w_qkv, w->wt_qkv, H, dx, M, IA_EPI_ADD, dz1buf, H, nullptr, nullptr, 0, st, row_blk));
   } else {
     if (!c->dy_colsum_done) IA_TRY(ia_colsum(dy, H, M, H, g->b_fc2, 1, k.ws, k.ws_bytes, st));
     IA_TRY(ia_gemm_bf16(dy, 1, H, s.hact, 1, I, g->w_fc2, 1, I, H, I, M, IA_EPI_NONE, nullptr, nullptr, 0, nullptr, 1, k.gws, k.gws_bytes, st));
diff --git a/item_alignment_amd/csrc/gemm.hip b/item_alignment_amd/csrc/gemm.hip
--- a/item_alignment_amd/csrc/gemm.hip
+++ b/item_alignment_amd/csrc/gemm.hip
@@ -15,12 +15,14 @@
 
 enum { EPI_NONE = 0, EPI_BIAS = 1, EPI_BIAS_GELU = 2, EPI_ADD = 3, EPI_DGELU = 4, EPI_BIAS_ADD = 5, EPI_DGELU_CS = 6, EPI_BIAS_GELU_ACT = 7 };
 constexpr int EPI_NONE_LIVE = 8;
+constexpr int EPI_ROWS = 16;
 
 struct GemmArgs {
   const bf16* A; const bf16* B; void* C; bf16* C2;
   union {
     const float* bias;
     const uint32_t* live_kt;
+    const int* row_blk;
   };
   const bf16* aux;
   int M, N, K;
@@ -564,6 +566,23 @@
     }
 }
 
+struct Blk8 { int b[8]; };
+struct RowOff { uint32_t o[8]; };
+struct RowBlk { int r[4]; };
+constexpr int ROW_BLK_HDR = 8;
+IA_DEV Blk8 load_blk8(const int* list, int bm, int n_live) {
+  typedef int i32x8 __attribute__((ext_vector_type(8)));
+  const uint64_t a64 = (uint64_t)(list + ROW_BLK_HDR + bm * 8);
+  const uint32_t alo = __builtin_amdgcn_readfirstlane((uint32_t)a64), ahi = __builtin_amdgcn_readfirstlane((uint32_t)(a64 >> 32));
+  const uint64_t addr = ((uint64_t)ahi << 32) | alo;
+  i32x8 v;
+  asm volatile("s_nop 4\n\ts_load_dwordx8 %0, %1, 0x0\n\ts_waitcnt lgkmcnt(0)" : "=&s"(v) : "s"(addr) : "memory");
+  Blk8 r;
+#pragma unroll
+  for (int j = 0; j < 8; ++j) r.b[j] = bm * 8 + j < n_live ? v[j] : -1;
+  return r;
+}
+
 struct LiveWalk {
   uint64_t rest;
   uint32_t w;
@@ -581,10 +600,11 @@
   return idx;
 }
 
-template <bool AKS, bool BKS, int PEND, bool PEEL_OK = true, bool LIVE = false>
+template <bool AKS, bool BKS, int PEND, bool PEEL_OK = true, bool LIVE = false, bool ROWS = false>
 IA_DEV void main_loop(const GemmArgs& p, char* smem, f32x16 (&acc)[4][4], __amdgpu_buffer_rsrc_t rsA, __amdgpu_buffer_rsrc_t rsB, int xa, int xb,
                       int kt0, int ktaA0, int ktaB0, int n_tiles, int nk_all, int wm, int wn, int wave, int lane, bool prologue_only,
-                      bool stores_in_flight, uint32_t live_mv = 0u) {
+                      bool stores_in_flight, uint32_t live_mv = 0u, RowOff ro = RowOff{}) {
+  static_assert(!ROWS || !AKS, "the row remap moves the pieces of a k-contiguous A");
   static_assert(!LIVE || (AKS && BKS), "the live-k-tile walk advances the running lane offsets of two k-strided operands");
   constexpr bool ROUND = !AKS && !BKS;
   const int li = lane & 31;
@@ -611,7 +631,7 @@
     const int kt = kt0 + u;
     const int kta = (dbg & 4) ? 0 : (isB ? ktaB0 : ktaA0) + (LIVE ? (u == 0 ? live0 : live1) : u);
     const bool ks = isB ? BKS : AKS;
-    const uint32_t soff = (uint32_t)kta * (isB ? kstepB : kstepA) + (uint32_t)j * (isB ? stepB : stepA);
+    const uint32_t soff = (uint32_t)kta * (isB ? kstepB : kstepA) + ((ROWS && !isB) ? ro.o[j] : (uint32_t)j * (isB ? stepB : stepA));
     if (ks) {
       const uint32_t off = (dma_on && (!LIVE || u < n_tiles)) ? (isB ? voffB : voffA) + soff : OOB;
       __builtin_amdgcn_raw_ptr_buffer_load_lds(isB ? rsB : rsA, IA_LDS(dst), 16, off, 0, 0, 0);
@@ -631,7 +651,7 @@
     const int j = i & 7;
     char* dst = my_part + (isB ? TILE_BYTES : 0) + (u & 1) * 2 * TILE_BYTES + j * 4096;
     const int kta = (dbg & 4) ? 0 : (isB ? ktaB0 : ktaA0) + u;
-    const uint32_t soff = (uint32_t)kta * (isB ? kstepB : kstepA) + (uint32_t)j * (isB ? stepB : stepA);
+    const uint32_t soff = (uint32_t)kta * (isB ? kstepB : kstepA) + ((ROWS && !isB) ? ro.o[j] : (uint32_t)j * (isB ? stepB : stepA));
     __builtin_amdgcn_raw_ptr_buffer_load_lds(isB ? rsB : rsA, IA_LDS(dst), 16, off, (int)soff, 0, 0);
   };
 
@@ -768,8 +788,9 @@
   tie<0>(a0); tie<0>(b0);
 }
 
-template <bool BKS, int NH, bool WITH_BIAS>
-IA_DEV void drain_half_plain(const GemmArgs& p, f32x16 (&acc)[4][4], int m0, int n0, char* stg, int lane_e, const f32x4 (&bct)[4][4], float ts = 1.f) {
+template <bool BKS, int NH, bool WITH_BIAS, bool ROWS = false>
+IA_DEV void drain_half_plain(const GemmArgs& p, f32x16 (&acc)[4][4], int m0, int n0, char* stg, int lane_e, const f32x4 (&bct)[4][4], float ts = 1.f,
+                             RowBlk rb = RowBlk{}) {
   static_assert(!(WITH_BIAS && BKS), "bias rows are laid out for the k-contiguous B fragment permutation");
   const int hh = lane_e >> 5, li = lane_e & 31, rrow = lane_e >> 3, c8 = lane_e & 7;
   auto stage = [&](int mi) {
@@ -807,9 +828,9 @@
       __builtin_amdgcn_sched_barrier(0);
     }
   };
-  const int rows_left = p.M - m0;
+  const int rows_left = ROWS ? p.M : p.M - m0;
   const uint64_t wbytes = rows_left > 0 ? (uint64_t)rows_left * p.ldc * 2 : 0;
-  const __amdgpu_buffer_rsrc_t rsC = ia_rsrc(reinterpret_cast<bf16*>(p.C) + (size_t)m0 * p.ldc, (uint32_t)(wbytes < 0x7FFFFFF0ull ? wbytes : 0x7FFFFFF0ull));
+  const __amdgpu_buffer_rsrc_t rsC = ia_rsrc(reinterpret_cast<bf16*>(p.C) + (ROWS ? (size_t)0 : (size_t)m0 * p.ldc), (uint32_t)(wbytes < 0x7FFFFFF0ull ? wbytes : 0x7FFFFFF0ull));
   const int ncol = n0 + c8 * 8;
   const uint32_t voffC = ncol < p.N ? (uint32_t)((rrow * p.ldc + ncol) * 2) : 0x80000000u;
   stage(0);
@@ -827,16 +848,17 @@
     if (mi < 3) stage(mi + 1);
 #pragma unroll
     for (int it = 0; it < 4; ++it) {
-      const uint32_t off = voffC + (uint32_t)((mi * 32 + it * 8) * p.ldc * 2);
+      uint32_t off = voffC + (uint32_t)((mi * 32 + it * 8) * p.ldc * 2);
+      if constexpr (ROWS) off = rb.r[mi] >= 0 ? voffC + (uint32_t)(rb.r[mi] + it * 8) * (uint32_t)(p.ldc * 2) : 0x80000000u;
       if (!IA_GEMM_DBG_HOOKS || !(p.dbg & 64)) __builtin_amdgcn_raw_buffer_store_b128(v[it], rsC, (int)off, 0, 0);
       else asm volatile("" : : "v"(v[it]));
     }
   }
 }
 
-template <int EPI, bool OUTF32, bool BKS, int NH>
+template <int EPI, bool OUTF32, bool BKS, int NH, bool ROWS = false>
 IA_DEV void drain_half(const GemmArgs& p, f32x16 (&acc)[4][4], int m0, int n0, char* stg, int lane_e, bool full, bool bias_ready, f32x4 bias_lo,
-                       f32x4 bias_hi) {
+                       f32x4 bias_hi, RowBlk rb = RowBlk{}) {
   const int hh = lane_e >> 5, li = lane_e & 31;
   const int rrow = lane_e >> 3, c8 = lane_e & 7;
   constexpr bool HAS_BIAS = EPI == EPI_BIAS || EPI == EPI_BIAS_GELU || EPI == EPI_BIAS_GELU_ACT || EPI == EPI_BIAS_ADD;
@@ -853,8 +875,8 @@
     bf16x8 ax[AHEAD + 1];
     constexpr bool BUF = PRE && !OUTF32;
     const auto window = [&](const void* base, int ld) {
-      const uint64_t bytes = (uint64_t)(p.M - m0) * ld * 2;
-      return ia_rsrc(reinterpret_cast<const bf16*>(base) + (size_t)m0 * ld, (uint32_t)(bytes < 0x7FFFFFF0ull ? bytes : 0x7FFFFFF0ull));
+      const uint64_t bytes = (uint64_t)(ROWS ? p.M : p.M - m0) * ld * 2;
+      return ia_rsrc(reinterpret_cast<const bf16*>(base) + (ROWS ? (size_t)0 : (size_t)m0 * ld), (uint32_t)(bytes < 0x7FFFFFF0ull ? bytes : 0x7FFFFFF0ull));
     };
     BufIO io{ia_rsrc(nullptr, 0), ia_rsrc(nullptr, 0), 0u};
     __amdgpu_buffer_rsrc_t rsAux = ia_rsrc(nullptr, 0);
@@ -866,7 +888,8 @@
       if (HAS_AUX) { rsAux = window(p.aux, p.ldaux); voffAux = (uint32_t)((rrow * p.ldaux + n0 + c8 * 8) * 2); }
     }
     auto aux_of = [&](int c) {
-      const int row_in = (c >> 2) * 32 + ((c >> 1) & 1) * 16 + (c & 1) * 8;
+      int row_in = (c >> 2) * 32 + ((c >> 1) & 1) * 16 + (c & 1) * 8;
+      if constexpr (ROWS) row_in = rb.r[c >> 2] + (c & 3) * 8;
       if (BUF) return __builtin_bit_cast(bf16x8, __builtin_amdgcn_raw_buffer_load_b128(rsAux, (int)(voffAux + (uint32_t)(row_in * p.ldaux * 2)), 0, 0));
       return *reinterpret_cast<const bf16x8*>(p.aux + (size_t)(m0 + row_in + rrow) * p.ldaux + n0 + c8 * 8);
     };
@@ -907,17 +930,17 @@
 #pragma unroll
       for (int it = 0; it < 4; ++it) {
         const int row = it * 8 + rrow;
-        const int m = m0 + mi * 32 + row, n = n0 + c8 * 8;
+        const int m = ROWS ? rb.r[mi] + row : m0 + mi * 32 + row, n = n0 + c8 * 8;
         const int c = mi * 4 + it;
         if (PRE) {
           if (HAS_AUX && c + AHEAD < 16) {
             ax[(c + AHEAD) % (AHEAD + 1)] = aux_of(c + AHEAD);
             asm volatile("" ::: "memory");
           }
-          io.off = voffC + (uint32_t)((mi * 32 + it * 8) * p.ldc * 2);
+          io.off = voffC + (uint32_t)(((ROWS ? rb.r[mi] : mi * 32) + it * 8) * p.ldc * 2);
           if (!(IA_DBG(p) & 64)) epi_store8<EPI, OUTF32, true, BUF>(p, m, n, lo[it], hi[it], pb0, pb1, ax[c % (AHEAD + 1)], cs, &io);
         } else {
-          if (m < p.M && n < p.N && !(IA_DBG(p) & 64)) epi_store8<EPI, OUTF32, false>(p, m, n, lo[it], hi[it], pb0, pb1, ax[0], cs);
+          if ((!ROWS || rb.r[mi] >= 0) && m < p.M && n < p.N && !(IA_DBG(p) & 64)) epi_store8<EPI, OUTF32, false>(p, m, n, lo[it], hi[it], pb0, pb1, ax[0], cs);
         }
         if (IA_DBG(p) & 64) asm volatile("" : : "v"(lo[it]), "v"(hi[it]));
       }
@@ -943,13 +966,20 @@
 template <bool AKS, bool BKS, int EPI_, bool OUTF32>
 __global__ __launch_bounds__(256) void gemm_kernel(GemmArgs p) {
   constexpr bool LIVE = EPI_ == EPI_NONE_LIVE;
-  constexpr int EPI = LIVE ? (int)EPI_NONE : EPI_;
+  constexpr bool ROWS = EPI_ >= EPI_ROWS;
+  constexpr int EPI = LIVE ? (int)EPI_NONE : (ROWS ? EPI_ - EPI_ROWS : EPI_);
   static_assert(!LIVE || (AKS && BKS && OUTF32), "live k-tiles: the weight-gradient form only");
+  static_assert(!ROWS || (!AKS && !OUTF32 && (EPI == EPI_NONE || EPI == EPI_ADD || EPI == EPI_DGELU_CS)), "row remap: the data-gradient forms only");
   extern __shared__ __attribute__((aligned(16))) char smem[];
   const int tid = threadIdx.x, lane0 = tid & 63;
   const int wave = __builtin_amdgcn_readfirstlane(tid >> 6);
   const int wm = wave >> 1, wn = wave & 1;
   const int nk_all = (p.K + BK - 1) / BK;
+  [[maybe_unused]] int n_live = 0;
+  if constexpr (ROWS) {
+    n_live = __builtin_amdgcn_readfirstlane(p.row_blk[0]);
+    p.tiles_m = (n_live + 7) >> 3;
+  }
   const int total_tiles = p.tiles_m * p.tiles_n;
   int first_tile = blockIdx.x;
   bool ordered = false;
@@ -981,10 +1011,16 @@
     coords(tile, bm, bn);
     int lane = lane0;
     asm volatile("" : "+v"(lane));
-    const uint64_t oa = (uint64_t)(AKS ? kt0 * BK : bm * BM) * p.lda, ob = (uint64_t)(BKS ? kt0 * BK : bn * BN) * p.ldb;
+    RowOff ro{};
+    if constexpr (ROWS) {
+      const Blk8 bl = load_blk8(p.row_blk, bm, n_live);
+#pragma unroll
+      for (int j = 0; j < 8; ++j) ro.o[j] = (uint32_t)(bl.b[j] >= 0 ? bl.b[j] : bl.b[0]) * (uint32_t)(32 * p.lda * 2);
+    }
+    const uint64_t oa = (uint64_t)(AKS ? kt0 * BK : (ROWS ? 0 : bm * BM)) * p.lda, ob = (uint64_t)(BKS ? kt0 * BK : bn * BN) * p.ldb;
     constexpr bool PEEL_OK = !(EPI == EPI_BIAS && !OUTF32 && !BKS);
-    main_loop<AKS, BKS, PEND, PEEL_OK, LIVE>(p, smem, acc, rsrc_at(p.A, p.a_bytes, oa), rsrc_at(p.B, p.b_bytes, ob), AKS ? bm * BM : 0, BKS ? bn * BN : 0, kt0,
-                              AKS ? 0 : kt0, BKS ? 0 : kt0, n_tiles, nk_all, wm, wn, wave, lane, prologue_only, stores_in_flight, live_mv);
+    main_loop<AKS, BKS, PEND, PEEL_OK, LIVE, ROWS>(p, smem, acc, rsrc_at(p.A, p.a_bytes, oa), rsrc_at(p.B, p.b_bytes, ob), AKS ? bm * BM : 0, BKS ? bn * BN : 0, kt0,
+                              AKS ? 0 : kt0, BKS ? 0 : kt0, n_tiles, nk_all, wm, wn, wave, lane, prologue_only, stores_in_flight, live_mv, ro);
   };
 
   const bool dyn = p.tile_ctr != nullptr && !ordered;
@@ -1044,6 +1080,9 @@
     if (first_tile < 0) { leave(); return; }
     claim_issue();
   }
+  if constexpr (ROWS) {
+    if (!dyn && first_tile >= total_tiles) return;
+  }
 
   f32x16 acc[4][4];
 #pragma unroll
@@ -1105,6 +1144,24 @@
     int m0 = m0_pre, n0 = n0_pre;
     asm volatile("" : "+s"(m0), "+s"(n0));
     char* stg = smem + 2 * 2 * TILE_BYTES + wave * 2 * STAGE_BYTES;
+    bool full_e = full;
+    if constexpr (ROWS) {
+      const Blk8 bl = load_blk8(p.row_blk, bm, n_live);
+      RowBlk rb;
+#pragma unroll
+      for (int mi = 0; mi < 4; ++mi) rb.r[mi] = (wm ? bl.b[4 + mi] : bl.b[mi]) * 32;
+      const bool rows_ok = bl.b[7] >= 0 && bl.b[7] * 32 + 32 <= p.M;
+      full_e = rows_ok && n0_pre + 128 <= p.N;
+      if (!(IA_DBG(p) & 32)) {
+        if constexpr (EPI == EPI_NONE) {
+          drain_half_plain<BKS, 0, false, true>(p, acc, m0, n0, stg, lane_e, bct, 1.f, rb);
+          drain_half_plain<BKS, 1, false, true>(p, acc, m0, n0 + 64, stg, lane_e, bct, 1.f, rb);
+        } else {
+          drain_half<EPI, OUTF32, BKS, 0, true>(p, acc, m0, n0, stg, lane_e, full_e || (rows_ok && n0 + 64 <= p.N), false, pbv[0], pbv[1], rb);
+          drain_half<EPI, OUTF32, BKS, 1, true>(p, acc, m0, n0 + 64, stg, lane_e, full_e, false, pbv[2], pbv[3], rb);
+        }
+      }
+    } else
     if (!(IA_DBG(p) & 32)) {
       if constexpr (EPI == EPI_NONE && !OUTF32) {
         drain_half_plain<BKS, 0, false>(p, acc, m0, n0, stg, lane_e, bct);
@@ -1118,7 +1175,7 @@
       }
     }
     if (next >= total_tiles) break;
-    stores_in_flight = !(IA_DBG(p) & 96) && full;
+    stores_in_flight = !(IA_DBG(p) & 96) && full_e;
     if (!stores_in_flight) asm volatile("s_waitcnt vmcnt(0)" ::: "memory");
     tile = next;
   }
@@ -1132,19 +1189,41 @@
 namespace t256la {
 using namespace t256w;
 
+template <bool ROWS>
 __global__ __launch_bounds__(256) void gemm_kernel(GemmArgs p) {
   extern __shared__ __attribute__((aligned(16))) char smem[];
   const int tid = threadIdx.x, lane0 = tid & 63;
   const int wave = __builtin_amdgcn_readfirstlane(tid >> 6);
   const int wm = wave >> 1, wn = wave & 1;
   const int nk_all = (p.K + BK - 1) / BK;
+  [[maybe_unused]] int n_live = 0;
+  if constexpr (ROWS) {
+    n_live = __builtin_amdgcn_readfirstlane(p.row_blk[0]);
+    p.tiles_m = (n_live + 7) >> 3;
+  }
   const int total_tiles = p.tiles_m * p.tiles_n;
   const int n_tiles = nk_all;
+  if constexpr (ROWS) {
+    if ((int)blockIdx.x >= total_tiles) return;
+  }
   auto coords = [&](int tile, int& bm, int& bn) { tile_of_index(p, tile, total_tiles, bm, bn); };
   auto window_a = [&](int tile) {
     int bm = 0, bn = 0;
     if (tile < total_tiles) coords(tile, bm, bn);
-    return tile < total_tiles ? rsrc_at(p.A, p.a_bytes, (uint64_t)bm * BM * p.lda) : ia_rsrc(p.A, 0u);
+    return tile < total_tiles ? rsrc_at(p.A, p.a_bytes, ROWS ? (uint64_t)0 : (uint64_t)bm * BM * p.lda) : ia_rsrc(p.A, 0u);
+  };
+  auto rows_a = [&](int tile) {
+    RowOff ro{};
+    if constexpr (ROWS) {
+      if (tile < total_tiles) {
+        int bm = 0, bn = 0;
+        coords(tile, bm, bn);
+        const Blk8 bl = load_blk8(p.row_blk, bm, n_live);
+#pragma unroll
+        for (int j = 0; j < 8; ++j) ro.o[j] = (uint32_t)(bl.b[j] >= 0 ? bl.b[j] : bl.b[0]) * (uint32_t)(32 * p.lda * 2);
+      }
+    }
+    return ro;
   };
   auto window_b = [&](int tile) {
     int bm = 0, bn = 0;
@@ -1170,6 +1249,7 @@
   int tile = blockIdx.x;
   __amdgpu_buffer_rsrc_t rsA = window_a(tile), rsB = window_b(tile);
   __amdgpu_buffer_rsrc_t rsAn = window_a(tile + (int)gridDim.x), rsBn = window_b(tile + (int)gridDim.x);
+  [[maybe_unused]] RowOff roA = rows_a(tile), roAn = rows_a(tile + (int)gridDim.x);
 
   auto off_of = [&](int v) -> uint32_t {
     const int kt = v >= n_tiles ? v - n_tiles : v;
@@ -1179,7 +1259,7 @@
     const bool isB = i >= 8, nx = v >= n_tiles;
     const int j = i & 7, kt = nx ? v - n_tiles : v;
     char* dst = my_part + (isB ? TILE_BYTES : 0) + buf + j * 4096;
-    const uint32_t soff = (uint32_t)kt * (uint32_t)(BK * 2) + (uint32_t)j * (isB ? stepB : stepA);
+    const uint32_t soff = (uint32_t)kt * (uint32_t)(BK * 2) + ((ROWS && !isB) ? (nx ? roAn.o[j] : roA.o[j]) : (uint32_t)j * (isB ? stepB : stepA));
     const uint32_t off = ok ? (isB ? voffB : voffA) : OOB;
     __builtin_amdgcn_raw_ptr_buffer_load_lds(isB ? (nx ? rsBn : rsB) : (nx ? rsAn : rsA), IA_LDS(dst), 16, off, (int)soff, 0, 0);
   };
@@ -1262,12 +1342,22 @@
     int m0 = m0_pre, n0 = n0_pre;
     asm volatile("" : "+s"(m0), "+s"(n0));
     char* stg = smem + 2 * 2 * TILE_BYTES + wave * 2 * STAGE_BYTES;
+    if constexpr (ROWS) {
+      const Blk8 bl = load_blk8(p.row_blk, bm, n_live);
+      RowBlk rb;
+#pragma unroll
+      for (int mi = 0; mi < 4; ++mi) rb.r[mi] = (wm ? bl.b[4 + mi] : bl.b[mi]) * 32;
+      drain_half_plain<false, 0, false, true>(p, acc, m0, n0, stg, lane_e, no_bias, 1.f, rb);
+      drain_half_plain<false, 1, false, true>(p, acc, m0, n0 + 64, stg, lane_e, no_bias, 1.f, rb);
+    } else {
     drain_half_plain<false, 0, false>(p, acc, m0, n0, stg, lane_e, no_bias);
     drain_half_plain<false, 1, false>(p, acc, m0, n0 + 64, stg, lane_e, no_bias);
+    }
     tile += (int)gridDim.x;
     if (tile >= total_tiles) break;
     rsA = rsAn; rsB = rsBn;
     rsAn = window_a(tile + (int)gridDim.x); rsBn = window_b(tile + (int)gridDim.x);
+    if constexpr (ROWS) { roA = roAn; roAn = rows_a(tile + (int)gridDim.x); }
   }
   tie2<0>(a0, b0);
   asm volatile("s_waitcnt vmcnt(0)" ::: "memory");
@@ -1387,11 +1477,33 @@
   return base + (size_t)(g_launch_seq.fetch_add(1u, std::memory_order_relaxed) % CTR_SLOTS) * CTR_WORDS;
 }
 
+__global__ __launch_bounds__(256) void zero_dead_rows_kernel(const int* __restrict__ list, bf16* __restrict__ C, int ldc, int M, int N,
+                                                             float* __restrict__ csum_part, int part_rows) {
+  const int n_live = list[0], n_dead = list[1], nbr = (list[2] + 7) & ~7;
+  const int* dead = list + t256w::ROW_BLK_HDR + nbr;
+  const int n8 = N >> 3;
+  const u32x4 z = {0u, 0u, 0u, 0u};
+  for (int d = blockIdx.x; d < n_dead; d += gridDim.x) {
+    const int r0 = dead[d] * 32;
+    for (int i = threadIdx.x; i < 32 * n8; i += 256) {
+      const int r = r0 + i / n8, c = (i % n8) * 8;
+      if (r < M) *reinterpret_cast<u32x4*>(C + (size_t)r * ldc + c) = z;
+    }
+  }
+  if (csum_part) {
+    const int first = ((n_live + 7) >> 3) * 2;
+    const size_t total = part_rows > first ? (size_t)(part_rows - first) * N : 0;
+    float* base = csum_part + (size_t)first * N;
+    for (size_t i = (size_t)blockIdx.x * 256 + threadIdx.x; i < total; i += (size_t)gridDim.x * 256) base[i] = 0.f;
+  }
+}
+
 template <bool AKS, bool BKS, int EPI, bool OUTF32>
 int launch(GemmArgs a, bool big, hipStream_t st) {
   constexpr int vid = AKS * 1000 + BKS * 100 + EPI * 10 + (OUTF32 ? 1 : 0);
+  constexpr bool DROWS = !AKS && !OUTF32 && (EPI == EPI_NONE || EPI == EPI_ADD || EPI == EPI_DGELU_CS);
   constexpr bool WGRAD = AKS && BKS && EPI == EPI_NONE && OUTF32;
-  const bool rec = g_prof.on && g_prof.variant == vid && g_prof.n < g_prof.cap && !(WGRAD && a.live_kt);
+  const bool rec = g_prof.on && g_prof.variant == vid && g_prof.n < g_prof.cap && !(WGRAD && a.live_kt) && !(DROWS && a.row_blk);
   if (rec) (void)hipEventRecord(g_prof.ev[2 * g_prof.n], st);
   if (big) {
     a.tiles_m = (a.M + t256w::BM - 1) / t256w::BM; a.tiles_n = (a.N + t256w::BN - 1) / t256w::BN;
@@ -1399,14 +1511,22 @@
     const int gx = a.splits > 1 ? ntile * a.splits : (ntile < 256 ? ntile : 256);
     a.tile_ctr = (a.splits == 1 && ntile > gx) ? next_ctr_slot() : nullptr;
     void (*kern)(GemmArgs) = t256w::gemm_kernel<AKS, BKS, EPI, OUTF32>;
-    static bool attr_set[3] = {false, false, false};
+    static bool attr_set[5] = {false, false, false, false, false};
     int la = 0;
     if constexpr (WGRAD) {
       if (a.live_kt) { kern = t256w::gemm_kernel<true, true, EPI_NONE_LIVE, true>; la = 2; }
     }
     if constexpr (!AKS && !BKS && EPI == EPI_NONE && !OUTF32) {
       const char* e = getenv("IA_GEMM_LA");
-      if ((e ? atoi(e) : 1) && a.splits == 1 && ntile > gx && !a.tile_ctr && a.K >= 2 * BK && !(IA_DBG(a))) { kern = t256la::gemm_kernel; la = 1; }
+      if ((e ? atoi(e) : 1) && a.splits == 1 && ntile > gx && !a.tile_ctr && a.K >= 2 * BK && !(IA_DBG(a))) { kern = t256la::gemm_kernel<false>; la = 1; }
+    }
+    if constexpr (DROWS) {
+      if (a.row_blk) {
+        if (la == 1) kern = t256la::gemm_kernel<true>;
+        else kern = t256w::gemm_kernel<false, BKS, EPI_ROWS + EPI, false>;
+        la = la == 1 ? 4 : 3;
+        hipLaunchKernelGGL(zero_dead_rows_kernel, dim3(1024), dim3(256), 0, st, a.row_blk, (bf16*)a.C, a.ldc, a.M, a.N, a.csum_part, ((a.M + 255) / 256) * 2);
+      }
     }
     if (!attr_set[la]) {
       if (hipFuncSetAttribute((const void*)kern, hipFuncAttributeMaxDynamicSharedMemorySize, t256w::LDS_BYTES) != hipSuccess) return IA_ERR_LAUNCH;
@@ -1448,7 +1568,7 @@
 static int gemm_core(const void* A, int a_kstrided, int lda, const void* B, int b_kstrided, int ldb, void* C, int c_is_f32, int ldc, int M,
                      int N, int K, int epilogue, const float* bias, const void* aux, int ldaux, void* C2, int accumulate, void* workspace,
                      size_t workspace_bytes, const IaViewGemm* view, hipStream_t stream, int qcols = 0, float qscale = 1.f,
-                     const uint32_t* live_kt = nullptr);
+                     const uint32_t* live_kt = nullptr, const int* row_blocks = nullptr);
 
 extern "C" size_t ia_gemm_colsum_workspace_bytes(int M, int N) {
   if (M <= 0 || N <= 0) return 0;
@@ -1468,6 +1588,104 @@
                                    int scaled_cols, float col_scale, hipStream_t stream) {
   return gemm_core(A, 0, lda, B, 0, ldb, C, 0, ldc, M, N, K, EPI_BIAS, bias, nullptr, 0, nullptr, 0, nullptr, 0, nullptr, stream, scaled_cols,
                    col_scale);
+}
+
+static bool dgrad_rows_fit(int M, int lda, int ldc, int ldaux) {
+  const uint64_t lim = 0x7FFFFFF0ull, rows = (uint64_t)M + 32;
+  return rows * lda * 2 < lim && rows * ldc * 2 < lim && rows * (uint64_t)ldaux * 2 < lim && !(ldc & 7) && !(ldaux & 7);
+}
+static __host__ __device__ inline bool row_block_live(const uint8_t* row_live, int M, int t) {
+  const uint8_t* r = row_live + (size_t)t * 32;
+  const int n = M - t * 32 < 32 ? M - t * 32 : 32;
+  uint64_t any = 0;
+  if (n == 32 && ((uintptr_t)r & 7) == 0) {
+    for (int i = 0; i < 4; ++i) any |= reinterpret_cast<const uint64_t*>(r)[i];
+  } else {
+    for (int i = 0; i < n; ++i) any |= r[i];
+  }
+  return any != 0;
+}
+namespace {
+inline size_t al256(size_t b) { return (b + 255) & ~(size_t)255; }
+__global__ __launch_bounds__(64) void row_blocks_kernel(const uint8_t* __restrict__ row_live, int M, int nb, int* __restrict__ out) {
+  const int nbr = (nb + 7) & ~7;
+  int* const live = out + t256w::ROW_BLK_HDR;
+  int* const dead = live + nbr;
+  const int lane = threadIdx.x;
+  int base = 0;
+  for (int c0 = 0; c0 < nb; c0 += 64 * 64) {
+    uint64_t flags = 0;
+#pragma unroll 8
+    for (int i = 0; i < 64; ++i) {
+      const int t = c0 + i * 64 + lane;
+      if (t < nb && row_block_live(row_live, M, t)) flags |= 1ull << i;
+    }
+    for (int i = 0; i < 64 && c0 + i * 64 < nb; ++i) {
+      const int t = c0 + i * 64 + lane;
+      const bool lv = (flags >> i) & 1ull;
+      const uint64_t b = __ballot(lv);
+      const int at = base + __popcll(b & ((1ull << lane) - 1ull));
+      if (t < nb) { if (lv) live[at] = t; else dead[t - at] = t; }
+      base += __popcll(b);
+    }
+  }
+  if (lane < t256w::ROW_BLK_HDR) out[lane] = lane == 0 ? base : (lane == 1 ? nb - base : (lane == 2 ? nb : 0));
+}
+}
+
+extern "C" size_t ia_row_blocks_bytes(int M_rows) {
+  if (M_rows <= 0) return 0;
+  const size_t nbr = (size_t)(((M_rows + 31) / 32 + 7) & ~7);
+  return (t256w::ROW_BLK_HDR + 2 * nbr) * sizeof(int);
+}
+extern "C" int ia_row_blocks(const uint8_t* row_live, int M_rows, int* list, hipStream_t stream) {
+  (void)hipGetLastError();
+  if (!row_live || !list || M_rows <= 0 || ((uintptr_t)list & 31)) return IA_ERR_ARG;
+  hipLaunchKernelGGL(row_blocks_kernel, dim3(1), dim3(64), 0, stream, row_live, M_rows, (M_rows + 31) / 32, list);
+  return ia_check_launch();
+}
+extern "C" int ia_row_blocks_host(const uint8_t* row_live, int M_rows, int* list) {
+  if (!row_live || !list || M_rows <= 0) return IA_ERR_ARG;
+  const int nb = (M_rows + 31) / 32, nbr = (nb + 7) & ~7;
+  int* const live = list + t256w::ROW_BLK_HDR;
+  int* const dead = live + nbr;
+  int n_live = 0;
+  for (int t = 0; t < nb; ++t) {
+    if (row_block_live(row_live, M_rows, t)) live[n_live++] = t; else dead[t - n_live] = t;
+  }
+  for (int i = 0; i < t256w::ROW_BLK_HDR; ++i) list[i] = 0;
+  list[0] = n_live; list[1] = nb - n_live; list[2] = nb;
+  return IA_OK;
+}
+int ia_gemm_dgrad_blocks(const void* dY, int ldy, const void* W, int w_kstrided, int ldw, void* dX, int ldx, int M_rows, int N_in, int K_out,
+                         int epilogue, const void* aux, int ldaux, void* C2, const int* row_blocks, void* workspace, size_t workspace_bytes,
+                         hipStream_t stream) {
+  if (epilogue != EPI_NONE && epilogue != EPI_ADD && epilogue != EPI_DGELU_CS) return IA_ERR_UNSUPPORTED;
+  return gemm_core(dY, 0, ldy, W, w_kstrided, ldw, dX, 0, ldx, M_rows, N_in, K_out, epilogue, nullptr, aux, ldaux, C2, 0, workspace,
+                   workspace_bytes, nullptr, stream, 0, 1.f, nullptr, row_blocks);
+}
+extern "C" size_t ia_gemm_dgrad_rows_workspace_bytes(int M_rows, int N_in, int K_out) {
+  if (M_rows <= 0 || N_in <= 0 || K_out <= 0) return 0;
+  return al256(ia_gemm_colsum_workspace_bytes(M_rows, N_in)) + ia_row_blocks_bytes(M_rows);
+}
+extern "C" int ia_gemm_dgrad_rows_filters(int M_rows, int N_in, int K_out) {
+  if (M_rows <= 0 || N_in <= 0 || K_out <= 0 || (K_out & 7)) return 0;
+  return make_plan(M_rows, N_in, K_out, false).big && dgrad_rows_fit(M_rows, K_out, N_in, N_in) ? 1 : 0;
+}
+extern "C" int ia_gemm_dgrad_rows(const void* dY, int ldy, const void* W, int w_kstrided, int ldw, void* dX, int ldx, int M_rows, int N_in,
+                                  int K_out, int epilogue, const void* aux, int ldaux, void* C2, const uint8_t* row_live, void* workspace,
+                                  size_t workspace_bytes, hipStream_t stream) {
+  if (epilogue != EPI_NONE && epilogue != EPI_ADD && epilogue != EPI_DGELU_CS) return IA_ERR_UNSUPPORTED;
+  if (!row_live)
+    return gemm_core(dY, 0, ldy, W, w_kstrided, ldw, dX, 0, ldx, M_rows, N_in, K_out, epilogue, nullptr, aux, ldaux, C2, 0, workspace,
+                     workspace_bytes, nullptr, stream);
+  if (M_rows <= 0 || N_in <= 0 || K_out <= 0) return IA_ERR_ARG;
+  const size_t cs_bytes = al256(ia_gemm_colsum_workspace_bytes(M_rows, N_in));
+  if (!workspace || workspace_bytes < cs_bytes + ia_row_blocks_bytes(M_rows) || ((uintptr_t)workspace & 31)) return IA_ERR_WORKSPACE;
+  int* list = reinterpret_cast<int*>((char*)workspace + cs_bytes);
+  int rc = ia_row_blocks(row_live, M_rows, list, stream);
+  return rc ? rc : ia_gemm_dgrad_blocks(dY, ldy, W, w_kstrided, ldw, dX, ldx, M_rows, N_in, K_out, epilogue, aux, ldaux, C2, list, workspace,
+                                        cs_bytes, stream);
 }
 
 static __host__ __device__ inline uint32_t ktile_live(const uint8_t* row_live, int M, int t) {
@@ -1487,7 +1705,6 @@
   const uint64_t b = __ballot(t < nk && ktile_live(row_live, M, t));
   if ((threadIdx.x & 31) == 0 && t < nk) mask[t >> 5] = (uint32_t)(b >> (threadIdx.x & 32));
 }
-inline size_t al256(size_t b) { return (b + 255) & ~(size_t)255; }
 }
 
 extern "C" size_t ia_ktile_mask_bytes(int M_rows) {
@@ -1564,7 +1781,8 @@
 
 static int gemm_core(const void* A, int a_kstrided, int lda, const void* B, int b_kstrided, int ldb, void* C, int c_is_f32, int ldc, int M,
                      int N, int K, int epilogue, const float* bias, const void* aux, int ldaux, void* C2, int accumulate, void* workspace,
-                     size_t workspace_bytes, const IaViewGemm* view, hipStream_t stream, int qcols, float qscale, const uint32_t* live_kt) {
+                     size_t workspace_bytes, const IaViewGemm* view, hipStream_t stream, int qcols, float qscale, const uint32_t* live_kt,
+                     const int* row_blocks) {
   const uint64_t a_window = view ? view->a_window : 0, b_window = view ? view->b_window : 0;
   const int groups = view ? view->groups : 1;
   (void)hipGetLastError();
@@ -1610,6 +1828,8 @@
     if (wa >= 0x7FFFFFF0ull || wb >= 0x7FFFFFF0ull) return IA_ERR_ARG;
   }
   if (a_kstrided && b_kstrided && c_is_f32 && epilogue == EPI_NONE) g.live_kt = (big && g.nk_per_split <= t256w::LIVE_MAX_KTILES) ? live_kt : nullptr;
+  if (!a_kstrided && !c_is_f32 && (epilogue == EPI_NONE || epilogue == EPI_ADD || epilogue == EPI_DGELU_CS))
+    g.row_blk = (row_blocks && big && !g.dbg && dgrad_rows_fit(M, lda, ldc, aux ? ldaux : 0)) ? row_blocks : nullptr;
   const bool needs_bias = epilogue == EPI_BIAS || epilogue == EPI_BIAS_GELU || epilogue == EPI_BIAS_GELU_ACT || epilogue == EPI_BIAS_ADD;
   const bool needs_aux = epilogue == EPI_ADD || epilogue == EPI_DGELU || epilogue == EPI_BIAS_ADD || epilogue == EPI_DGELU_CS;
   if (needs_bias && !bias) return IA_ERR_ARG;
diff --git a/item_alignment_amd/ops.py b/item_alignment_amd/ops.py
--- a/item_alignment_amd/ops.py
+++ b/item_alignment_amd/ops.py
@@ -79,6 +79,36 @@
     return out
 
 
+def row_blocks(row_live):
+    lib = _lib.load()
+    _need(row_live, torch.uint8, "row_live")
+    M = row_live.numel()
+    out = torch.empty(lib.ia_row_blocks_bytes(M) // 4, device=row_live.device, dtype=torch.int32)
+    check(lib.ia_row_blocks(row_live.data_ptr(), M, out.data_ptr(), stream_ptr()), "ia_row_blocks")
+    return out
+
+
+def gemm_dgrad_rows(dy, w, row_live=None, *, w_kstrided=True, epilogue=EPI_NONE, aux=None, out=None, colsum_out=None):
+    lib = _lib.load()
+    _need(dy, BF16, "dy"); _need(w, BF16, "w"); _need(aux, BF16, "aux"); _need(row_live, torch.uint8, "row_live")
+    _need(colsum_out, F32, "colsum_out")
+    M, K = dy.shape
+    Kw, N = w.shape if w_kstrided else w.shape[::-1]
+    if K != Kw or (row_live is not None and row_live.numel() != M):
+        raise ValueError("gemm_dgrad_rows: dy, w and row_live do not fit together")
+    if epilogue == EPI_DGELU_COLSUM and colsum_out is None:
+        raise ValueError("gemm_dgrad_rows: EPI_DGELU_COLSUM needs colsum_out")
+    if out is None:
+        out = torch.empty((M, N), device=dy.device, dtype=BF16)
+    _need(out, BF16, "out")
+    ws_bytes = lib.ia_gemm_dgrad_rows_workspace_bytes(M, N, K)
+    ws = torch.empty(ws_bytes, device=dy.device, dtype=torch.uint8)
+    check(lib.ia_gemm_dgrad_rows(dy.data_ptr(), K, w.data_ptr(), int(w_kstrided), w.shape[1], out.data_ptr(), N, M, N, K, epilogue,
+                                 ptr(aux), N if aux is not None else 0, ptr(colsum_out), ptr(row_live), ws.data_ptr(), ws_bytes,
+                                 stream_ptr()), "ia_gemm_dgrad_rows")
+    return out
+
+
 def ln_fwd(x, gamma, beta, eps, *, bias=None, residual=None, write_z=True, drop_p=0.0, seed=0, stream_id=0):
     lib = _lib.load()
     _need(x, BF16, "x"); _need(gamma, F32, "gamma"); _need(beta, F32, "beta"); _need(bias, F32, "bias"); _need(residual, BF16, "residual")
```

After: 633.6, median of 6. +1.8%, better.
